# microsoft/neurips21-self-supervised-bug-detection-and-repair

Hardware: AMD Instinct MI355X
Metric: code-graphs/sec (train: fwd+bwd+optimizer) (higher is better)
Workload: dtype f32 (f16x3 / bf16x6 split products); 1 GPU; gnn-mlp hidden=128 layers=8 edge_types=16 batch=64 graphs/GPU x (2000 nodes, 10000 msgs) dropout=0.2; message_activation_placement=aggregated, message_gemm_split=f16x3, message_aggregation_function=max, global_batch=64, parallelism=dp1

## Files before the change

### include/buglab_hip.h

```cpp
#ifndef BUGLAB_HIP_H
#define BUGLAB_HIP_H

#include <stdint.h>

#ifdef __cplusplus
extern "C" {
#endif

#define BL_OK 0
#define BL_EINVAL (-1)
#define BL_ERANGE (-2)

enum { BL_ACT_NONE = 0, BL_ACT_RELU = 1, BL_ACT_SIGMOID = 2, BL_ACT_TANH = 3, BL_ACT_GELU = 4, BL_ACT_GELU_AGG = 5 };

const char* bl_last_error(void);
int bl_version(void);
void bl_set_deterministic(int32_t on);
int32_t bl_get_deterministic(void);

typedef struct {
  const float* x[3];
  const int32_t* idx[3];
  int32_t ld[3];
  int32_t width[3];
// ... 151 lines not shown
                               const uint32_t* win_bits, int32_t ld_bits, const int32_t* type_ptr, int32_t T, const float* wt,
                               int32_t E, int32_t Dm, int32_t Din, int32_t split, float* g_h_lo, int32_t ld_lo, float* g_h_hi,
                               int32_t ld_hi, float* g_src, int32_t ld_src, void* stream);

int bl_gru_cell_fwd(const float* gi, const float* gh, const float* h, int32_t ld_h, int32_t N, int32_t D,
                    bl_dropout_t drop, float* out, void* stream);
int bl_gru_cell_bwd(const float* g_out, const float* gi, const float* gh, const float* h, int32_t ld_h, int32_t N,
                    int32_t D, bl_dropout_t drop, float* g_gi, float* g_gh, float* g_h, void* stream);

int64_t bl_gru_scan_saved_elems(int32_t B, int32_t L, int32_t Hh);
int bl_gru_scan_fwd(const float* gi, int32_t ld_gi, const float* w_hh, const float* b_hh, const int32_t* lens, int32_t B, int32_t L,
                    int32_t Hh, float* out, int32_t ld_out, float* saved, void* stream);
int bl_gru_scan_bwd(const float* g_out, int32_t ld_g, const float* w_hh, const float* saved, const int32_t* lens, int32_t B, int32_t L,
                    int32_t Hh, float* g_gi, int32_t ld_ggi, float* g_gh, void* stream);

typedef struct {
  int32_t N, E, T, Din, Dm, Dout;
  const int32_t *msg_src, *msg_tgt, *type_ptr, *tgt_ptr, *tgt_msgs, *src_ptr, *src_msgs, *node_order;
  const float* W;
  const float *ln_g, *ln_b;
  const float* Wd;
  const float* bd;
  int32_t msg_act;
  float ln_eps;
  bl_dropout_t drop;
  const float* Wt;
  const uint16_t* Wd_packed;
  const uint16_t* Wd_packed_bwd;
  int32_t num_hub_slots;
  int32_t aggregation;
  int32_t num_runs;
  const int32_t* run_ptr;
  const int32_t* bwd_group_ptr;
  const int32_t* bwd_group_w;
  const int32_t* bwd_rows_tgt;
  const int32_t* bwd_rows_src;
  const int32_t* tgt_run_ptr;
  const int32_t* tgt_run_rows;
  int32_t live_num_nodes;
  int32_t live_num_recv;
  int32_t live_num_msgs;
  int32_t live_num_runs;
  const int32_t* live_nodes;
  const int32_t* live_recv;
  const int32_t* live_msgs;
  const int32_t* live_run_ptr;
  const int32_t* live_group_ptr;
  const int32_t* live_rows_tgt;
  const int32_t* live_rows_src;
  const int32_t* live_src_ptr;
  const int32_t* live_src_msgs;
  const int32_t* live_run_csr_ptr;
  const int32_t* live_run_csr_rows;
} bl_mp_layer_t;
#define BL_AGG_MAX 0
#define BL_AGG_SUM 1
#define BL_AGG_MEAN 2

int64_t bl_mp_layer_saved_bytes(int32_t N, int32_t E, int32_t Din, int32_t Dm, int32_t msg_act);
int64_t bl_mp_layer_workspace_bytes(int32_t N, int32_t E, int32_t Din, int32_t Dm, int32_t Dout, int32_t backward);
int32_t bl_mp_layer_weight_image(int32_t Din, int32_t Dm, int32_t for_backward);
int64_t bl_mp_layer_packed_weight_elems(int32_t T, int32_t Din, int32_t Dm, int32_t for_backward);

int bl_mp_layer_fwd(const bl_mp_layer_t* L, const float* h_lo, int32_t ld_lo, int32_t width_lo, const float* h_hi,
                    int32_t ld_hi, const uint16_t* w_packed, float* h_out, int32_t* winner_out, void* saved, void* ws,
                    void* stream);
int bl_mp_layer_bwd(const bl_mp_layer_t* L, const float* h_out, const float* g_out, const uint16_t* w_packed_bwd,
                    const void* saved, void* ws, float* g_h_lo, int32_t ld_lo, int32_t width_lo, float* g_h_hi,
                    int32_t ld_hi, float* g_W, float* g_ln_g, float* g_ln_b, float* g_Wd, float* g_bd, void* stream,
                    void* side_stream, int32_t join_side);

int32_t bl_node_update_bwd_ok(int32_t Dm, int32_t Dout);
int bl_node_update_bwd(const float* g_out, const float* h_out, int32_t nrows, int32_t Dout, bl_dropout_t drop,
                       const uint16_t* wd_packed_bwd, const float* agg, const float* mean, const float* rstd, const float* ln_g,
                       const float* dact, int32_t Dm, uint16_t* g_z_packed, float* g_bias, float* gq, uint16_t* gq_packed,
                       float* g_ln_g, float* g_ln_b, void* stream);
int32_t bl_set_fused_node_bwd(int32_t on);

int bl_winbits_or_runs(uint32_t* bits, int32_t ld_bits, const int32_t* run_ptr, int32_t E, int32_t R, int32_t words, void* stream);
int bl_mp_scatter_grad_runs(const float* g_a, int32_t ld_ga, const int32_t* src_ptr, const int32_t* src_msgs,
                            const int32_t* tgt_run_ptr, const int32_t* tgt_run_rows, int32_t N, int32_t Din, int32_t split,
                            float* g_h_lo, int32_t ld_lo, float* g_h_hi, int32_t ld_hi, const int32_t* node_order,
                            int32_t num_hub_slots, void* stream);
int32_t bl_set_run_rows(int32_t on);
int bl_winbits_gather(const uint32_t* bits, int32_t ld_bits, int32_t nrows_in, const int32_t* rows, int32_t n, int32_t words,
                      uint32_t* out, int32_t ld_out, void* stream);
int bl_node_update_bwd_rows(const float* g_out, const float* h_out, const int32_t* rows, int32_t nrows, int32_t Dout, bl_dropout_t drop,
                            const uint16_t* wd_packed_bwd, const float* agg, const float* mean, const float* rstd, const float* ln_g,
                            const float* dact, int32_t Dm, uint16_t* g_z_packed, float* g_bias, float* gq, uint16_t* gq_packed,
                            float* g_ln_g, float* g_ln_b, void* stream);
int bl_mp_scatter_grad_rows(const float* g_a, int32_t ld_ga, const int32_t* src_ptr, const int32_t* src_msgs,
                            const int32_t* run_csr_ptr, const int32_t* run_csr_rows, const int32_t* out_rows, int32_t n, int32_t Din,
                            int32_t split, float* g_h_lo, int32_t ld_lo, float* g_h_hi, int32_t ld_hi, void* stream);
int32_t bl_set_live_backward(int32_t on);
int32_t bl_get_live_backward(void);

int bl_prof_enable(int32_t on);
int bl_prof_reset(void);
int bl_prof_num_kinds(void);
const char* bl_prof_kind_name(int32_t kind);
int bl_prof_read(int32_t kind, double* ms, double* flop, int64_t* launches, int32_t* overlapped);
double bl_prof_read_bytes(int32_t kind);

#define BL_H3_ROW_SCALE 256.0f
#define BL_H3_W_SCALE 64.0f
int32_t bl_set_msg_gemm_mode(int32_t mode);
int32_t bl_get_msg_gemm_mode(void);
int32_t bl_set_seq_gemm_mode(int32_t mode);
int32_t bl_seq_gemm_mode(void);
int64_t bl_h3_saturation_events(int32_t reset);
int bl_pack_f16x2(const float* x, int32_t ld, int64_t R, int32_t D, int32_t D_total, int32_t col_off, float scale,
                  const float* amax_dev, uint16_t* out, void* stream);
int bl_amax(const float* x, int64_t n, float* amax_dev, void* stream);
int64_t bl_packed_weight_elems_h3(int32_t G, int32_t K, int32_t N);
int bl_pack_weights_h3(const float* w, int32_t G, int32_t K, int32_t N, int32_t w_is_kn, float scale, uint16_t* out, void* stream);
int bl_gemm_rows_h3(const bl_rows_packed_t* a, const uint32_t* win_bits, int32_t ld_bits, const uint16_t* bp, int64_t b_group_stride,
                    const int32_t* group_ptr, const int32_t* group_w, int32_t G, int32_t M, int32_t N, int32_t K, float out_scale,
                    const float* a_amax_dev, float* c, int32_t ldc, void* stream);
int bl_gemm_wgrad_h3(const bl_rows_packed_t* a, const uint16_t* g_packed, const int32_t* g_idx, const uint32_t* win_bits,
                     int32_t ld_bits, const int32_t* group_ptr, const int32_t* group_w, int32_t G, int32_t M, int32_t N, int32_t K,
                     float out_scale, const float* g_amax_dev, float* gw, int64_t gw_group_stride, int32_t ld_gw, void* stream);

int bl_calib_mfma_bf16(int32_t iters, int32_t workgroups, float* sink, double* flop, void* stream);
int bl_calib_stream_copy(const void* src, void* dst, int64_t nbytes, void* stream);

int bl_segment_log_softmax_fwd(const float* x, const int32_t* seg_ptr, const int32_t* seg_items, int32_t nseg,
                               float eps, float* y, void* stream);
int bl_segment_log_softmax_bwd(const float* g_y, const float* y, const int32_t* seg_ptr, const int32_t* seg_items,
                               int32_t nseg, float* g_x, void* stream);

int bl_rowdot_fwd(const float* x, int32_t ldx, const float* w, const float* b, int32_t R, int32_t H, float* y,
                  void* stream);
int bl_rowdot_bwd(const float* g_y, const float* x, int32_t ldx, const float* w, int32_t R, int32_t H, float* g_x,
                  int32_t ld_gx, float* g_w, float* g_b, void* stream);

int bl_scatter_add_rows(const float* src, int32_t ld_src, int32_t col_off, int32_t width, const int32_t* idx,
                        int32_t R, float* out, int32_t ld_out, void* stream);
int bl_gather_rows(const float* x, int32_t ld_x, const int32_t* idx, int32_t R, int32_t width, float* out,
                   int32_t ld_out, void* stream);

int bl_gather_concat_mlp_score_fwd(const bl_rows_t* a, const float* W1, const float* b1, const float* w2, const float* b2,
                                   int32_t R, int32_t H, float* hidden, float* score, void* stream);
int64_t bl_gather_concat_mlp_score_workspace_bytes(int32_t R, int32_t H, int32_t K);
int bl_gather_concat_mlp_score_bwd(const bl_rows_t* a, const float* W1, const float* w2, const float* hidden,
                                   const float* g_score, int32_t R, int32_t H, void* ws, float* g_W1, float* g_b1,
                                   float* g_w2, float* g_b2, float* const* g_x, const int32_t* ld_gx, void* stream);
int64_t bl_localization_scores_saved_bytes(int32_t C, int32_t B, int32_t H);
int64_t bl_localization_scores_workspace_bytes(int32_t C, int32_t B, int32_t H, int32_t backward);
// ... 337 lines not shown
```

### neurips21-self-supervised-bug-detection-and-repair_amd/buglab/models/hip_ops/_cabi.py

```python
from __future__ import annotations

import ctypes
import os
from ctypes import POINTER, Structure, c_double, c_float, c_int8, c_int32, c_int64, c_uint32, c_uint64, c_void_p
from typing import List, NamedTuple, Optional, Sequence, Tuple

import torch

__all__ = [
    "ACT_NONE", "ACT_RELU", "ACT_SIGMOID", "ACT_TANH", "ACT_GELU", "ACT_GELU_AGG", "_ACTS", "message_activation_code", "LIB_NAME",
    "HipOpsUnavailable", "bl_rows_t", "bl_rows_packed_t", "bl_dropout_t", "bl_mp_layer_t", "bl_x6_epi_t", "bl_head_view_t",
    "bl_packed_head_view_t", "bl_great_layer_t", "bl_great_layer_grads_t", "bl_pack_job_t", "bl_bug_loss_t", "bl_varmisuse_head_t",
    "VARMISUSE_STATS", "_SIGNATURES", "EXPORTED_SYMBOLS", "load_library", "_check", "_stream", "_p", "_req", "_f32", "_i32", "Dropout",
    "NO_DROPOUT", "RowSource", "_rows", "_rows_packed"]
FORWARDED_BY_PACKAGE = ("CALL_COUNT", "_lib", "LIB_PATH")

ACT_NONE, ACT_RELU, ACT_SIGMOID, ACT_TANH, ACT_GELU, ACT_GELU_AGG = 0, 1, 2, 3, 4, 5
_ACTS = {"none": ACT_NONE, "relu": ACT_RELU, "sigmoid": ACT_SIGMOID, "tanh": ACT_TANH, "gelu": ACT_GELU,
         "gelu_aggregated": ACT_GELU_AGG}


def message_activation_code(activation: str, placement: str = "aggregated") -> str:
    if activation not in ("gelu", "none"):
        raise ValueError(f"message_activation must be 'gelu' or 'none' (got {activation!r})")
    if placement not in ("aggregated", "message"):
        raise ValueError(f"message_activation_placement must be 'aggregated' or 'message' (got {placement!r})")
    return "gelu_aggregated" if (activation == "gelu" and placement == "aggregated") else activation
LIB_NAME = "libbuglab_hip.so"
LIB_PATH = os.environ.get("BL_HIP_LIB") or os.path.join(os.path.dirname(os.path.abspath(__file__)), LIB_NAME)


class HipOpsUnavailable(RuntimeError):
    pass


class bl_rows_t(Structure):
    _fields_ = [("x", c_void_p * 3), ("idx", c_void_p * 3), ("ld", c_int32 * 3), ("width", c_int32 * 3), ("nsrc", c_int32)]


class bl_rows_packed_t(Structure):
    _fields_ = [("xp", c_void_p * 3), ("idx", c_void_p * 3), ("width", c_int32 * 3), ("nsrc", c_int32)]


class bl_dropout_t(Structure):
    _fields_ = [("p", c_float), ("seed", c_uint32), ("stream", c_uint32)]


class bl_mp_layer_t(Structure):
    _fields_ = [("N", c_int32), ("E", c_int32), ("T", c_int32), ("Din", c_int32), ("Dm", c_int32), ("Dout", c_int32),
                ("msg_src", c_void_p), ("msg_tgt", c_void_p), ("type_ptr", c_void_p), ("tgt_ptr", c_void_p), ("tgt_msgs", c_void_p),
                ("src_ptr", c_void_p), ("src_msgs", c_void_p), ("node_order", c_void_p),
                ("W", c_void_p), ("ln_g", c_void_p), ("ln_b", c_void_p), ("Wd", c_void_p), ("bd", c_void_p),
                ("msg_act", c_int32), ("ln_eps", c_float), ("drop", bl_dropout_t), ("Wt", c_void_p),
                ("Wd_packed", c_void_p), ("Wd_packed_bwd", c_void_p), ("num_hub_slots", c_int32), ("aggregation", c_int32),
                ("num_runs", c_int32), ("run_ptr", c_void_p), ("bwd_group_ptr", c_void_p), ("bwd_group_w", c_void_p),
                ("bwd_rows_tgt", c_void_p), ("bwd_rows_src", c_void_p), ("tgt_run_ptr", c_void_p), ("tgt_run_rows", c_void_p),
                ("live_num_nodes", c_int32), ("live_num_recv", c_int32), ("live_num_msgs", c_int32), ("live_num_runs", c_int32),
                ("live_nodes", c_void_p), ("live_recv", c_void_p), ("live_msgs", c_void_p), ("live_run_ptr", c_void_p),
                ("live_group_ptr", c_void_p), ("live_rows_tgt", c_void_p), ("live_rows_src", c_void_p), ("live_src_ptr", c_void_p),
                ("live_src_msgs", c_void_p), ("live_run_csr_ptr", c_void_p), ("live_run_csr_rows", c_void_p)]


class bl_x6_epi_t(Structure):
    _fields_ = [("form", c_int32), ("bias", c_void_p), ("act", c_int32), ("drop", bl_dropout_t), ("res", c_void_p), ("ld_res", c_int32),
                ("y_packed", c_void_p), ("mask_scale", c_float), ("colsum", c_void_p), ("c_packed", c_void_p)]


class bl_head_view_t(Structure):
    _fields_ = [("p", c_void_p), ("sb", c_int64), ("sh", c_int32), ("sl", c_int32)]


class bl_packed_head_view_t(Structure):
    _fields_ = [("p", c_void_p), ("W", c_int32), ("col0", c_int32), ("hs", c_int32)]


class bl_great_layer_t(Structure):
    _fields_ = [("B", c_int32), ("L", c_int32), ("H", c_int32), ("dk", c_int32), ("T", c_int32), ("FF", c_int32),
                ("row_ptr", c_void_p), ("ekey", c_void_p), ("ecode", c_void_p), ("lens", c_void_p),
                ("bias_f", c_void_p), ("bias_r", c_void_p), ("norm_g", c_void_p), ("norm_b", c_void_p), ("lin1_b", c_void_p), ("lin2_b", c_void_p),
                ("qkv_w", c_void_p), ("out_w", c_void_p), ("lin1_w", c_void_p), ("lin2_w", c_void_p),
                ("qkv_w_bwd", c_void_p), ("out_w_bwd", c_void_p), ("lin1_w_bwd", c_void_p), ("lin2_w_bwd", c_void_p),
                ("ln_eps", c_float), ("drop_attn", bl_dropout_t), ("drop_att_out", bl_dropout_t), ("drop_ff_hidden", bl_dropout_t),
                ("drop_ff_out", bl_dropout_t)]


class bl_great_layer_grads_t(Structure):
    _fields_ = [("qkv_w", c_void_p), ("out_w", c_void_p), ("lin1_w", c_void_p), ("lin1_b", c_void_p), ("lin2_w", c_void_p), ("lin2_b", c_void_p),
                ("norm_g", c_void_p), ("norm_b", c_void_p), ("bias_f", c_void_p), ("bias_r", c_void_p)]


class bl_pack_job_t(Structure):
    _fields_ = [("w", c_void_p), ("out", c_void_p), ("kind", c_int32), ("G", c_int32), ("K", c_int32), ("N", c_int32),
                ("first_block", c_int32), ("pad_", c_int32)]


class bl_bug_loss_t(Structure):
    _fields_ = [("B", c_int32), ("C", c_int32), ("Rt", c_int32), ("Rv", c_int32), ("Rs", c_int32), ("G", c_int32),
                ("loc_scores", c_void_p), ("repair_logits", c_void_p), ("loc_group_ptr", c_void_p), ("loc_group_items", c_void_p),
                ("candidate_ptr", c_void_p), ("has_bug", c_void_p), ("correct_candidate_idxs", c_void_p),
                ("repair_group_ptr", c_void_p), ("repair_group_items", c_void_p), ("logit_group", c_void_p * 3),
                ("target", c_void_p * 3), ("ntarget", c_int32 * 3), ("w_buggy", c_float), ("abstain_weight", c_float)]


class bl_varmisuse_head_t(Structure):
    _fields_ = [("B", c_int32), ("L", c_int32), ("D", c_int32), ("ln_eps", c_float), ("x", c_void_p), ("ln_g", c_void_p), ("ln_b", c_void_p),
                ("W", c_void_p), ("bias", c_void_p), ("lens_att", c_void_p), ("error_location", c_void_p), ("candidate_mask", c_void_p),
                ("target_mask", c_void_p)]


VARMISUSE_STATS = 8


_SIGNATURES = {
    "bl_version": ([], ctypes.c_int),
    "bl_set_deterministic": ([c_int32], None),
    "bl_get_deterministic": ([], c_int32),
    "bl_set_wgrad_tile": ([c_int32], c_int32),
    "bl_set_wgrad_kchunk_cap": ([c_int32], c_int32),
    "bl_node_update_bwd_ok": ([c_int32, c_int32], c_int32),
    "bl_node_update_bwd": ([c_void_p, c_void_p, c_int32, c_int32, bl_dropout_t, c_void_p, c_void_p, c_void_p, c_void_p, c_void_p, c_void_p,
                            c_int32, c_void_p, c_void_p, c_void_p, c_void_p, c_void_p, c_void_p, c_void_p], ctypes.c_int),
    "bl_set_fused_node_bwd": ([c_int32], c_int32),
    "bl_set_run_rows": ([c_int32], c_int32),
    "bl_winbits_or_runs": ([c_void_p, c_int32, c_void_p, c_int32, c_int32, c_int32, c_void_p], ctypes.c_int),
    "bl_mp_scatter_grad_runs": ([c_void_p, c_int32, c_void_p, c_void_p, c_void_p, c_void_p, c_int32, c_int32, c_int32, c_void_p, c_int32, c_void_p,
                                 c_int32, c_void_p, c_int32, c_void_p], ctypes.c_int),
    "bl_set_live_backward": ([c_int32], c_int32),
    "bl_get_live_backward": ([], c_int32),
    "bl_winbits_gather": ([c_void_p, c_int32, c_int32, c_void_p, c_int32, c_int32, c_void_p, c_int32, c_void_p], ctypes.c_int),
    "bl_node_update_bwd_rows": ([c_void_p, c_void_p, c_void_p, c_int32, c_int32, bl_dropout_t, c_void_p, c_void_p, c_void_p, c_void_p, c_void_p,
                                 c_void_p, c_int32, c_void_p, c_void_p, c_void_p, c_void_p, c_void_p, c_void_p, c_void_p], ctypes.c_int),
    "bl_mp_scatter_grad_rows": ([c_void_p, c_int32, c_void_p, c_void_p, c_void_p, c_void_p, c_void_p, c_int32, c_int32, c_int32, c_void_p,
                                 c_int32, c_void_p, c_int32, c_void_p], ctypes.c_int),
    "bl_last_error": ([], ctypes.c_char_p),
    "bl_embed_subtoken_pool_fwd": ([c_void_p, c_int32, c_int32, c_void_p, c_void_p, c_int32, c_int32, c_int32, bl_dropout_t, c_int32, c_void_p, c_int32, c_void_p, c_void_p], ctypes.c_int),
    "bl_embed_subtoken_pool_bwd": ([c_void_p, c_int32, c_void_p, c_void_p, c_void_p, c_int32, c_int32, c_int32, c_int32, c_int32, bl_dropout_t, c_int32, c_void_p, c_void_p], ctypes.c_int),
    "bl_embed_subtoken_pool_bwd_sorted": ([c_void_p, c_int32, c_void_p, c_void_p, c_void_p, c_int32, c_void_p, c_void_p, c_int32, c_int32, c_int32, bl_dropout_t, c_int32, c_void_p, c_void_p], ctypes.c_int),
    "bl_embed_subtoken_max_fwd": ([c_void_p, c_int32, c_int32, c_void_p, c_void_p, c_int32, c_int32, bl_dropout_t, c_int32, c_void_p, c_int32, c_void_p, c_void_p], ctypes.c_int),
    "bl_embed_subtoken_max_bwd": ([c_void_p, c_int32, c_void_p, c_void_p, c_int32, c_int32, c_int32, c_int32, bl_dropout_t, c_int32, c_void_p, c_void_p], ctypes.c_int),
    "bl_embed_subtoken_max_bwd_sorted": ([c_void_p, c_int32, c_void_p, c_void_p, c_void_p, c_int32, c_void_p, c_int32, c_int32, bl_dropout_t, c_int32, c_void_p, c_void_p], ctypes.c_int),
    "bl_gemm_rows": ([POINTER(bl_rows_t), c_void_p, c_int64, c_int32, c_int32, c_void_p, c_void_p, c_void_p, c_int32, c_int32, c_int32, c_int32, c_int32, bl_dropout_t, c_void_p, c_int32, c_void_p], ctypes.c_int),
    "bl_gemm_rows_routed": ([POINTER(bl_rows_t), c_void_p, c_int32, c_void_p, c_int64, c_int32, c_void_p, c_void_p, c_int32, c_int32, c_int32, c_int32, c_void_p, c_int32, c_void_p], ctypes.c_int),
    "bl_pack_bf16x3": ([c_void_p, c_int32, c_int64, c_int32, c_void_p, c_void_p], ctypes.c_int),
    "bl_pack_weights_x6": ([c_void_p, c_int32, c_int32, c_int32, c_int32, c_void_p, c_void_p], ctypes.c_int),
    "bl_pack_job_blocks": ([c_int32, c_int32, c_int32, c_int32], c_int64),
    "bl_pack_weights_multi": ([c_void_p, c_int32, c_int32, c_void_p], ctypes.c_int),
    "bl_gemm_rows_x6": ([POINTER(bl_rows_packed_t), c_void_p, c_int32, c_void_p, c_int64, c_void_p, c_void_p, c_int32, c_int32, c_int32, c_int32, c_void_p, c_int32, c_void_p], ctypes.c_int),
    "bl_gemm_rows_x6w_ok": ([c_int32, c_int32], c_int32),
    "bl_set_rows_tile": ([c_int32], c_int32),
    "bl_packed_weight_elems_x6w": ([c_int32, c_int32, c_int32], c_int64),
    "bl_pack_weights_x6w": ([c_void_p, c_int32, c_int32, c_int32, c_int32, c_void_p, c_void_p], ctypes.c_int),
    "bl_gemm_rows_x6w": ([POINTER(bl_rows_packed_t), c_void_p, c_int32, c_void_p, c_int64, c_void_p, c_void_p, c_int32, c_int32, c_int32, c_int32, c_void_p, c_int32, c_void_p], ctypes.c_int),
    "bl_gemm_rows_x6_epi": ([POINTER(bl_rows_packed_t), c_void_p, c_int64, c_void_p, c_void_p, c_int32, c_int32, c_int32, c_int32, c_void_p, c_int32,
                             bl_dropout_t, c_void_p, c_int32, c_void_p], ctypes.c_int),
    "bl_gemm_rows_x6_epi2": ([POINTER(bl_rows_packed_t), c_void_p, c_int32, c_int32, c_int32, POINTER(bl_x6_epi_t), c_void_p, c_int32, c_void_p], ctypes.c_int),
    "bl_gemm_wgrad_x6": ([POINTER(bl_rows_packed_t), c_void_p, c_void_p, c_void_p, c_void_p, c_int32, c_int32, c_int32, c_int32, c_void_p, c_int64,
                          c_int32, c_void_p], ctypes.c_int),
    "bl_routed_dgrad_vec_ok": ([c_int32, c_int32], c_int32),
    "bl_routed_dgrad_vec": ([c_void_p, c_int32, c_void_p, c_void_p, c_int32, c_void_p, c_int32, c_void_p, c_int32, c_int32, c_int32, c_void_p, c_int32, c_void_p], ctypes.c_int),
    "bl_routed_dgrad_nodes": ([c_void_p, c_int32, c_void_p, c_void_p, c_void_p, c_int32, c_void_p, c_int32, c_void_p, c_int32, c_int32, c_int32, c_int32,
                               c_void_p, c_int32, c_void_p, c_int32, c_void_p], ctypes.c_int),
    "bl_routed_dgrad_nodes_rows": ([c_void_p, c_int32, c_void_p, c_void_p, c_void_p, c_int32, c_void_p, c_int32, c_void_p, c_int32, c_int32, c_int32,
                                    c_int32, c_void_p, c_int32, c_void_p, c_int32, c_void_p, c_int32, c_void_p], ctypes.c_int),
    "bl_gemm_wgrad_routed_x6": ([POINTER(bl_rows_packed_t), c_void_p, c_void_p, c_void_p, c_int32, c_void_p, c_void_p, c_int32, c_int32, c_int32, c_int32, c_void_p, c_int64, c_int32, c_void_p], ctypes.c_int),
    "bl_gemm_wgrad": ([POINTER(bl_rows_t), c_void_p, c_int32, c_void_p, c_void_p, c_int32, c_int32, c_int32, c_int32, c_void_p, c_int64, c_int32, c_void_p], ctypes.c_int),
    "bl_gemm_wgrad_routed": ([POINTER(bl_rows_t), c_void_p, c_int32, c_void_p, c_void_p, c_int32, c_void_p, c_void_p, c_int32, c_int32, c_int32, c_int32, c_void_p, c_int64, c_int32, c_void_p], ctypes.c_int),
    "bl_pack_bf16x3_cols": ([c_void_p, c_int32, c_int64, c_int32, c_int32, c_int32, c_void_p, c_void_p], ctypes.c_int),
    "bl_mp_scatter_grad_split": ([c_void_p, c_int32, c_void_p, c_void_p, c_void_p, c_void_p, c_int32, c_int32, c_int32, c_void_p, c_int32, c_void_p, c_int32, c_void_p, c_void_p], ctypes.c_int),
    "bl_mp_layer_saved_bytes": ([c_int32, c_int32, c_int32, c_int32, c_int32], c_int64),
    "bl_mp_layer_workspace_bytes": ([c_int32, c_int32, c_int32, c_int32, c_int32, c_int32], c_int64),
    "bl_mp_layer_packed_weight_elems": ([c_int32, c_int32, c_int32, c_int32], c_int64),
    "bl_mp_layer_weight_image": ([c_int32, c_int32, c_int32], c_int32),
    "bl_mp_layer_fwd": ([POINTER(bl_mp_layer_t), c_void_p, c_int32, c_int32, c_void_p, c_int32, c_void_p, c_void_p, c_void_p, c_void_p, c_void_p, c_void_p], ctypes.c_int),
    "bl_mp_layer_bwd": ([POINTER(bl_mp_layer_t), c_void_p, c_void_p, c_void_p, c_void_p, c_void_p, c_void_p, c_int32, c_int32, c_void_p, c_int32,
                         c_void_p, c_void_p, c_void_p, c_void_p, c_void_p, c_void_p, c_void_p, c_int32], ctypes.c_int),
    "bl_gather_concat_mlp_score_fwd": ([POINTER(bl_rows_t), c_void_p, c_void_p, c_void_p, c_void_p, c_int32, c_int32, c_void_p, c_void_p, c_void_p], ctypes.c_int),
    "bl_gather_concat_mlp_score_workspace_bytes": ([c_int32, c_int32, c_int32], c_int64),
    "bl_gather_concat_mlp_score_bwd": ([POINTER(bl_rows_t), c_void_p, c_void_p, c_void_p, c_void_p, c_int32, c_int32, c_void_p, c_void_p, c_void_p,
                                        c_void_p, c_void_p, POINTER(c_void_p), POINTER(c_int32), c_void_p], ctypes.c_int),
    "bl_localization_scores_saved_bytes": ([c_int32, c_int32, c_int32], c_int64),
    "bl_localization_scores_workspace_bytes": ([c_int32, c_int32, c_int32, c_int32], c_int64),
# ... 290 lines not shown
```

### neurips21-self-supervised-bug-detection-and-repair_amd/buglab/models/hip_ops/graph.py

```python
from __future__ import annotations

import ctypes
from typing import NamedTuple, Optional

import torch

from . import _switches, _streams
from ._cabi import (ACT_GELU_AGG, ACT_NONE, ACT_TANH, _ACTS, bl_mp_layer_t, _check, Dropout, _f32, _i32, load_library,
                    NO_DROPOUT, _p, _stream)
from ._streams import _direct_grad_target, _direct_small, _on_side_stream, _timed
from ._autograd import _take_saved
from .gemm import (act_bwd, gemm_rows, gemm_rows_routed, gemm_rows_x6, gemm_wgrad, gemm_wgrad_routed, gemm_wgrad_routed_x6,
                   layernorm_bwd, pack_bf16x3, pack_weights_x6, scatter_add_rows, segment_max, x6_ok)
from .weights import _as_groups, _packed_layer_weights, _packed_message_weights, _transposed_layer_weights

__all__ = ["GraphIndex", "MessageRuns", "LiveRows", "live_rows_of", "POOLINGS", "AGGREGATIONS", "_EmbedSubtokenMax", "embed_subtoken_max", "_MpLayer", "node_update_bwd",
           "_use_vector_dgrad", "_layer_desc", "_MpLayerFused", "_pending_uses", "set_grad_ready_callback", "_note_use",
           "_notify_backward_launched", "fused_layer_ok", "_GatedMpLayer", "gated_mp_layer", "_MpLayerFeat",
           "mp_layer_with_edge_features", "mp_layer"]


class MessageRuns(NamedTuple):

    run_ptr: torch.Tensor
    bwd_group_ptr: torch.Tensor
    bwd_group_w: torch.Tensor
    bwd_rows_tgt: torch.Tensor
    bwd_rows_src: torch.Tensor
    tgt_run_ptr: torch.Tensor
    tgt_run_rows: torch.Tensor

    @classmethod
    def of(cls, *arrays) -> Optional["MessageRuns"]:
        return cls(*arrays) if all(a is not None for a in arrays) else None

    @property
    def num_runs(self) -> int:
        return int(self.run_ptr.shape[0]) - 1


class LiveRows(NamedTuple):

    nodes: torch.Tensor
    recv: torch.Tensor
    msgs: torch.Tensor
    run_ptr: torch.Tensor
    group_ptr: torch.Tensor
    rows_tgt: torch.Tensor
    rows_src: torch.Tensor
    src_ptr: torch.Tensor
    src_msgs: torch.Tensor
    run_csr_ptr: torch.Tensor
    run_csr_rows: torch.Tensor


def live_rows_of(live_arrays: torch.Tensor, live_layout, T: int):
    out = []
    for row in (live_layout.tolist() if hasattr(live_layout, "tolist") else live_layout):
        nn, nr, ex, rx = row[:4]
        sizes = (nn, nr, ex, rx + 1, 2 * T + 1, ex + rx, ex + rx, nr + 1, ex, nr + 1, rx)
        out.append(LiveRows(*[live_arrays[o : o + n] for o, n in zip(row[4:], sizes)]))
    return out


class GraphIndex(NamedTuple):

    msg_src: torch.Tensor
    msg_tgt: torch.Tensor
    type_ptr: torch.Tensor
    tgt_ptr: torch.Tensor
    tgt_msgs: torch.Tensor
    src_ptr: torch.Tensor
    src_msgs: torch.Tensor
    num_nodes: int
    num_messages: int
    num_types: int
    node_order: Optional[torch.Tensor] = None
    num_hubs: int = -1
    runs: Optional[MessageRuns] = None
    live: Optional[LiveRows] = None


POOLINGS = ("max", "sum", "mean")


AGGREGATIONS = ("max", "sum", "mean")


class _EmbedSubtokenMax(torch.autograd.Function):
    @staticmethod
    def forward(ctx, table, ids, lens, drop: Dropout, tok_csr, before_pool: bool, comb: int):
        _f32(table, "embedding table")
        N, S = ids.shape
        V, H = table.shape
        out = torch.empty((N, H), dtype=torch.float32, device=table.device)
        argsub = torch.empty((N, H), dtype=torch.int8, device=table.device) if comb == 0 else None
        _check(
            load_library().bl_embed_subtoken_pool_fwd(table.data_ptr(), V, H, _i32(ids).data_ptr(), _i32(lens).data_ptr(), N, S, comb,
                                                      drop.c(), int(bool(before_pool)), out.data_ptr(), out.stride(0), _p(argsub), _stream()),
            "bl_embed_subtoken_pool_fwd")
        ctx.saved = (table, ids, lens, argsub, drop, V, H, tok_csr, int(bool(before_pool)), comb)
        return out

    @staticmethod
    def backward(ctx, g_out):
        table, ids, lens, argsub, drop, V, H, tok_csr, before_pool, comb = _take_saved(ctx)
        g_out = g_out.contiguous()
        N, S = ids.shape
        direct = _direct_small(table)
        g_table = direct if direct is not None else torch.zeros((V, H), dtype=torch.float32, device=g_out.device)
        if tok_csr is not None:
            occ, chunk_ptr, chunk_tok = tok_csr
            _check(
                load_library().bl_embed_subtoken_pool_bwd_sorted(g_out.data_ptr(), g_out.stride(0), _i32(occ).data_ptr(),
                                                                 _i32(chunk_ptr).data_ptr(), _i32(chunk_tok).data_ptr(),
                                                                 int(chunk_tok.shape[0]), _i32(lens).data_ptr(), _p(argsub), S, H, comb, drop.c(),
                                                                 before_pool, g_table.data_ptr(), _stream()),
                "bl_embed_subtoken_pool_bwd_sorted")
        else:
            _check(
                load_library().bl_embed_subtoken_pool_bwd(g_out.data_ptr(), g_out.stride(0), ids.data_ptr(), _i32(lens).data_ptr(), _p(argsub),
                                                          N, S, H, V, comb, drop.c(), before_pool, g_table.data_ptr(), _stream()),
                "bl_embed_subtoken_pool_bwd")
        return (None if direct is not None else g_table), None, None, None, None, None, None


def embed_subtoken_max(table, ids, lens, drop: Dropout = NO_DROPOUT, tok_csr=None, dropout_before_pooling: bool = False,
                       combination: str = "max"):
    return _EmbedSubtokenMax.apply(table, ids, lens, drop, tok_csr, bool(dropout_before_pooling), POOLINGS.index(combination))


class _MpLayer(torch.autograd.Function):

    @staticmethod
    def forward(ctx, h, W, ln_g, ln_b, Wd, bd, g: GraphIndex, msg_act: int, drop: Dropout):
# ... 72 lines not shown
        with side2:
            if hp is not None:
                gemm_wgrad_routed_x6([(hp, g.msg_src, Din), (hp, g.msg_tgt, Din)], gqp, g.msg_tgt, bits, E, Dm, g_W,
                                     gw_group_stride=K2 * Dm, group_ptr=g.type_ptr, G=T)
            else:
                gemm_wgrad_routed([(h, g.msg_src), (h, g.msg_tgt)], gq, g.msg_tgt, arg, E, Dm, g_W, gw_group_stride=K2 * Dm,
                                  group_ptr=g.type_ptr, G=T)
        if gqp is not None:
            g_a = gemm_rows_x6([(gqp, g.msg_tgt, Dm)], pack_weights_x6(W, False), E, K2, group_ptr=g.type_ptr, G=T,
                               win_bits=bits, kind="gemm_rows_nk_routed_x6")
        else:
            g_a = gemm_rows_routed(gq, g.msg_tgt, arg, W, E, K2, b_group_stride=K2 * Dm, ldb=Dm, group_ptr=g.type_ptr, G=T)
        g_h = torch.empty((N, Din), dtype=torch.float32, device=dev)
        _check(
            load_library().bl_mp_scatter_grad(g_a.data_ptr(), g_a.stride(0), g.src_ptr.data_ptr(), g.src_msgs.data_ptr(),
                                              g.tgt_ptr.data_ptr(), g.tgt_msgs.data_ptr(), N, Din, 0, g_h.data_ptr(),
                                              g_h.stride(0), _p(g.node_order), _stream()),
            "bl_mp_scatter_grad")
        if W_direct is not None and Wd_direct is not None:
            _streams.mark_free_running()
            side2.detach(h, gq, arg, bits, hp, gqp)
            side1.detach(ln_out, g_z)
            pair.__exit__(None, None, None)
            return g_h, None, g_lng, g_lnb, None, g_bd, None, None, None
        side2.join()
        side1.join()
        pair.__exit__(None, None, None)
        if W_direct is not None:
            g_W = None
        if Wd_direct is not None:
            g_Wd = None
        return g_h, g_W, g_lng, g_lnb, g_Wd, g_bd, None, None, None


def node_update_bwd(g_out, h_out, drop: "Dropout", wd_packed_bwd, agg, mean, rstd, ln_g, dact, g_bias, g_ln_g, g_ln_b, want_f32=True):
    N, Dout = g_out.shape
    Dm = agg.shape[1]
    dev = g_out.device
    gz = torch.empty((N, 3 * Dout), dtype=torch.int16, device=dev)
    gq = torch.empty((N, Dm), dtype=torch.float32, device=dev) if want_f32 else None
    gqp = torch.empty((N, 3 * Dm), dtype=torch.int16, device=dev)
    _check(load_library().bl_node_update_bwd(_f32(g_out).data_ptr(), _f32(h_out).data_ptr(), N, Dout, drop.c(), wd_packed_bwd.data_ptr(),
                                             _f32(agg).data_ptr(), mean.data_ptr(), rstd.data_ptr(), ln_g.data_ptr(), _p(dact), Dm,
                                             gz.data_ptr(), _p(g_bias), _p(gq), gqp.data_ptr(), g_ln_g.data_ptr(), g_ln_b.data_ptr(),
                                             _stream()), "bl_node_update_bwd")
    return gz, gq, gqp


def _use_vector_dgrad(lib, E: int, Dm: int, K2: int) -> bool:
    want = _switches.DGRAD_VEC if _switches.DGRAD_VEC is not None else not lib.bl_get_msg_gemm_mode()
    return bool(want) and E > 0 and bool(lib.bl_routed_dgrad_vec_ok(Dm, K2))


def _layer_desc(g: "GraphIndex", W, ln_g, ln_b, Wd, bd, Din, msg_act, drop: Dropout, agg: int = 0, backward: bool = False) -> bl_mp_layer_t:
    L = bl_mp_layer_t()
    L.aggregation = int(agg)
    L.N, L.E, L.T, L.Din, L.Dm, L.Dout = g.num_nodes, g.num_messages, W.shape[0], Din, W.shape[2], Wd.shape[1]
    L.msg_src, L.msg_tgt, L.type_ptr = g.msg_src.data_ptr(), g.msg_tgt.data_ptr(), g.type_ptr.data_ptr()
    L.tgt_ptr, L.tgt_msgs, L.src_ptr, L.src_msgs = g.tgt_ptr.data_ptr(), g.tgt_msgs.data_ptr(), g.src_ptr.data_ptr(), g.src_msgs.data_ptr()
    L.node_order = _p(g.node_order)
    L.num_hub_slots = int(g.num_hubs)
    L.W, L.ln_g, L.ln_b, L.Wd, L.bd = W.data_ptr(), ln_g.data_ptr(), ln_b.data_ptr(), Wd.data_ptr(), bd.data_ptr()
    L.msg_act, L.ln_eps, L.drop = int(msg_act), 1e-5, drop.c()
    if g.runs is not None and g.runs.num_runs > 0:
        L.num_runs = g.runs.num_runs
        for name in MessageRuns._fields:
            setattr(L, name, getattr(g.runs, name).data_ptr())
    if backward and g.live is not None and g.live.nodes.shape[0] > 0:
        lv = g.live
        L.live_num_nodes, L.live_num_recv = int(lv.nodes.shape[0]), int(lv.recv.shape[0])
        L.live_num_msgs, L.live_num_runs = int(lv.msgs.shape[0]), int(lv.run_ptr.shape[0]) - 1
        for name in LiveRows._fields:
            setattr(L, "live_" + name, getattr(lv, name).data_ptr())
    return L


class _MpLayerFused(torch.autograd.Function):

    @staticmethod
    def forward(ctx, h_lo, h_hi, W, ln_g, ln_b, Wd, bd, g: GraphIndex, msg_act: int, drop: Dropout, agg: int = 0):
        _f32(h_lo, "node states")
        lib = load_library()
        N = h_lo.shape[0]
        Din = h_lo.shape[1] + (h_hi.shape[1] if h_hi is not None else 0)
        T, K2, Dm = W.shape
        Dout = Wd.shape[1]
        E = g.num_messages
        assert K2 == 2 * Din and T == g.num_types and N == g.num_nodes
        for t, nm in ((W, "W"), (ln_g, "ln_g"), (ln_b, "ln_b"), (Wd, "Wd"), (bd, "bd")):
            _f32(t, nm)
        need_bwd = any(ctx.needs_input_grad[:7])
        use_vec = agg == 0 and _use_vector_dgrad(lib, E, Dm, K2)
        wkn, wnk = _packed_message_weights(W, Din, need_bwd and not use_vec)
        wt = _transposed_layer_weights(W) if (need_bwd and use_vec) else None
        dev = h_lo.device
        L = _layer_desc(g, W, ln_g, ln_b, Wd, bd, Din, msg_act, drop, agg)
        dense_x6 = _switches.DENSE_X6 and Dm % 32 == 0 and Dout % 32 == 0
        wd_kn = wd_nk = None
        if dense_x6:
            wd_kn, wd_nk = _packed_layer_weights(Wd, need_bwd)
            L.Wd_packed = wd_kn.data_ptr()
        infer = not need_bwd and _switches.INFERENCE_MODE
        saved_act = ACT_GELU_AGG if (agg == 2 and msg_act == ACT_NONE) else msg_act
        saved = None if infer else torch.empty((lib.bl_mp_layer_saved_bytes(N, E + L.num_runs, Din, Dm, saved_act),), dtype=torch.uint8, device=dev)
        ws = torch.empty((lib.bl_mp_layer_workspace_bytes(N, E, Din, Dm, Dout, 3 if infer else 0),), dtype=torch.uint8, device=dev)
        out = torch.empty((N, Dout), dtype=torch.float32, device=dev)
        winner = torch.empty((N, Dm), dtype=torch.int32, device=dev) if (_switches.WINNER_SINK is not None and agg == 0) else None
        _check(lib.bl_mp_layer_fwd(ctypes.byref(L), h_lo.data_ptr(), h_lo.stride(0), h_lo.shape[1], _p(h_hi),
                                   h_hi.stride(0) if h_hi is not None else 0, wkn.data_ptr(), out.data_ptr(), _p(winner),
                                   _p(saved), ws.data_ptr() if (E > 0 or infer) else None, _stream()), "bl_mp_layer_fwd")
        if winner is not None:
            _switches.WINNER_SINK.append(winner)
        if need_bwd:
            _note_use((W, ln_g, ln_b, Wd, bd))
        ctx.save_for_backward(out)
        ctx.saved = (h_lo.shape[1], h_hi.shape[1] if h_hi is not None else 0, W, ln_g, ln_b, Wd, bd, g, msg_act, drop, saved, wnk,
                     dense_x6, wd_kn, wd_nk, wt, agg)
        return out

    @staticmethod
    def backward(ctx, g_out):
        w_lo, w_hi, W, ln_g, ln_b, Wd, bd, g, msg_act, drop, saved, wnk, dense_x6, wd_kn, wd_nk, wt, agg = _take_saved(ctx)
        (out,) = ctx.saved_tensors
        lib = load_library()
        N, E = g.num_nodes, g.num_messages
        T, K2, Dm = W.shape
        Din, Dout = w_lo + w_hi, Wd.shape[1]
        dev = out.device
        g_out = g_out.contiguous()
        use_vec = agg == 0 and _use_vector_dgrad(lib, E, Dm, 2 * Din)
        if use_vec and wt is None:
            wt = _transposed_layer_weights(W)
        if wnk is None and not use_vec:
            wnk = _packed_message_weights(W, Din, True)[1]
        direct = [_direct_small(bd), _direct_small(ln_g), _direct_small(ln_b), _direct_grad_target(Wd), _direct_grad_target(W)]
        tgt = [d if d is not None else torch.zeros_like(p) for d, p in zip(direct, (bd, ln_g, ln_b, Wd, W))]
        g_bd, g_lng, g_lnb, g_Wd, g_W = tgt
        L = _layer_desc(g, W, ln_g, ln_b, Wd, bd, Din, msg_act, drop, agg, backward=True)
        if dense_x6:
            if wd_nk is None:
                wd_nk = pack_weights_x6(_as_groups(Wd.detach()), False)
            L.Wd_packed, L.Wd_packed_bwd = wd_kn.data_ptr(), wd_nk.data_ptr()
        ws_mode = 1
        if use_vec:
            L.Wt = wt.data_ptr()
            if not lib.bl_get_deterministic():
                ws_mode = 2
        ws = torch.empty((lib.bl_mp_layer_workspace_bytes(N, E, Din, Dm, Dout, ws_mode),), dtype=torch.uint8, device=dev)
        g_lo = torch.empty((N, w_lo), dtype=torch.float32, device=dev)
        g_hi = torch.empty((N, w_hi), dtype=torch.float32, device=dev) if w_hi else None
        side = _streams.side_stream_for_current_device()
        free_running = side is not None and direct[3] is not None and direct[4] is not None
        _check(lib.bl_mp_layer_bwd(ctypes.byref(L), out.data_ptr(), g_out.data_ptr(), _p(wnk), saved.data_ptr(), ws.data_ptr(),
                                   g_lo.data_ptr(), g_lo.stride(0), w_lo, _p(g_hi), g_hi.stride(0) if g_hi is not None else 0,
                                   g_W.data_ptr(), g_lng.data_ptr(), g_lnb.data_ptr(), g_Wd.data_ptr(), g_bd.data_ptr(), _stream(),
                                   side.cuda_stream if side is not None else None, 0 if free_running else 1), "bl_mp_layer_bwd")
        if free_running:
            _streams.mark_free_running(saved, ws)
        ret = [None if d is not None else t for d, t in zip(direct, tgt)]
        if all(d is not None for d in direct):
            _notify_backward_launched((W, ln_g, ln_b, Wd, bd))
        return g_lo, g_hi, ret[4], ret[1], ret[2], ret[3], ret[0], None, None, None, None


_pending_uses = {}


def set_grad_ready_callback(fn) -> None:
    _switches.GRAD_READY_CALLBACK = fn
    _pending_uses.clear()


def _note_use(params) -> None:
    if _switches.GRAD_READY_CALLBACK is not None:
        for p in params:
            _pending_uses[id(p)] = _pending_uses.get(id(p), 0) + 1


def _notify_backward_launched(params) -> None:
    if _switches.GRAD_READY_CALLBACK is None:
        return
    done = []
    for p in params:
        n = _pending_uses.get(id(p), 1) - 1
        if n <= 0:
            _pending_uses.pop(id(p), None)
            done.append(p)
        else:
            _pending_uses[id(p)] = n
    if done:
        _switches.GRAD_READY_CALLBACK(done)
# ... 94 lines not shown
            dact = None
        out = gemm_rows([(ln_out, None)], _f32(Wd, "Wd"), N, Dout, bias=_f32(bd), act=ACT_TANH, drop=drop)
        ctx.save_for_backward(out)
        ctx.saved = (h, hp, tp, bits, W, ln_g, Wd, table, msg_feat, dact, arg, agg, mean, rstd, ln_out, g, drop)
        return out

    @staticmethod
    def backward(ctx, g_out):
        h, hp, tp, bits, W, ln_g, Wd, table, msg_feat, dact, arg, agg, mean, rstd, ln_out, g, drop = _take_saved(ctx)
        (out,) = ctx.saved_tensors
        N, Din = h.shape
        T, K3, Dm = W.shape
        F, Dout, E, dev = table.shape[1], Wd.shape[1], g.num_messages, h.device
        z = lambda *shape: torch.zeros(shape, dtype=torch.float32, device=dev)
        g_bd, g_Wd, g_W, g_lng, g_lnb, g_table = z(Dout), torch.zeros_like(Wd), torch.zeros_like(W), z(Dm), z(Dm), torch.zeros_like(table)
        g_z = act_bwd(g_out.contiguous(), out, ACT_TANH, drop, g_bd)
        gemm_wgrad([(ln_out, None)], g_z, N, Dout, g_Wd)
        g_ln = gemm_rows([(g_z, None)], Wd, N, Dm, b_is_nk=True, ldb=Dout)
        if hp is not None:
            gqp = layernorm_bwd(g_ln, agg, mean, rstd, ln_g, g_lng, g_lnb, post_scale=dact, want="packed")
            gemm_wgrad_routed_x6([(hp, g.msg_src, Din), (hp, g.msg_tgt, Din), (tp, msg_feat, F)], gqp, g.msg_tgt, bits, E, Dm, g_W,
                                 gw_group_stride=K3 * Dm, group_ptr=g.type_ptr, G=T)
            g_a = gemm_rows_x6([(gqp, g.msg_tgt, Dm)], _packed_layer_weights(W, True)[1], E, K3, group_ptr=g.type_ptr, G=T, win_bits=bits,
                               kind="gemm_rows_nk_routed_x6")
        else:
            gq = layernorm_bwd(g_ln, agg, mean, rstd, ln_g, g_lng, g_lnb, post_scale=dact)
            src3 = [(h, g.msg_src), (h, g.msg_tgt), (table, msg_feat)]
            gemm_wgrad_routed(src3, gq, g.msg_tgt, arg, E, Dm, g_W, gw_group_stride=K3 * Dm, group_ptr=g.type_ptr, G=T)
            g_a = gemm_rows_routed(gq, g.msg_tgt, arg, W, E, K3, b_group_stride=K3 * Dm, ldb=Dm, group_ptr=g.type_ptr, G=T)
        g_h = torch.empty((N, Din), dtype=torch.float32, device=dev)
        _check(load_library().bl_mp_scatter_grad(g_a.data_ptr(), g_a.stride(0), g.src_ptr.data_ptr(), g.src_msgs.data_ptr(), g.tgt_ptr.data_ptr(),
                                                 g.tgt_msgs.data_ptr(), N, Din, 0, g_h.data_ptr(), g_h.stride(0), _p(g.node_order), _stream()),
               "bl_mp_scatter_grad")
        if E > 0:
            scatter_add_rows(g_a, 2 * Din, F, msg_feat, g_table)
        return g_h, g_W, g_lng, g_lnb, g_Wd, g_bd, g_table, None, None, None, None


def mp_layer_with_edge_features(h, W, ln_g, ln_b, Wd, bd, table, msg_feat, graph: GraphIndex, msg_act: str = "gelu_aggregated",
                                drop: Dropout = NO_DROPOUT):
    if isinstance(h, (tuple, list)):
        h = torch.cat(list(h), dim=-1)
    return _MpLayerFeat.apply(h.contiguous(), W, ln_g, ln_b, Wd, bd, table, msg_feat, graph, _ACTS[msg_act], drop)


def mp_layer(h, W, ln_g, ln_b, Wd, bd, graph: GraphIndex, msg_act: str = "gelu_aggregated", drop: Dropout = NO_DROPOUT,
             aggregation: str = "max"):
    pair = isinstance(h, (tuple, list))
    Din = sum(t.shape[1] for t in h) if pair else h.shape[1]
    agg = AGGREGATIONS.index(aggregation)
    if fused_layer_ok(Din, W.shape[2]) and (not pair or h[0].shape[1] % 32 == 0):
        lo, hi = (h[0].contiguous(), h[1].contiguous()) if pair else (h.contiguous(), None)
        return _MpLayerFused.apply(lo, hi, W, ln_g, ln_b, Wd, bd, graph, _ACTS[msg_act], drop, agg)
    if agg != 0:
        raise NotImplementedError("sum / mean message aggregation runs in the one-call layer form only (state and message widths multiples of "
                                  "32, message width <= 512, FUSED_LAYER on)")
    if pair:
        h = torch.cat(list(h), dim=-1)
    return _MpLayer.apply(h.contiguous(), W, ln_g, ln_b, Wd, bd, graph, _ACTS[msg_act], drop)
```

### neurips21-self-supervised-bug-detection-and-repair_amd/buglab/models/hip_ops/runtime.py

```python
from __future__ import annotations

import os

from . import _switches
from ._cabi import load_library

__all__ = ["set_deterministic", "_MSG_GEMM_MODES", "set_msg_gemm_mode", "msg_gemm_mode", "set_seq_gemm_mode", "seq_gemm_mode", "set_wgrad_tile",
           "set_wgrad_kchunk_cap", "set_fused_node_bwd", "set_run_rows", "set_live_backward", "live_backward", "deterministic"]


def set_deterministic(on: bool = True) -> None:
    load_library().bl_set_deterministic(1 if on else 0)
    os.environ["BL_DETERMINISTIC"] = "1" if on else "0"


_MSG_GEMM_MODES = ("bf16x6", "f16x3", "f16x1")


def set_msg_gemm_mode(mode: str) -> str:
    if mode not in _MSG_GEMM_MODES:
        raise ValueError(f"mode must be one of {_MSG_GEMM_MODES}")
    prev = load_library().bl_set_msg_gemm_mode(_MSG_GEMM_MODES.index(mode))
    return _MSG_GEMM_MODES[prev]


def msg_gemm_mode() -> str:
    return _MSG_GEMM_MODES[load_library().bl_get_msg_gemm_mode()]


def set_seq_gemm_mode(mode: str) -> str:
    if mode not in _switches._SEQ_GEMM_MODES:
        raise ValueError(f"mode must be one of {_switches._SEQ_GEMM_MODES}")
    prev = load_library().bl_set_seq_gemm_mode(_switches._SEQ_GEMM_MODES.index(mode))
    return _switches._SEQ_GEMM_MODES[prev]


def seq_gemm_mode() -> str:
    return _switches._SEQ_GEMM_MODES[load_library().bl_seq_gemm_mode()]


def set_wgrad_tile(rows: int) -> int:
    return int(load_library().bl_set_wgrad_tile(int(rows)))


def set_wgrad_kchunk_cap(rows: int) -> int:
    return int(load_library().bl_set_wgrad_kchunk_cap(int(rows)))


def set_fused_node_bwd(on: bool) -> bool:
    return bool(load_library().bl_set_fused_node_bwd(1 if on else 0))


def set_run_rows(on: bool) -> bool:
    return bool(load_library().bl_set_run_rows(1 if on else 0))


def set_live_backward(on: bool) -> bool:
    return bool(load_library().bl_set_live_backward(1 if on else 0))


def live_backward() -> bool:
    return bool(load_library().bl_get_live_backward())


def deterministic() -> bool:
    return bool(load_library().bl_get_deterministic())
```

### neurips21-self-supervised-bug-detection-and-repair_amd/buglab/models/layers/messagepassing.py

```python
from __future__ import annotations

import math
from typing import Any, Dict, List, NamedTuple, Optional

import torch
from torch import nn

from buglab.models import hip_ops
from buglab.models.hip_ops import Dropout, GraphIndex, MessageRuns, live_rows_of


class GnnOutput(NamedTuple):

    input_node_representations: torch.Tensor
    output_node_representations: torch.Tensor
    node_to_graph_idx: torch.Tensor
    node_idx_references: Dict[str, torch.Tensor]
    node_graph_idx_reference: Dict[str, torch.Tensor]
    num_graphs: int
    head_node_representations: Optional[torch.Tensor] = None
    head_idx_references: Optional[Dict[str, torch.Tensor]] = None


MAX_MESSAGE_DIMENSION = 512
# ... 86 lines not shown

    def __init__(self, state_dimension: int, message_dimension: int, num_edge_types: int,
                 message_aggregation_function: str = "max", dropout_rate: float = 0.0):
        super().__init__()
        if message_aggregation_function != "max":
            raise NotImplementedError("the HIP path implements the reference's `max` aggregation (gnnlayerdefs.py:47,63)")
        D, Dm, T = state_dimension, message_dimension, num_edge_types
        _check_message_width(Dm, "GatedMessagePassingLayer")
        self.state_dimension, self.message_dimension, self.output_state_dimension = D, Dm, D
        self.num_edge_types, self.dropout_rate = T, dropout_rate
        k = 1.0 / math.sqrt(D)
        self.W = nn.Parameter(_uniform_(torch.empty(T, D, Dm), 1.0 / math.sqrt(D)))
        self.Wi = nn.Parameter(_uniform_(torch.empty(Dm, 3 * D), k))
        self.bi = nn.Parameter(_uniform_(torch.empty(3 * D), k))
        self.Wh = nn.Parameter(_uniform_(torch.empty(D, 3 * D), k))
        self.bh = nn.Parameter(_uniform_(torch.empty(3 * D), k))

    def forward(self, node_states, graph: GraphIndex, drop: Dropout):
        return hip_ops.gated_mp_layer(node_states, self.W, self.Wi, self.bi, self.Wh, self.bh, graph, drop)


class ConcatResidualLayer:

    def __init__(self, hidden_state_size: int):
        self.hidden_state_size = hidden_state_size
        self.output_state_dimension = 2 * hidden_state_size
        self.dummy = _PassThrough(self)

    def pass_through_dummy_layer(self):
        return self.dummy


class _PassThrough:
    def __init__(self, owner: ConcatResidualLayer):
        self.owner = owner
        self.output_state_dimension = owner.hidden_state_size


class GraphNeuralNetwork(nn.Module):

    def __init__(self, node_embedder: SubtokenEmbedder, layer_recipe: List[Any], edge_embedder: Optional[TokenEmbedder] = None):
        super().__init__()
        self.embed = node_embedder
        self.edge_embed = edge_embedder
        self._recipe = layer_recipe
        mp, seen = [], set()
        for l in layer_recipe:
            if isinstance(l, (MlpMessagePassingLayer, GatedMessagePassingLayer)) and id(l) not in seen:
                seen.add(id(l))
                mp.append(l)
        self.mp = nn.ModuleList(mp)
        self.input_node_state_dim = node_embedder.embedding_size
        self.output_node_state_dim = [l for l in layer_recipe if isinstance(l, nn.Module)][-1].output_state_dimension

    @property
    def message_passing_layers(self):
        return list(self.mp)

    def forward(self, *, token_ids, token_lens, msg_src, msg_tgt, type_ptr, tgt_ptr, tgt_msgs, src_ptr, src_msgs,
                node_to_graph, reference_node_ids, reference_node_graph_idx, num_graphs, num_nodes, num_messages,
                return_all_states: bool = False, dropout_seed: Optional[int] = None, tok_occ=None, tok_chunk_ptr=None,
                tok_chunk_id=None, node_order=None, num_hub_nodes: int = -1, msg_feat=None, input_transform=None, run_ptr=None,
                bwd_group_ptr=None, bwd_group_w=None, bwd_rows_tgt=None, bwd_rows_src=None, tgt_run_ptr=None, tgt_run_rows=None,
                live_arrays=None, live_layout=None, live_backward: bool = False, **_unused) -> GnnOutput:
        graph = GraphIndex(msg_src, msg_tgt, type_ptr, tgt_ptr, tgt_msgs, src_ptr, src_msgs, int(num_nodes),
                           int(num_messages), int(type_ptr.shape[0]) - 1, node_order, int(num_hub_nodes),
                           MessageRuns.of(run_ptr, bwd_group_ptr, bwd_group_w, bwd_rows_tgt, bwd_rows_src, tgt_run_ptr, tgt_run_rows))
        training = self.training and dropout_seed is not None
        seed = int(dropout_seed or 0)
        mk = lambda rate, stream: Dropout(rate if training else 0.0, seed, stream)
        tok_csr = (tok_occ, tok_chunk_ptr, tok_chunk_id) if tok_occ is not None else None
        h0 = self.embed(token_ids, token_lens, mk(self.embed.dropout_rate, 0), tok_csr)
        if input_transform is not None:
            h0 = input_transform(h0)
        edge_features = None
        if self.edge_embed is not None:
            if msg_feat is None:
                raise ValueError("the model has an edge-feature embedding but the minibatch carries no `msg_feat`")
            edge_features = (self.edge_embed.table, msg_feat)
        live = []
        if live_backward and live_arrays is not None and live_layout is not None and not return_all_states and input_transform is None:
            live = live_rows_of(live_arrays, live_layout, graph.num_types)
        num_mp = sum(1 for l in self._recipe if isinstance(l, nn.Module))
        h = h0
        all_states = [h0]
        stash: Dict[int, torch.Tensor] = {}
        li = 0
        for layer in self._recipe:
            if isinstance(layer, _PassThrough):
                stash[id(layer.owner)] = h
            elif isinstance(layer, ConcatResidualLayer):
                h = (stash.pop(id(layer)), h)
            else:
                if isinstance(h, tuple) and not isinstance(layer, MlpMessagePassingLayer):
                    h = torch.cat(h, dim=-1)
                depth = num_mp - 1 - li
                layer_graph = graph._replace(live=live[depth]) if depth < len(live) else graph
                if isinstance(layer, MlpMessagePassingLayer) and layer.features_dimension > 0:
                    h = layer(h, graph, mk(layer.dropout_rate, 1 + li), edge_features)
                else:
                    h = layer(h, layer_graph, mk(layer.dropout_rate, 1 + li))
                li += 1
                all_states.append(h)
        if isinstance(h, tuple):
            h = torch.cat(h, dim=-1)
        out = torch.cat(all_states, dim=-1) if return_all_states else h
        return GnnOutput(h0, out, node_to_graph, reference_node_ids, reference_node_graph_idx, int(num_graphs))
```

### neurips21-self-supervised-bug-detection-and-repair_amd/csrc/bl_common.h

```cpp
#pragma once
#include <hip/hip_runtime.h>
#include <stdint.h>
#include <stdio.h>

#include "../../include/buglab_hip.h"

#define BL_WAVE 64

void bl_set_error(const char* fmt, ...);
extern "C" int32_t bl_get_deterministic(void);
int bl_num_cus();
int bl_max_lds_per_block();
unsigned* bl_order_counters(int n, void* stream);
unsigned* bl_h3_sat_counter();

int bl_segment_max_fwd_impl(const float* x, int32_t ldx, const int32_t* seg_ptr, const int32_t* seg_items, int32_t nseg, int32_t D,
                            int32_t act, float* out, int32_t* arg, const float* ln_g, const float* ln_b, float eps, float* ln_out,
                            float* mean, float* rstd, float* dact, uint32_t* winbits, const int32_t* seg_order,
                            uint16_t* ln_out_packed, int32_t num_hub_slots, void* stream);
int bl_segment_sum_fwd_impl(const float* x, int32_t ldx, const int32_t* seg_ptr, const int32_t* seg_items, int32_t nseg, int32_t D,
                            int32_t act, int32_t mean_agg, float* out, const float* ln_g, const float* ln_b, float eps, float* ln_out,
                            float* mean, float* rstd, float* dact, const int32_t* seg_order, uint16_t* ln_out_packed, void* stream);
int bl_act_bwd_impl(const float* g_y, const float* y, int32_t nrows, int32_t N, int32_t ld, int32_t act, bl_dropout_t drop,
                    float* g_z, float* g_bias, uint16_t* g_z_packed, void* stream);
int bl_mp_scatter_src_accum_impl(const float* g_src, int32_t ld_src, const int32_t* src_ptr, const int32_t* src_msgs, int32_t N,
                                 int32_t Din, int32_t split, float* g_h_lo, int32_t ld_lo, float* g_h_hi, int32_t ld_hi,
                                 const int32_t* node_order, int32_t hub_slots, void* stream);
int bl_mp_scatter_grad_hubs_impl(const float* g_a, int32_t ld_ga, const int32_t* src_ptr, const int32_t* src_msgs, const int32_t* tgt_ptr,
                                 const int32_t* tgt_msgs, int32_t N, int32_t Din, int32_t split, float* g_h_lo, int32_t ld_lo, float* g_h_hi,
                                 int32_t ld_hi, const int32_t* node_order, int32_t hub_slots, int32_t col_tgt, void* stream,
                                 const int32_t* out_rows = nullptr);
int bl_gemm_wgrad_h3_impl(const bl_rows_packed_t* a, const uint16_t* g_packed, const int32_t* g_idx, const uint32_t* win_bits,
                          int32_t ld_bits, const int32_t* group_ptr, const int32_t* group_w, int32_t G, int32_t M, int32_t N, int32_t K,
                          float out_scale, const float* g_amax_dev, float* gw, int64_t gw_group_stride, int32_t ld_gw,
                          bool group_w_one_to_one, void* stream);

int bl_node_update_bwd_impl(const float* g_out, const float* h_out, int32_t nrows, int32_t Dout, bl_dropout_t drop,
                            const uint16_t* wd_packed_bwd, const float* agg, const float* mean, const float* rstd, const float* ln_g,
                            const float* dact, int32_t Dm, uint16_t* g_z_packed, float* g_bias, float* gq, uint16_t* gq_packed,
                            float* g_ln_g, float* g_ln_b, float* gq_amax, const int32_t* rows, void* stream);

struct BlProfScope {
  void* st;
  bool on;
  BlProfScope(int kind, double flop, void* stream, double bytes = 0.0, bool overlapped = false);
  ~BlProfScope();
};
enum {
  BL_PROF_PACK_ROWS = 0,
  BL_PROF_LINEAR_FWD = 17,
  BL_PROF_LINEAR_DGRAD,
  BL_PROF_LINEAR_WGRAD,
  BL_PROF_ATTN_PROBS_FWD,
  BL_PROF_ATTN_PROBS_BWD,
  BL_PROF_ATTN_ROWS_TIMES,
  BL_PROF_ATTN_TRANSPOSED_TIMES,
  BL_PROF_ADD_LAYERNORM,
  BL_PROF_LAYERNORM_BWD_BRANCH
};

#define BL_CHECK_ARG(cond, ...)   \
  do {                            \
    if (!(cond)) {                \
      bl_set_error(__VA_ARGS__);  \
      return BL_EINVAL;           \
    }                             \
  } while (0)
#define BL_CHECK_RANGE(cond, ...) \
  do {                            \
    if (!(cond)) {                \
      bl_set_error(__VA_ARGS__);  \
      return BL_ERANGE;           \
// ... 138 lines not shown
```

### neurips21-self-supervised-bug-detection-and-repair_amd/csrc/bl_gemm_h3.hip

```cpp
#include <stdio.h>
#include <stdlib.h>

#include "bl_common.h"
#include "bl_gemm_host.h"
#include "bl_gemm_split.h"
#include "bl_x6_locate.h"
#include "bl_h3_image.h"

__global__ __launch_bounds__(256) void pack_rows_h_kernel(const float* __restrict__ x, int ld, long long R, int D, uint4* __restrict__ out,
                                                          int kg_total, int kg_off, float scale, const float* __restrict__ amax_dev,
                                                          unsigned* __restrict__ sat_counter) {
  const int kgs = D >> 3;
  const long long t = (long long)blockIdx.x * blockDim.x + threadIdx.x;
  if (t >= R * kgs) return;
  if (amax_dev) scale *= h3_scale_from_amax(*amax_dev);
  const long long r = t / kgs;
  const int kgn = kg_total;
  const int kg = (int)(t % kgs) + kg_off;
  x -= 8 * kg_off;
  const float4 a = *reinterpret_cast<const float4*>(x + r * ld + 8 * kg);
  const float4 b = *reinterpret_cast<const float4*>(x + r * ld + 8 * kg + 4);
  const float v[8] = {a.x, a.y, a.z, a.w, b.x, b.y, b.z, b.w};
  uint16_t h[8], l[8];
  bool sat = false;
#pragma unroll
  for (int j = 0; j < 8; ++j) split2h(v[j] * scale, h[j], l[j], sat);
  if (sat && sat_counter) atomicAdd(sat_counter, 1u);
  uint4* o = out + r * 2 * kgn + kg;
  o[0] = make_uint4(PK(h[0], h[1]), PK(h[2], h[3]), PK(h[4], h[5]), PK(h[6], h[7]));
  o[kgn] = make_uint4(PK(l[0], l[1]), PK(l[2], l[3]), PK(l[4], l[5]), PK(l[6], l[7]));
}

__global__ __launch_bounds__(256) void pack_weights_h_kernel(const float* __restrict__ w, int G, int K, int N, int w_is_kn,
                                                             uint4* __restrict__ out, float scale, unsigned* __restrict__ sat_counter) {
  pack_weights_h_thread(w, G, K, N, w_is_kn, out, (long long)blockIdx.x * blockDim.x + threadIdx.x, scale, sat_counter);
}

template <bool MASKED, bool ONE>
__global__ __launch_bounds__(256, MASKED ? 2 : 3) void gemm_rows_h3_kernel(
    const uint4* __restrict__ xp0, const uint4* __restrict__ xp1, const uint4* __restrict__ xp2,
    const int* __restrict__ idx0, const int* __restrict__ idx1, const int* __restrict__ idx2, int w0, int w1, int w2,
    int koff1, int koff2, int nsrc, const uint32_t* __restrict__ win_bits, int ld_bits, const uint4* __restrict__ bp,
    long long strideB, const int* __restrict__ group_ptr, const int* __restrict__ group_w, int G, int M, int N, int K,
    float* __restrict__ c, int ldc, int xcd_remap, float out_scale, const float* __restrict__ a_amax_dev) {
  gemm_rows_body<SplitF16x2, MASKED, -1, ONE>(xp0, xp1, xp2, idx0, idx1, idx2, w0, w1, w2, koff1, koff2, nsrc, win_bits, ld_bits, bp,
                                              strideB, group_ptr, group_w, G, M, N, K, c, ldc, xcd_remap, X6Epi{}, out_scale, a_amax_dev);
}

template <bool ROUTED, bool ONE>
__global__ __launch_bounds__(256, 2) void gemm_wgrad_h3_kernel(
    const uint4* __restrict__ xp0, const uint4* __restrict__ xp1, const uint4* __restrict__ xp2,
    const int* __restrict__ idx0, const int* __restrict__ idx1, const int* __restrict__ idx2, int w0, int w1, int w2,
    int koff1, int koff2, int nsrc, const uint4* __restrict__ gp, const int* __restrict__ g_idx,
    const uint32_t* __restrict__ win_bits, int ld_bits, const int* __restrict__ group_ptr, const int* __restrict__ group_w, int G,
    int M, int N, int K, int kchunk, float* __restrict__ gw_base, long long strideW, int ldw, int ntiles_n, int xcd_remap,
    unsigned* __restrict__ order_ctr, float out_scale, const float* __restrict__ g_amax_dev) {
  gemm_wgrad_body<SplitF16x2, ROUTED, ONE>(xp0, xp1, xp2, idx0, idx1, idx2, w0, w1, w2, koff1, koff2, nsrc, gp, g_idx, win_bits, ld_bits,
                                           group_ptr, group_w, G, M, N, K, kchunk, gw_base, strideW, ldw, ntiles_n, xcd_remap, order_ctr,
                                           out_scale, g_amax_dev);
}

__global__ __launch_bounds__(256) void amax_kernel(const float* __restrict__ x, long long n4, float* __restrict__ amax) {
  __shared__ float part[4];
  float m = 0.f;
  const long long stride = (long long)gridDim.x * blockDim.x;
  for (long long i = (long long)blockIdx.x * blockDim.x + threadIdx.x; i < n4; i += stride) {
    const float4 v = reinterpret_cast<const float4*>(x)[i];
    m = fmaxf(m, fmaxf(fmaxf(fabsf(v.x), fabsf(v.y)), fmaxf(fabsf(v.z), fabsf(v.w))));
  }
  m = bl_wave_max(m);
  if ((threadIdx.x & 63) == 0) part[threadIdx.x >> 6] = m;
  __syncthreads();
  if (threadIdx.x == 0) {
    m = fmaxf(fmaxf(part[0], part[1]), fmaxf(part[2], part[3]));
    if (m > 0.f) atomicMax(reinterpret_cast<unsigned int*>(amax), __float_as_uint(m));
  }
}

unsigned* bl_h3_sat_counter() {
  static unsigned* ctr[BL_MAX_DEVICES] = {nullptr};
  int dev = 0;
  if (hipGetDevice(&dev) != hipSuccess || dev < 0 || dev >= BL_MAX_DEVICES) return nullptr;
  if (ctr[dev] == nullptr) {
    if (hipMalloc((void**)&ctr[dev], sizeof(unsigned)) != hipSuccess) return nullptr;
    if (hipMemset(ctr[dev], 0, sizeof(unsigned)) != hipSuccess) return nullptr;
  }
  return ctr[dev];
}

extern "C" int64_t bl_h3_saturation_events(int32_t reset) {
  unsigned* c = bl_h3_sat_counter();
  unsigned v = 0;
  if (c == nullptr || hipMemcpy(&v, c, sizeof(v), hipMemcpyDeviceToHost) != hipSuccess) return -1;
  if (reset && hipMemset(c, 0, sizeof(unsigned)) != hipSuccess) return -1;
  return (int64_t)v;
}

extern "C" int bl_pack_f16x2(const float* x, int32_t ld, int64_t R, int32_t D, int32_t D_total, int32_t col_off, float scale,
                             const float* amax_dev, uint16_t* out, void* stream) {
  if (R == 0) return BL_OK;
  BL_CHECK_ARG(x && out && bl_aligned16(x) && bl_aligned16(out), "bl_pack_f16x2: null or misaligned pointer");
  BL_CHECK_ARG(D > 0 && D % 8 == 0 && ld % 4 == 0 && D_total % 8 == 0 && col_off % 8 == 0 && col_off >= 0 && col_off + D <= D_total,
               "bl_pack_f16x2: widths / offset must be multiples of 8 with col_off + D <= D_total");
  BL_CHECK_ARG(scale > 0.f, "bl_pack_f16x2: scale must be positive (a power of two)");
  const long long total = (long long)R * (D / 8);
  hipLaunchKernelGGL(pack_rows_h_kernel, dim3((unsigned)((total + 255) / 256)), dim3(256), 0, (hipStream_t)stream, x, ld, (long long)R, D,
                     reinterpret_cast<uint4*>(out), D_total / 8, col_off / 8, scale, amax_dev, bl_h3_sat_counter());
  BL_LAUNCH_CHECK("bl_pack_f16x2");
  return BL_OK;
}

extern "C" int bl_amax(const float* x, int64_t n, float* amax_dev, void* stream) {
  if (n == 0) return BL_OK;
  BL_CHECK_ARG(x && amax_dev && bl_aligned16(x) && n % 4 == 0, "bl_amax: aligned pointer and a multiple of 4 elements required");
  const long long n4 = n / 4;
  const int grid = (int)((n4 + 255) / 256 < (long long)bl_num_cus() * 2 ? (n4 + 255) / 256 : (long long)bl_num_cus() * 2);
  hipLaunchKernelGGL(amax_kernel, dim3(grid), dim3(256), 0, (hipStream_t)stream, x, n4, amax_dev);
  BL_LAUNCH_CHECK("bl_amax");
  return BL_OK;
}

extern "C" int64_t bl_packed_weight_elems_h3(int32_t G, int32_t K, int32_t N) { return (int64_t)G * ((N + 127) / 128) * (K / 32) * 8192; }

extern "C" int bl_pack_weights_h3(const float* w, int32_t G, int32_t K, int32_t N, int32_t w_is_kn, float scale, uint16_t* out,
                                  void* stream) {
  if (G == 0) return BL_OK;
  BL_CHECK_ARG(w && out && bl_aligned16(out), "bl_pack_weights_h3: null or misaligned pointer");
  BL_CHECK_ARG(K > 0 && K % 32 == 0 && N > 0 && scale > 0.f, "bl_pack_weights_h3: K must be a multiple of 32 (got %d), scale positive", K);
  const long long total = (long long)G * ((N + 127) / 128) * (K / 32) * 512;
  hipLaunchKernelGGL(pack_weights_h_kernel, dim3((unsigned)((total + 255) / 256)), dim3(256), 0, (hipStream_t)stream, w, G, K, N, w_is_kn,
                     reinterpret_cast<uint4*>(out), scale, bl_h3_sat_counter());
  BL_LAUNCH_CHECK("bl_pack_weights_h3");
  return BL_OK;
}

bool g_h3_one_term = false;

extern "C" int bl_gemm_rows_h3(const bl_rows_packed_t* a, const uint32_t* win_bits, int32_t ld_bits, const uint16_t* bp,
                               int64_t b_group_stride, const int32_t* group_ptr, const int32_t* group_w, int32_t G, int32_t M, int32_t N,
                               int32_t K, float out_scale, const float* a_amax_dev, float* c, int32_t ldc, void* stream) {
  const char* who = "bl_gemm_rows_h3";
  if (M == 0) return BL_OK;
  BlPackedRows r;
  dim3 grid;
  if (int rc = bl_rows_gemm_plan(who, a, win_bits, ld_bits, bp, group_ptr, G, M, N, K, c, ldc, XBM, r, grid)) return rc;
  BL_CHECK_ARG(b_group_stride % 8 == 0 && (G <= 1 || b_group_stride >= bl_packed_weight_elems_h3(1, K, N)),
               "%s: packed group stride must cover one group's tiled weights (bl_pack_weights_h3)", who);
  BL_CHECK_ARG(out_scale > 0.f, "%s: out_scale must be positive", who);
#define H3_ARGS                                                                                                               \
  BL_PACKED_ROWS_ARGS(r), win_bits, ld_bits, reinterpret_cast<const uint4*>(bp), (long long)(b_group_stride / 8), group_ptr, \
      group_w, G, M, N, K, c, ldc, 1, out_scale, a_amax_dev
  if (g_h3_one_term) {
    if (win_bits)
      hipLaunchKernelGGL((gemm_rows_h3_kernel<true, true>), grid, dim3(256), 0, (hipStream_t)stream, H3_ARGS);
    else
      hipLaunchKernelGGL((gemm_rows_h3_kernel<false, true>), grid, dim3(256), 0, (hipStream_t)stream, H3_ARGS);
  } else if (win_bits)
    hipLaunchKernelGGL((gemm_rows_h3_kernel<true, false>), grid, dim3(256), 0, (hipStream_t)stream, H3_ARGS);
  else
    hipLaunchKernelGGL((gemm_rows_h3_kernel<false, false>), grid, dim3(256), 0, (hipStream_t)stream, H3_ARGS);
  BL_LAUNCH_CHECK(who);
// ... 47 lines not shown
```

### neurips21-self-supervised-bug-detection-and-repair_amd/csrc/bl_gemm_split.h

```cpp
#pragma once
#include <float.h>

#include "bl_common.h"
#include "bl_x6_locate.h"

typedef float f32x16 __attribute__((ext_vector_type(16)));
typedef __bf16 bf16x8 __attribute__((ext_vector_type(8)));
typedef _Float16 f16x8 __attribute__((ext_vector_type(8)));
typedef short s16x4 __attribute__((ext_vector_type(4)));

#define XBM 128
#define XBN 128
#define PK(a_, b_) ((uint32_t)(a_) | ((uint32_t)(b_) << 16))

__device__ __forceinline__ float h3_scale_from_amax(float amax) {
  if (!(amax > 0.f) || amax > FLT_MAX) return 1.f;
  int e;
  (void)frexpf(amax, &e);
  int k = 14 - e;
  k = k > 100 ? 100 : (k < -100 ? -100 : k);
  return ldexpf(1.f, k);
}

struct SplitBf16x3 {
  static constexpr int NP = 3;
  typedef bf16x8 frag;
  static constexpr bool SCALED = false;
  static constexpr bool STREAM_OUT = false;
  static constexpr bool swizzled(bool masked) { return masked; }
  static constexpr int row(bool masked, bool one) { return one ? (masked ? 4 : 5) : (masked ? 12 : 13); }
  static constexpr int NT = 6;
  static __device__ __forceinline__ f32x16 term(int t, const frag* x, const frag* y, f32x16 a) {
    constexpr int X[NT] = {1, 2, 0, 1, 0, 0}, Y[NT] = {1, 0, 2, 0, 1, 0};
    return __builtin_amdgcn_mfma_f32_32x32x16_bf16(x[X[t]], y[Y[t]], a, 0, 0, 0);
  }
};

struct SplitF16x2 {
  static constexpr int NP = 2;
  typedef f16x8 frag;
  static constexpr bool SCALED = true;
  static constexpr bool STREAM_OUT = true;
  static constexpr bool swizzled(bool) { return false; }
  static constexpr int row(bool, bool) { return 9; }
  static constexpr int NT = 3;
  static __device__ __forceinline__ f32x16 term(int t, const frag* x, const frag* y, f32x16 a) {
    constexpr int X[NT] = {1, 0, 0}, Y[NT] = {0, 1, 0};
    return __builtin_amdgcn_mfma_f32_32x32x16_f16(x[X[t]], y[Y[t]], a, 0, 0, 0);
  }
};

struct X6Epi {
  const float* bias;
  int act;
  uint32_t drop_key, drop_thresh;
  float drop_scale;
  int form;
  const float* res;
  int ld_res;
  const uint2* himask;
  float mask_scale;
  float* colsum;
  uint2* c_packed;
};

template <class S, bool MASKED, int EPI, bool ONE>
__device__ __forceinline__ void gemm_rows_body(
    const uint4* __restrict__ xp0, const uint4* __restrict__ xp1, const uint4* __restrict__ xp2,
    const int* __restrict__ idx0, const int* __restrict__ idx1, const int* __restrict__ idx2, int w0, int w1, int w2,
    int koff1, int koff2, int nsrc, const uint32_t* __restrict__ win_bits, int ld_bits, const uint4* __restrict__ bp,
    long long strideB, const int* __restrict__ group_ptr, const int* __restrict__ group_w, int G, int M, int N, int K,
    float* __restrict__ c, int ldc, int xcd_remap, X6Epi epi, float out_scale, const float* __restrict__ a_amax_dev) {
  static_assert(EPI == -1 || !S::SCALED, "the epilogues are built for the unscaled split only");
  constexpr bool E_ACT = EPI >= 0 && EPI < 32, E_PACK = EPI >= 16 && (EPI < 32 || EPI == 64), E_RES = EPI == 32, E_MASK = EPI == 64;
  constexpr int ACT = EPI >= 0 ? (EPI & 15) : 0;
  constexpr bool SWZ = S::swizzled(MASKED);
  constexpr int NP = ONE ? 1 : S::NP;
  constexpr int T0 = ONE ? S::NT - 1 : 0;
  constexpr int XROW = S::row(MASKED, ONE);
  constexpr int XEPI = 4 * 32 * 68 / 4;
  constexpr int XLDS = (XBM + XBN) * XROW > XEPI ? (XBM + XBN) * XROW : XEPI;
#define XSLOT(row_, kg_) (SWZ ? ((kg_) ^ (((row_) >> 2) & 3)) : (kg_))
  __shared__ uint4 ABs[XLDS];
  uint4* As = ABs;
  uint4* Bs = ABs + XBM * XROW;

  const int tid = threadIdx.x, lane = tid & 63, wave = tid >> 6;
  int g, row0, nrows, tile_y;
  if (!x6_locate(group_ptr, G, M, XBM, xcd_remap, tile_y, g, row0, nrows)) return;
  const int n0 = tile_y * XBN;
  const int wsel = group_w ? group_w[g] : g;
  const uint4* __restrict__ Bt = bp + (long long)wsel * strideB + (size_t)tile_y * (K >> 5) * (S::NP * 512) + tid;

  const int p_kg = tid & 3, p_row0 = tid >> 2;
  int gr0[2], gr1[2], gr2[2];
#pragma unroll
  for (int i = 0; i < 2; ++i) {
    const int r = row0 + min(p_row0 + 64 * i, nrows - 1);
    gr0[i] = idx0 ? idx0[r] : r;
    gr1[i] = nsrc > 1 ? (idx1 ? idx1[r] : r) : 0;
    gr2[i] = nsrc > 2 ? (idx2 ? idx2[r] : r) : 0;
  }
  uint4 ra[2][NP], rb[2][NP];
  uint32_t ma[2];
  const int nk = (K + 31) / 32;

#define ROWS_LOAD_STAGE(k0_)                                                                                  \
  {                                                                                                           \
    const int k_ = (k0_) + 8 * p_kg;                                                                          \
    const int kc_ = k_ < K ? k_ : 0;                                                                          \
    int j_ = 0;                                                                                               \
    if (nsrc > 1 && kc_ >= koff1) j_ = 1;                                                                     \
    if (nsrc > 2 && kc_ >= koff2) j_ = 2;                                                                     \
    const int kl_ = kc_ - (j_ == 0 ? 0 : (j_ == 1 ? koff1 : koff2));                                          \
    const uint4* base_ = j_ == 0 ? xp0 : (j_ == 1 ? xp1 : xp2);                                               \
    const int wj_ = j_ == 0 ? w0 : (j_ == 1 ? w1 : w2);                                                       \
    _Pragma("unroll") for (int i = 0; i < 2; ++i) {                                                           \
      const int row_ = p_row0 + 64 * i;                                                                       \
      const int gr_ = j_ == 0 ? gr0[i] : (j_ == 1 ? gr1[i] : gr2[i]);                                         \
      const uint4* src_ = base_ + (size_t)gr_ * S::NP * (wj_ >> 3) + (kl_ >> 3);                              \
      ra[i][0] = src_[0];                                                                                     \
      if constexpr (NP > 1) ra[i][1] = src_[wj_ >> 3];                                                        \
      if constexpr (NP > 2) ra[i][2] = src_[2 * (wj_ >> 3)];                                                  \
      if (MASKED) ma[i] = win_bits[(size_t)(row0 + min(row_, nrows - 1)) * ld_bits + (kc_ >> 5)];              \
      const uint4* bsrc_ = Bt + (size_t)((k0_) >> 5) * (S::NP * 512) + i * (S::NP * 256);                     \
      rb[i][0] = bsrc_[0];                                                                                    \
      if constexpr (NP > 1) rb[i][1] = bsrc_[256];                                                            \
// ... 24 lines not shown
#pragma unroll
    for (int tj = 0; tj < 2; ++tj)
#pragma unroll
      for (int r = 0; r < 16; ++r) acc[ti][tj][r] = 0.f;

  const int wm = wave >> 1, wn = wave & 1, li = lane & 31, half = lane >> 5;

  ROWS_LOAD_STAGE(0)
  ROWS_STORE_STAGE(0)
  __syncthreads();
  for (int kt = 0; kt < nk; ++kt) {
    if (kt + 1 < nk) ROWS_LOAD_STAGE((kt + 1) * 32)
#pragma unroll
    for (int s = 0; s < 2; ++s) {
      const int kg = 2 * s + half;
      typename S::frag af[2][NP], bf[2][NP];
#pragma unroll
      for (int t = 0; t < 2; ++t) {
        const uint4* pa = &As[(wm * 64 + t * 32 + li) * XROW + XSLOT(li, kg)];
        const uint4* pb = &Bs[(wn * 64 + t * 32 + li) * XROW + XSLOT(li, kg)];
#pragma unroll
        for (int p = 0; p < NP; ++p) {
          af[t][p] = __builtin_bit_cast(typename S::frag, pa[4 * p]);
          bf[t][p] = __builtin_bit_cast(typename S::frag, pb[4 * p]);
        }
      }
#pragma unroll
      for (int ti = 0; ti < 2; ++ti)
#pragma unroll
        for (int tj = 0; tj < 2; ++tj) {
          f32x16 a = acc[ti][tj];
#pragma unroll
          for (int t = T0; t < S::NT; ++t) a = S::term(t, bf[tj], af[ti], a);
          acc[ti][tj] = a;
        }
    }
    __syncthreads();
    if (kt + 1 < nk) {
      ROWS_STORE_STAGE((kt + 1) * 32)
      __syncthreads();
    }
  }
#undef ROWS_LOAD_STAGE
#undef ROWS_STORE_STAGE
#undef XSLOT

  if constexpr (S::SCALED)
    if (a_amax_dev) out_scale /= h3_scale_from_amax(*a_amax_dev);
  float* stage = reinterpret_cast<float*>(ABs) + wave * (32 * 68);
  float4 csum = make_float4(0.f, 0.f, 0.f, 0.f);
#pragma unroll
  for (int ti = 0; ti < 2; ++ti) {
    const int m = wm * 64 + ti * 32 + li;
#pragma unroll
    for (int tj = 0; tj < 2; ++tj)
#pragma unroll
      for (int gq = 0; gq < 4; ++gq) {
        const int n = n0 + wn * 64 + tj * 32 + 8 * gq + 4 * half;
        float v[4] = {acc[ti][tj][4 * gq + 0], acc[ti][tj][4 * gq + 1], acc[ti][tj][4 * gq + 2], acc[ti][tj][4 * gq + 3]};
        if constexpr (S::SCALED) {
#pragma unroll
          for (int u = 0; u < 4; ++u) v[u] *= out_scale;
        }
        if (E_ACT) {
          float4 bv = make_float4(0.f, 0.f, 0.f, 0.f);
          if (epi.bias && n < N) bv = *reinterpret_cast<const float4*>(epi.bias + n);
          v[0] += bv.x; v[1] += bv.y; v[2] += bv.z; v[3] += bv.w;
#pragma unroll
          for (int u = 0; u < 4; ++u) {
            v[u] = bl_act(ACT, v[u]);
            if (epi.drop_thresh) {
              const uint32_t idx = (uint32_t)(row0 + m) * (uint32_t)N + (uint32_t)(n + u);
              v[u] = ((bl_lowbias32(idx + epi.drop_key) >> 8) >= epi.drop_thresh) ? v[u] * epi.drop_scale : 0.f;
            }
          }
        }
        *reinterpret_cast<float4*>(stage + li * 68 + tj * 32 + 8 * gq + 4 * half) = make_float4(v[0], v[1], v[2], v[3]);
      }
    const int c4 = lane & 15, n = n0 + wn * 64 + 4 * c4;
#pragma unroll
    for (int j = 0; j < 8; ++j) {
      const int r = (lane >> 4) + 4 * j;
      const int mm = wm * 64 + ti * 32 + r;
      float4 v = *reinterpret_cast<const float4*>(stage + r * 68 + 4 * c4);
      if (mm < nrows && n < N) {
        const size_t grow = (size_t)(row0 + mm);
        if (E_RES) {
          const float4 rv = *reinterpret_cast<const float4*>(epi.res + grow * epi.ld_res + n);
          v.x += rv.x; v.y += rv.y; v.z += rv.z; v.w += rv.w;
        }
        if (E_MASK) {
          const uint2 hm = epi.himask[(grow * 3 * N + n) >> 2];
          v.x = (hm.x & 0x7fffu) ? v.x * epi.mask_scale : 0.f;
          v.y = (hm.x & 0x7fff0000u) ? v.y * epi.mask_scale : 0.f;
          v.z = (hm.y & 0x7fffu) ? v.z * epi.mask_scale : 0.f;
          v.w = (hm.y & 0x7fff0000u) ? v.w * epi.mask_scale : 0.f;
          csum.x += v.x; csum.y += v.y; csum.z += v.z; csum.w += v.w;
        }
        if (E_PACK) {
          uint16_t h[4], m[4], l[4];
          split3(v.x, h[0], m[0], l[0]);
          split3(v.y, h[1], m[1], l[1]);
          split3(v.z, h[2], m[2], l[2]);
          split3(v.w, h[3], m[3], l[3]);
          uint2* o = epi.c_packed + ((grow * 3 * N + n) >> 2);
          o[0] = make_uint2(PK(h[0], h[1]), PK(h[2], h[3]));
          o[N >> 2] = make_uint2(PK(m[0], m[1]), PK(m[2], m[3]));
          o[N >> 1] = make_uint2(PK(l[0], l[1]), PK(l[2], l[3]));
        } else if constexpr (S::STREAM_OUT) {
          bl_store_streaming(c + grow * ldc + n, v);
        } else {
          *reinterpret_cast<float4*>(c + grow * ldc + n) = v;
        }
      }
    }
  }
  if (E_MASK) {
    csum.x += __shfl_xor(csum.x, 16, 64); csum.y += __shfl_xor(csum.y, 16, 64); csum.z += __shfl_xor(csum.z, 16, 64); csum.w += __shfl_xor(csum.w, 16, 64);
    csum.x += __shfl_xor(csum.x, 32, 64); csum.y += __shfl_xor(csum.y, 32, 64); csum.z += __shfl_xor(csum.z, 32, 64); csum.w += __shfl_xor(csum.w, 32, 64);
    const int n = n0 + wn * 64 + 4 * (lane & 15);
    if (lane < 16 && n < N && epi.colsum) {
      unsafeAtomicAdd(epi.colsum + n, csum.x);
      unsafeAtomicAdd(epi.colsum + n + 1, csum.y);
      unsafeAtomicAdd(epi.colsum + n + 2, csum.z);
      unsafeAtomicAdd(epi.colsum + n + 3, csum.w);
    }
  }
}

#define WRS 160
#define WPLANE (32 * WRS)

template <class F>
__device__ __forceinline__ F tr_frag(const short* p) {
  typedef s16x4 __attribute__((address_space(3))) * lds_s16x4_ptr;
  const s16x4 lo = __builtin_amdgcn_ds_read_tr16_b64_v4i16((lds_s16x4_ptr)(p));
  const s16x4 hi = __builtin_amdgcn_ds_read_tr16_b64_v4i16((lds_s16x4_ptr)(p + 4 * WRS));
  return __builtin_bit_cast(F, __builtin_shufflevector(lo, hi, 0, 1, 2, 3, 4, 5, 6, 7));
}
// ... 154 lines not shown
```

### neurips21-self-supervised-bug-detection-and-repair_amd/csrc/bl_gemm_x6.hip

```cpp
#include <stdio.h>
#include <stdlib.h>
#include <string.h>

#include "bl_common.h"
#include "bl_gemm_host.h"
#include "bl_gemm_split.h"
#include "bl_x6_locate.h"
#include "bl_x6w_image.h"
#include "bl_h3_image.h"

__global__ __launch_bounds__(256) void pack_rows_kernel(const float* __restrict__ x, int ld, long long R, int D,
                                                        uint4* __restrict__ out, int kg_total, int kg_off) {
  const int kgs = D >> 3;
  const long long t = (long long)blockIdx.x * blockDim.x + threadIdx.x;
  if (t >= R * kgs) return;
  const long long r = t / kgs;
  const int kgn = kg_total;
  const int kg = (int)(t % kgs) + kg_off;
  x -= 8 * kg_off;
  const float4 a = *reinterpret_cast<const float4*>(x + r * ld + 8 * kg);
  const float4 b = *reinterpret_cast<const float4*>(x + r * ld + 8 * kg + 4);
  const float v[8] = {a.x, a.y, a.z, a.w, b.x, b.y, b.z, b.w};
  uint16_t h[8], m[8], l[8];
#pragma unroll
// ... 349 lines not shown
                     bl_h3_sat_counter());
  BL_LAUNCH_CHECK("bl_pack_weights_multi");
  return BL_OK;
}

static int g_seq_gemm_mode = -1;
extern "C" int32_t bl_seq_gemm_mode(void) {
  if (g_seq_gemm_mode < 0) {
    const char* e = getenv("BL_SEQ_GEMM");
    g_seq_gemm_mode = (e && (strcmp(e, "x1") == 0 || strcmp(e, "bf16x1") == 0 || strcmp(e, "amp") == 0)) ? 1 : 0;
  }
  return g_seq_gemm_mode;
}
extern "C" int32_t bl_set_seq_gemm_mode(int32_t mode) {
  const int32_t prev = bl_seq_gemm_mode();
  BL_CHECK_ARG(mode == 0 || mode == 1, "bl_set_seq_gemm_mode: mode must be 0 (bf16x6) or 1 (bf16x1), got %d", mode);
  g_seq_gemm_mode = mode;
  return prev;
}

namespace {
int gemm_rows_x6_impl(const char* who, const bl_rows_packed_t* a, const uint32_t* win_bits, int32_t ld_bits, const uint16_t* bp,
                      int64_t b_group_stride, const int32_t* group_ptr, const int32_t* group_w, int32_t G, int32_t M, int32_t N,
                      int32_t K, const X6Epi* epi, float* c, int32_t ldc, void* stream) {
  const bool one = bl_seq_gemm_mode() == 1;
  if (M == 0) return BL_OK;
  BlPackedRows r;
  dim3 grid;
  if (int rc = bl_rows_gemm_plan(who, a, win_bits, ld_bits, bp, group_ptr, G, M, N, K, c, ldc, XBM, r, grid)) return rc;
  BL_CHECK_ARG(b_group_stride % 8 == 0 && (G <= 1 || b_group_stride >= (int64_t)((N + 127) / 128) * (K / 32) * 12288),
               "%s: packed group stride must cover one group's tiled weights (bl_pack_weights_x6)", who);
  BL_CHECK_ARG(!(win_bits && epi), "%s: the routed form has no epilogue", who);
  const int xcd = 1;
  X6Epi e = {nullptr, BL_ACT_NONE, 0u, 0u, 1.f, 0, nullptr, 0, nullptr, 1.f, nullptr, nullptr};
  if (epi) e = *epi;
#define X6_ARGS                                                                                                               \
  BL_PACKED_ROWS_ARGS(r), win_bits, ld_bits, reinterpret_cast<const uint4*>(bp), (long long)(b_group_stride / 8), group_ptr, \
      group_w, G, M, N, K, c, ldc, xcd, e
#define X6_LAUNCH(masked_, epi_)                                                                                        \
  {                                                                                                                    \
    if (one)                                                                                                           \
      hipLaunchKernelGGL((gemm_rows_x6_kernel<masked_, epi_, true>), grid, dim3(256), 0, (hipStream_t)stream, X6_ARGS);  \
    else                                                                                                               \
      hipLaunchKernelGGL((gemm_rows_x6_kernel<masked_, epi_, false>), grid, dim3(256), 0, (hipStream_t)stream, X6_ARGS); \
  }
  if (win_bits)
    X6_LAUNCH(true, -1)
  else if (epi && e.form == BL_X6_EPI_ACT_PACK && e.act == BL_ACT_RELU)
    X6_LAUNCH(false, 16 + BL_ACT_RELU)
  else if (epi && e.form == BL_X6_EPI_RES)
    X6_LAUNCH(false, 32)
  else if (epi && e.form == BL_X6_EPI_MASK_PACK)
    X6_LAUNCH(false, 64)
  else if (epi && e.form != BL_X6_EPI_ACT) {
    bl_set_error("%s: epilogue form %d with activation %d is not built (packed result: relu only)", who, e.form, e.act);
    return BL_EINVAL;
  } else if (epi == nullptr)
    X6_LAUNCH(false, -1)
  else if (e.act == BL_ACT_TANH)
    X6_LAUNCH(false, BL_ACT_TANH)
  else if (e.act == BL_ACT_RELU)
    X6_LAUNCH(false, BL_ACT_RELU)
  else if (e.act == BL_ACT_SIGMOID)
    X6_LAUNCH(false, BL_ACT_SIGMOID)
  else if (e.act == BL_ACT_NONE)
    X6_LAUNCH(false, BL_ACT_NONE)
  else {
    bl_set_error("%s: activation %d has no bf16x6 epilogue (none / relu / sigmoid / tanh)", who, e.act);
    return BL_EINVAL;
  }
  BL_LAUNCH_CHECK(who);
  return BL_OK;
}

bool g_wgrad_wide = true;

template <bool ROUTED, bool ONE>
int wgrad_x6_resident() {
  return bl_resident_workgroups<gemm_wgrad_x6_kernel<ROUTED, ONE>>(256, 2);
}

int gemm_wgrad_x6_impl(const char* who, const bl_rows_packed_t* a, const uint16_t* g_packed, const int32_t* g_idx,
                       const uint32_t* win_bits, int32_t ld_bits, const int32_t* group_ptr, const int32_t* group_w, int32_t G,
                       int32_t M, int32_t N, int32_t K, float* gw, int64_t gw_group_stride, int32_t ld_gw, bool one, void* stream) {
  if (M == 0) return BL_OK;
  BlPackedRows r;
  if (int rc = bl_packed_rows(who, a, K, r)) return rc;
  BL_CHECK_ARG(M > 0 && N > 0 && N % 32 == 0 && g_packed && gw && bl_aligned16(g_packed),
               "%s: N a multiple of 32 and aligned pointers required", who);
  const bool routed = win_bits != nullptr;
  BL_CHECK_ARG(!routed || (g_idx && ld_bits * 32 >= N), "%s: the routed form needs g_idx and ld_bits >= N / 32", who);
  bool wide = g_wgrad_wide && K % 256 == 0;
  int nidx = g_idx ? 1 : 0;
  for (int j = 0; j < a->nsrc; ++j) {
    wide = wide && a->width[j] % 128 == 0;
    nidx += a->idx[j] ? 1 : 0;
  }
  const bool gather = nidx == a->nsrc + 1;
  wide = wide && (gather || nidx == 0) && (gather || !routed);
  if (!gather && M < 65536) wide = false;
  if (one) wide = false;
  const int resident = wide ? bl_num_cus() : (one ? (routed ? wgrad_x6_resident<true, true>() : wgrad_x6_resident<false, true>())
                                                        : (routed ? wgrad_x6_resident<true, false>() : wgrad_x6_resident<false, false>()));
  const BlWgradPlan p = bl_wgrad_plan(group_ptr, group_w, G, M, N, K, wide ? 256 : XBM, XBN, resident, stream);
  const dim3 grid = p.grid;
#define WX6_ARGS                                                                                                              \
  BL_PACKED_ROWS_ARGS(r), reinterpret_cast<const uint4*>(g_packed), g_idx, win_bits, ld_bits, group_ptr, group_w, G, M, N, K, \
      p.kchunk, gw, (long long)gw_group_stride, ld_gw, p.ntiles_n, p.xcd, p.order_ctr
  if (wide && routed)
    hipLaunchKernelGGL((gemm_wgrad_x6_wide_kernel<true, true>), grid, dim3(512), 0, (hipStream_t)stream, WX6_ARGS);
  else if (wide && gather)
    hipLaunchKernelGGL((gemm_wgrad_x6_wide_kernel<false, true>), grid, dim3(512), 0, (hipStream_t)stream, WX6_ARGS);
  else if (wide)
    hipLaunchKernelGGL((gemm_wgrad_x6_wide_kernel<false, false>), grid, dim3(512), 0, (hipStream_t)stream, WX6_ARGS);
  else if (routed && one)
    hipLaunchKernelGGL((gemm_wgrad_x6_kernel<true, true>), grid, dim3(256), 0, (hipStream_t)stream, WX6_ARGS);
  else if (one)
    hipLaunchKernelGGL((gemm_wgrad_x6_kernel<false, true>), grid, dim3(256), 0, (hipStream_t)stream, WX6_ARGS);
  else if (routed)
    hipLaunchKernelGGL((gemm_wgrad_x6_kernel<true, false>), grid, dim3(256), 0, (hipStream_t)stream, WX6_ARGS);
  else
    hipLaunchKernelGGL((gemm_wgrad_x6_kernel<false, false>), grid, dim3(256), 0, (hipStream_t)stream, WX6_ARGS);
  BL_LAUNCH_CHECK(who);
  return BL_OK;
}
}

extern "C" int32_t bl_set_wgrad_tile(int32_t rows) {
  const int32_t prev = g_wgrad_wide ? 256 : 128;
  g_wgrad_wide = rows != 128;
  return prev;
}

extern "C" int32_t bl_set_wgrad_kchunk_cap(int32_t rows) {
  const int32_t prev = g_wgrad_kchunk_cap;
  if (rows >= 256) g_wgrad_kchunk_cap = rows;
  return prev;
}

extern "C" int bl_gemm_rows_x6(const bl_rows_packed_t* a, const uint32_t* win_bits, int32_t ld_bits, const uint16_t* bp,
                               int64_t b_group_stride, const int32_t* group_ptr, const int32_t* group_w, int32_t G,
                               int32_t M, int32_t N, int32_t K, float* c, int32_t ldc, void* stream) {
  return gemm_rows_x6_impl("bl_gemm_rows_x6", a, win_bits, ld_bits, bp, b_group_stride, group_ptr, group_w, G, M, N, K, nullptr, c, ldc,
                           stream);
}

extern "C" int bl_gemm_rows_x6_epi(const bl_rows_packed_t* a, const uint16_t* bp, int64_t b_group_stride, const int32_t* group_ptr,
                                   const int32_t* group_w, int32_t G, int32_t M, int32_t N, int32_t K, const float* bias,
                                   int32_t act, bl_dropout_t drop, float* c, int32_t ldc, void* stream) {
  BL_CHECK_ARG((uint64_t)M * (uint64_t)N < (1ull << 32) || drop.p <= 0.f, "bl_gemm_rows_x6_epi: dropout index space is 32 bit");
  BL_CHECK_ARG(bias == nullptr || bl_aligned16(bias), "bl_gemm_rows_x6_epi: misaligned bias");
  const bl_drop_dev d = bl_make_drop(drop);
  X6Epi e = {bias, act, d.key, d.thresh, d.scale, 0, nullptr, 0, nullptr, 1.f, nullptr, nullptr};
  return gemm_rows_x6_impl("bl_gemm_rows_x6_epi", a, nullptr, 0, bp, b_group_stride, group_ptr, group_w, G, M, N, K, &e, c, ldc, stream);
}

extern "C" int bl_gemm_rows_x6_epi2(const bl_rows_packed_t* a, const uint16_t* bp, int32_t M, int32_t N, int32_t K, const bl_x6_epi_t* epi,
                                    float* c, int32_t ldc, void* stream) {
  BL_CHECK_ARG(epi, "bl_gemm_rows_x6_epi2: null epilogue");
  BL_CHECK_ARG((uint64_t)M * (uint64_t)N < (1ull << 32) || epi->drop.p <= 0.f, "bl_gemm_rows_x6_epi2: dropout index space is 32 bit");
  BL_CHECK_ARG(epi->bias == nullptr || bl_aligned16(epi->bias), "bl_gemm_rows_x6_epi2: misaligned bias");
  const bool packs = epi->form == BL_X6_EPI_ACT_PACK || epi->form == BL_X6_EPI_MASK_PACK;
  BL_CHECK_ARG(!packs || (epi->c_packed && bl_aligned16(epi->c_packed) && N % 8 == 0),
               "bl_gemm_rows_x6_epi2: the packed result needs a 16-byte aligned buffer and N %% 8 == 0");
  BL_CHECK_ARG(epi->form != BL_X6_EPI_RES || (epi->res && bl_aligned16(epi->res) && epi->ld_res % 4 == 0 && epi->ld_res >= N),
               "bl_gemm_rows_x6_epi2: the residual needs an aligned [M, ld_res >= N] matrix");
  BL_CHECK_ARG(epi->form != BL_X6_EPI_MASK_PACK || (epi->y_packed && bl_aligned16(epi->y_packed)),
               "bl_gemm_rows_x6_epi2: the masked form needs the packed forward output");
  BL_CHECK_ARG(epi->form != BL_X6_EPI_MASK_PACK || epi->colsum == nullptr || !bl_get_deterministic(),
               "bl_gemm_rows_x6_epi2: the column sums are flushed by unordered atomics (deterministic mode is on)");
  const bl_drop_dev d = bl_make_drop(epi->drop);
  X6Epi e = {epi->bias, epi->act, d.key, d.thresh, d.scale, epi->form, epi->res, epi->ld_res,
             reinterpret_cast<const uint2*>(epi->y_packed), epi->mask_scale, epi->colsum, reinterpret_cast<uint2*>(epi->c_packed)};
  float* cc = packs ? reinterpret_cast<float*>(epi->c_packed) : c;
  return gemm_rows_x6_impl("bl_gemm_rows_x6_epi2", a, nullptr, 0, bp, 0, nullptr, nullptr, 1, M, N, K, &e, cc, packs ? N : ldc, stream);
}

extern "C" int bl_gemm_wgrad_routed_x6(const bl_rows_packed_t* a, const uint16_t* g_node_packed, const int32_t* g_idx,
                                       const uint32_t* win_bits, int32_t ld_bits, const int32_t* group_ptr,
                                       const int32_t* group_w, int32_t G, int32_t M, int32_t N, int32_t K, float* gw,
                                       int64_t gw_group_stride, int32_t ld_gw, void* stream) {
  BL_CHECK_ARG(M == 0 || (g_idx && win_bits), "bl_gemm_wgrad_routed_x6: needs g_idx and the winner bitmask");
  return gemm_wgrad_x6_impl("bl_gemm_wgrad_routed_x6", a, g_node_packed, g_idx, win_bits, ld_bits, group_ptr, group_w, G, M, N, K, gw,
                            gw_group_stride, ld_gw, false, stream);
}

extern "C" int bl_gemm_wgrad_x6(const bl_rows_packed_t* a, const uint16_t* g_packed, const int32_t* g_idx, const int32_t* group_ptr,
                                const int32_t* group_w, int32_t G, int32_t M, int32_t N, int32_t K, float* gw,
                                int64_t gw_group_stride, int32_t ld_gw, void* stream) {
  return gemm_wgrad_x6_impl("bl_gemm_wgrad_x6", a, g_packed, g_idx, nullptr, 0, group_ptr, group_w, G, M, N, K, gw, gw_group_stride, ld_gw,
                            bl_seq_gemm_mode() == 1, stream);
}
```

### neurips21-self-supervised-bug-detection-and-repair_amd/csrc/bl_graph_ops.hip

```cpp
#include "bl_common.h"

#define NEG_INF (-__builtin_huge_valf())
#define BL_MAX_WINS(t, best) ((t) > (best) || ((t) != (t) && (best) == (best)))

__global__ __launch_bounds__(256) void embed_fwd_kernel(const float* __restrict__ table, int H,
                                                        const int* __restrict__ ids, const int* __restrict__ lens,
                                                        int N, int S, bl_drop_dev drop, float* __restrict__ out,
                                                        int ld_out, int8_t* __restrict__ argsub, int drop_before_pool, int comb) {
  const int h4n = H >> 2;
  const long long t = (long long)blockIdx.x * blockDim.x + threadIdx.x;
  if (t >= (long long)N * h4n) return;
  const int n = (int)(t / h4n), h = (int)(t % h4n) * 4;
  int len = lens[n];
  len = len < 1 ? 1 : (len > S ? S : len);
  const bool pre = drop_before_pool && drop.thresh;
  float4 best = *reinterpret_cast<const float4*>(table + (size_t)ids[(size_t)n * S] * H + h);
  if (pre) {
    const uint32_t i = (uint32_t)n * (uint32_t)S * (uint32_t)H + (uint32_t)h;
    best.x = bl_keep(drop, i) ? best.x * drop.scale : 0.f;
    best.y = bl_keep(drop, i + 1) ? best.y * drop.scale : 0.f;
    best.z = bl_keep(drop, i + 2) ? best.z * drop.scale : 0.f;
    best.w = bl_keep(drop, i + 3) ? best.w * drop.scale : 0.f;
  }
  int a0 = 0, a1 = 0, a2 = 0, a3 = 0;
// ... 97 lines not shown
                                                               int comb, const int* __restrict__ lens) {
  const int lane = threadIdx.x & 63;
  const int c = blockIdx.x * (blockDim.x >> 6) + (threadIdx.x >> 6);
  if (c >= nchunks) return;
  const int beg = chunk_ptr[c], end = chunk_ptr[c + 1];
  float acc[NV];
#pragma unroll
  for (int j = 0; j < NV; ++j) acc[j] = 0.f;
  for (int base = beg; base < end; base += 64) {
    const int cnt = min(64, end - base);
    const int mine = lane < cnt ? occ[base + lane] : 0;
    for (int i0 = 0; i0 < cnt; i0 += 4) {
      float g[4][NV], inv[4];
      int a[4][NV], n[4], sl[4];
#pragma unroll
      for (int u = 0; u < 4; ++u) {
        const int pos = __shfl(mine, min(i0 + u, cnt - 1), 64);
        n[u] = pos / S;
        sl[u] = i0 + u < cnt ? pos - n[u] * S : -2;
        inv[u] = 1.f;
        if (comb == 2) {
          int len = lens[n[u]];
          len = len < 1 ? 1 : (len > S ? S : len);
          inv[u] = 1.0f / (float)len;
        }
#pragma unroll
        for (int j = 0; j < NV; ++j) {
          const int h = lane + 64 * j;
          g[u][j] = h < H ? g_out[(size_t)n[u] * ld_g + h] : 0.f;
          a[u][j] = comb != 0 ? (h < H ? sl[u] : -1) : (h < H ? (int)argsub[(size_t)n[u] * H + h] : -1);
        }
      }
#pragma unroll
      for (int u = 0; u < 4; ++u)
#pragma unroll
        for (int j = 0; j < NV; ++j) {
          float v = g[u][j];
          if (drop.thresh) v = bl_keep(drop, embed_mask_index(n[u], sl[u] < 0 ? 0 : sl[u], lane + 64 * j, S, H, drop_before_pool)) ? v * drop.scale : 0.f;
          if (a[u][j] == sl[u] && sl[u] >= 0) acc[j] += v * inv[u];
        }
    }
  }
  const size_t row = (size_t)chunk_tok[c] * H;
#pragma unroll
  for (int j = 0; j < NV; ++j) {
    const int h = lane + 64 * j;
    if (h < H && acc[j] != 0.f) unsafeAtomicAdd(&g_table[row + h], acc[j]);
  }
}

#define SEGMAX_HUB 40
#define SEGMAX_HUB_SLOTS 4096

template <int NV, bool GELU2>
__device__ __forceinline__ void segmax_scan(const float* __restrict__ x, int ldx, const int* __restrict__ seg_items, int beg, int end, int D,
                                            int act, float (&best)[NV], int (&barg)[NV], float (&low)[NV], int (&larg)[NV]) {
  constexpr int U = NV <= 4 ? 8 : 4;
  const int lane = threadIdx.x & 63;
  for (int base = beg; base < end; base += 64) {
    const int cnt = min(64, end - base);
    const int mine = lane < cnt ? (seg_items ? seg_items[base + lane] : base + lane) : 0;
    for (int i = 0; i < cnt; i += U) {
      int e[U];
      float v[U][NV];
#pragma unroll
      for (int u = 0; u < U; ++u) {
        e[u] = __shfl(mine, min(i + u, cnt - 1), 64);
        const float* __restrict__ row = x + (size_t)e[u] * ldx;
#pragma unroll
        for (int j = 0; j < NV; ++j) {
          const int d = lane + 64 * j;
          v[u][j] = d < D ? row[d] : NEG_INF;
        }
      }
#pragma unroll
      for (int u = 0; u < U; ++u) {
        if (i + u >= cnt) break;
#pragma unroll
        for (int j = 0; j < NV; ++j) {
          if (lane + 64 * j >= D) continue;
          float t = v[u][j];
          if (GELU2) {
            if (t < low[j]) { low[j] = t; larg[j] = e[u]; }
          } else if (act == BL_ACT_GELU) {
            t = bl_gelu(t);
          }
          if (BL_MAX_WINS(t, best[j])) { best[j] = t; barg[j] = e[u]; }
        }
      }
    }
  }
}

template <int NV, bool GELU2>
__device__ __forceinline__ void segmax_pick(float (&best)[NV], int (&barg)[NV], const float (&low)[NV], const int (&larg)[NV], float (&raw)[NV],
                                            float (&werf)[NV]) {
  if (GELU2) {
#pragma unroll
    for (int j = 0; j < NV; ++j) {
      raw[j] = best[j];
      werf[j] = 0.f;
      if (barg[j] < 0) continue;
      const float eh = erff(best[j] * 0.70710678118654752440f), el = erff(low[j] * 0.70710678118654752440f);
      const float gh = 0.5f * best[j] * (1.0f + eh), gl = 0.5f * low[j] * (1.0f + el);
      best[j] = gh;
      werf[j] = eh;
      if (gl > gh || gl != gl) { best[j] = gl; barg[j] = larg[j]; raw[j] = low[j]; werf[j] = el; }
    }
  }
}

template <int NV>
__device__ __forceinline__ void segmax_winbits(const int* __restrict__ seg_items, int beg, int end, int D, const int (&barg)[NV],
                                               uint32_t* __restrict__ winbits) {
  const int lane = threadIdx.x & 63;
  const int wpr = (D + 31) >> 5;
  for (int base = beg; base < end; base += 64) {
    const int cnt = min(64, end - base);
    const int mine = lane < cnt ? (seg_items ? seg_items[base + lane] : base + lane) : 0;
    for (int i = 0; i < cnt; ++i) {
      const int e = __shfl(mine, i, 64);
// ... 112 lines not shown
  if (HUBS && split) {
    if (wave > 0) {
#pragma unroll
      for (int j = 0; j < NV; ++j) { hub_f[wave - 1][lane + 64 * j] = best[j]; hub_i[wave - 1][lane + 64 * j] = barg[j]; }
    }
    __syncthreads();
    if (wave == 0) {
      for (int w = 0; w < 3; ++w) {
#pragma unroll
        for (int j = 0; j < NV; ++j) {
          const float tb = hub_f[w][lane + 64 * j];
          const int ab = hub_i[w][lane + 64 * j];
          if (ab >= 0 && BL_MAX_WINS(tb, best[j])) { best[j] = tb; barg[j] = ab; }
        }
      }
    }
    if (GELU2) {
      __syncthreads();
      if (wave > 0) {
#pragma unroll
        for (int j = 0; j < NV; ++j) { hub_f[wave - 1][lane + 64 * j] = low[j]; hub_i[wave - 1][lane + 64 * j] = larg[j]; }
      }
      __syncthreads();
      if (wave == 0) {
        for (int w = 0; w < 3; ++w) {
#pragma unroll
          for (int j = 0; j < NV; ++j) {
            const float tl = hub_f[w][lane + 64 * j];
            const int al = hub_i[w][lane + 64 * j];
            if (al >= 0 && tl < low[j]) { low[j] = tl; larg[j] = al; }
          }
        }
      }
    }
    if (wave == 0) {
      segmax_pick<NV, GELU2>(best, barg, low, larg, raw, werf);
#pragma unroll
      for (int j = 0; j < NV; ++j) hub_i[0][lane + 64 * j] = barg[j];
    }
    __syncthreads();
    if (winbits) {
      int fin[NV];
#pragma unroll
      for (int j = 0; j < NV; ++j) fin[j] = hub_i[0][lane + 64 * j];
      segmax_winbits<NV>(seg_items, wb, we, D, fin, winbits);
    }
    if (wave > 0) return;
  } else {
    segmax_pick<NV, GELU2>(best, barg, low, larg, raw, werf);
    if (winbits) segmax_winbits<NV>(seg_items, beg, end, D, barg, winbits);
  }
  segmax_finish<NV, HAS_LN, GELU2>(x, ldx, seg, D, act, best, barg, raw, werf, out, arg, ln_g, ln_b, eps, ln_out, mean_out, rstd_out, dact,
                                   ln_out_packed);
}

template <int NV, bool HAS_LN>
__global__ __launch_bounds__(256) void segment_sum_kernel(const float* __restrict__ x, int ldx, const int* __restrict__ seg_ptr,
                                                          const int* __restrict__ seg_items, int nseg, int D, int act, int mean_agg,
                                                          float* __restrict__ out, const float* __restrict__ ln_g,
                                                          const float* __restrict__ ln_b, float eps, float* __restrict__ ln_out,
                                                          float* __restrict__ mean_out, float* __restrict__ rstd_out,
                                                          float* __restrict__ dact, const int* __restrict__ seg_order,
                                                          uint32_t* __restrict__ ln_out_packed) {
  constexpr int U = NV <= 4 ? 8 : 4;
  const int lane = threadIdx.x & 63;
  const int slot = (int)blockIdx.x * 4 + (threadIdx.x >> 6);
  if (slot >= nseg) return;
  const int seg = seg_order ? seg_order[slot] : slot;
  const int beg = seg_ptr[seg], end = seg_ptr[seg + 1];
  float best[NV], raw[NV], werf[NV];
  int barg[NV];
#pragma unroll
  for (int j = 0; j < NV; ++j) { best[j] = 0.f; raw[j] = 0.f; werf[j] = 0.f; barg[j] = (end > beg && lane + 64 * j < D) ? 0 : -1; }
  for (int base = beg; base < end; base += 64) {
    const int cnt = min(64, end - base);
    const int mine = lane < cnt ? (seg_items ? seg_items[base + lane] : base + lane) : 0;
    for (int i = 0; i < cnt; i += U) {
      float v[U][NV];
#pragma unroll
      for (int u = 0; u < U; ++u) {
        const int e = __shfl(mine, min(i + u, cnt - 1), 64);
        const float* __restrict__ row = x + (size_t)e * ldx;
#pragma unroll
        for (int j = 0; j < NV; ++j) {
          const int d = lane + 64 * j;
          v[u][j] = d < D ? row[d] : 0.f;
        }
      }
#pragma unroll
      for (int u = 0; u < U; ++u) {
        if (i + u >= cnt) break;
#pragma unroll
        for (int j = 0; j < NV; ++j) best[j] += v[u][j];
      }
    }
  }
  float dscale = 1.f;
  if (mean_agg && end > beg) {
    dscale = 1.0f / (float)(end - beg);
#pragma unroll
    for (int j = 0; j < NV; ++j) best[j] *= dscale;
  }
  segmax_finish<NV, HAS_LN, false>(x, ldx, seg, D, act, best, barg, raw, werf, out, nullptr, ln_g, ln_b, eps, ln_out, mean_out, rstd_out, dact,
                                   ln_out_packed, dscale);
}

// ... 381 lines not shown
  BL_LAUNCH_CHECK(who);
  return BL_OK;
}

extern "C" int bl_embed_subtoken_pool_bwd_sorted(const float* g_out, int32_t ld_g, const int32_t* occ, const int32_t* chunk_ptr,
                                                 const int32_t* chunk_tok, int32_t nchunks, const int32_t* lens, const int8_t* argsub,
                                                 int32_t S, int32_t H, int32_t combination, bl_dropout_t drop, int32_t drop_before_pool,
                                                 float* g_table, void* stream) {
  const char* who = "bl_embed_subtoken_pool_bwd_sorted";
  if (nchunks == 0) return BL_OK;
  BL_CHECK_ARG(combination >= 0 && combination <= 2, "%s: combination must be 0 (max), 1 (sum) or 2 (mean)", who);
  BL_CHECK_ARG(g_out && occ && chunk_ptr && chunk_tok && g_table && (combination == 0 ? argsub != nullptr : true) &&
                   (combination == 2 ? lens != nullptr : true), "%s: null pointer", who);
  BL_CHECK_ARG(H > 0 && H <= 512 && S >= 1 && S <= 127, "%s: H in 1..512, 1 <= S <= 127", who);
  hipStream_t st = (hipStream_t)stream;
  DISPATCH_NV(H, hipLaunchKernelGGL((embed_bwd_sorted_kernel<NV>), dim3((nchunks + 3) / 4), dim3(256), 0, st, g_out, ld_g, occ,
                                     chunk_ptr, chunk_tok, nchunks, argsub, S, H, bl_make_drop(drop), g_table, drop_before_pool,
                                     combination, lens))
  BL_LAUNCH_CHECK(who);
  return BL_OK;
}

extern "C" int bl_embed_subtoken_max_fwd(const float* table, int32_t V, int32_t H, const int32_t* ids,
                                         const int32_t* lens, int32_t N, int32_t S, bl_dropout_t drop, int32_t drop_before_pool,
                                         float* out, int32_t ld_out, int8_t* argsub, void* stream) {
  return bl_embed_subtoken_pool_fwd(table, V, H, ids, lens, N, S, 0, drop, drop_before_pool, out, ld_out, argsub, stream);
}

extern "C" int bl_embed_subtoken_max_bwd(const float* g_out, int32_t ld_g, const int32_t* ids, const int8_t* argsub,
                                         int32_t N, int32_t S, int32_t H, int32_t V, bl_dropout_t drop, int32_t drop_before_pool,
                                         float* g_table, void* stream) {
  return bl_embed_subtoken_pool_bwd(g_out, ld_g, ids, nullptr, argsub, N, S, H, V, 0, drop, drop_before_pool, g_table, stream);
}

extern "C" int bl_embed_subtoken_max_bwd_sorted(const float* g_out, int32_t ld_g, const int32_t* occ,
                                               const int32_t* chunk_ptr, const int32_t* chunk_tok, int32_t nchunks,
                                               const int8_t* argsub, int32_t S, int32_t H, bl_dropout_t drop,
                                               int32_t drop_before_pool, float* g_table, void* stream) {
  return bl_embed_subtoken_pool_bwd_sorted(g_out, ld_g, occ, chunk_ptr, chunk_tok, nchunks, nullptr, argsub, S, H, 0, drop, drop_before_pool,
                                           g_table, stream);
}

extern "C" int bl_segment_max_fwd(const float* x, int32_t ldx, const int32_t* seg_ptr, const int32_t* seg_items,
                                  int32_t nseg, int32_t D, int32_t act, float* out, int32_t* arg, const float* ln_g,
                                  const float* ln_b, float eps, float* ln_out, float* mean, float* rstd, float* dact,
                                  uint32_t* winbits, const int32_t* seg_order, void* stream) {
  return bl_segment_max_fwd_impl(x, ldx, seg_ptr, seg_items, nseg, D, act, out, arg, ln_g, ln_b, eps, ln_out, mean, rstd, dact, winbits,
                                 seg_order, nullptr, -1, stream);
}

int bl_segment_max_fwd_impl(const float* x, int32_t ldx, const int32_t* seg_ptr, const int32_t* seg_items, int32_t nseg, int32_t D,
                            int32_t act, float* out, int32_t* arg, const float* ln_g, const float* ln_b, float eps, float* ln_out,
                            float* mean, float* rstd, float* dact, uint32_t* winbits, const int32_t* seg_order,
                            uint16_t* ln_out_packed, int32_t num_hub_slots, void* stream) {
  if (nseg == 0) return BL_OK;
  BL_CHECK_ARG(seg_ptr && (out || ln_g), "bl_segment_max_fwd: null pointer");
  BL_CHECK_ARG(D > 0 && D <= 512, "bl_segment_max_fwd: D must be in 1..512 (got %d)", D);
  BL_CHECK_ARG(ldx >= D, "bl_segment_max_fwd: ldx (%d) must be >= D (%d)", ldx, D);
  BL_CHECK_ARG(act == BL_ACT_NONE || act == BL_ACT_GELU || act == BL_ACT_GELU_AGG, "bl_segment_max_fwd: act must be NONE, GELU or GELU_AGG");
  const bool has_ln = ln_g != nullptr;
  BL_CHECK_ARG(!has_ln || (ln_b && (ln_out || ln_out_packed) && (mean == nullptr) == (rstd == nullptr)), "bl_segment_max_fwd: LayerNorm outputs missing");
  BL_CHECK_ARG(ln_out_packed == nullptr || (has_ln && D % 8 == 0), "bl_segment_max_fwd: the packed LayerNorm output needs D %% 8 == 0");
  hipStream_t st = (hipStream_t)stream;
  uint32_t* lnp = reinterpret_cast<uint32_t*>(ln_out_packed);
  const int hub_slots = seg_order ? (num_hub_slots < 0 ? min(nseg, SEGMAX_HUB_SLOTS) : min(nseg, num_hub_slots)) : 0;
  dim3 grid(hub_slots + (nseg - hub_slots + 3) / 4), block(256);
#define SEGMAX_GO(LN_, G2_)                                                                                                          \
  DISPATCH_NV(D, {                                                                                                                   \
    if (hub_slots > 0)                                                                                                               \
      hipLaunchKernelGGL((segment_max_kernel<NV, LN_, G2_, true>), grid, block, 0, st, x, ldx, seg_ptr, seg_items, nseg, D, act, out, \
                         arg, ln_g, ln_b, eps, ln_out, mean, rstd, dact, winbits, seg_order, lnp, hub_slots);                        \
    else                                                                                                                             \
      hipLaunchKernelGGL((segment_max_kernel<NV, LN_, G2_, false>), grid, block, 0, st, x, ldx, seg_ptr, seg_items, nseg, D, act,     \
                         out, arg, ln_g, ln_b, eps, ln_out, mean, rstd, dact, winbits, seg_order, lnp, 0);                           \
  })
  if (has_ln) {
    if (act == BL_ACT_GELU) SEGMAX_GO(true, true) else SEGMAX_GO(true, false)
  } else {
    if (act == BL_ACT_GELU) SEGMAX_GO(false, true) else SEGMAX_GO(false, false)
  }
  BL_LAUNCH_CHECK("bl_segment_max_fwd");
  return BL_OK;
}

int bl_segment_sum_fwd_impl(const float* x, int32_t ldx, const int32_t* seg_ptr, const int32_t* seg_items, int32_t nseg, int32_t D,
                            int32_t act, int32_t mean_agg, float* out, const float* ln_g, const float* ln_b, float eps, float* ln_out,
                            float* mean, float* rstd, float* dact, const int32_t* seg_order, uint16_t* ln_out_packed, void* stream) {
  if (nseg == 0) return BL_OK;
  BL_CHECK_ARG(seg_ptr && (out || ln_g), "bl_segment_sum_fwd: null pointer");
  BL_CHECK_ARG(D > 0 && D <= 512, "bl_segment_sum_fwd: D must be in 1..512 (got %d)", D);
  BL_CHECK_ARG(act == BL_ACT_NONE || act == BL_ACT_GELU_AGG, "bl_segment_sum_fwd: the activation sits on the aggregate (GELU_AGG) or is absent");
  const bool has_ln = ln_g != nullptr;
  BL_CHECK_ARG(!has_ln || (ln_b && (ln_out || ln_out_packed) && (mean == nullptr) == (rstd == nullptr)), "bl_segment_sum_fwd: LayerNorm outputs missing");
  BL_CHECK_ARG(ln_out_packed == nullptr || (has_ln && D % 8 == 0), "bl_segment_sum_fwd: the packed LayerNorm output needs D %% 8 == 0");
  hipStream_t st = (hipStream_t)stream;
  uint32_t* lnp = reinterpret_cast<uint32_t*>(ln_out_packed);
  dim3 grid((nseg + 3) / 4), block(256);
  DISPATCH_NV(D, {
    if (has_ln)
      hipLaunchKernelGGL((segment_sum_kernel<NV, true>), grid, block, 0, st, x, ldx, seg_ptr, seg_items, nseg, D, act, mean_agg, out, ln_g, ln_b,
                         eps, ln_out, mean, rstd, dact, seg_order, lnp);
    else
      hipLaunchKernelGGL((segment_sum_kernel<NV, false>), grid, block, 0, st, x, ldx, seg_ptr, seg_items, nseg, D, act, mean_agg, out, ln_g, ln_b,
                         eps, ln_out, mean, rstd, dact, seg_order, lnp);
  })
  BL_LAUNCH_CHECK("bl_segment_sum_fwd");
  return BL_OK;
}

extern "C" int bl_segment_max_bwd(const float* g_out, const int32_t* arg, const float* x, int32_t ldx,
                                  const int32_t* seg_of, int32_t nitems, int32_t D, int32_t act, float* g_x,
                                  void* stream) {
  if (nitems == 0) return BL_OK;
  BL_CHECK_ARG(g_out && arg && seg_of && g_x, "bl_segment_max_bwd: null pointer");
  BL_CHECK_ARG(D > 0 && D % 4 == 0 && ldx % 4 == 0, "bl_segment_max_bwd: D and ldx must be multiples of 4");
  BL_CHECK_ARG(act == BL_ACT_NONE || ((act == BL_ACT_GELU || act == BL_ACT_GELU_AGG) && x), "bl_segment_max_bwd: act must be NONE or GELU / GELU_AGG (+x)");
  const long long total = (long long)nitems * (D / 4);
// ... 245 lines not shown
```

### neurips21-self-supervised-bug-detection-and-repair_amd/csrc/bl_mp_layer.hip

```cpp
#include <vector>

#include <string.h>

#include "bl_common.h"

namespace {
struct ProfRec {
  int kind;
  double flop;
  hipEvent_t e0, e1;
  bool overlapped;
  double bytes;
};
bool g_prof_on = false;
std::vector<ProfRec> g_prof;
std::vector<hipEvent_t> g_prof_pool;
const char* kProfNames[] = {"pack_rows",      "msg_gemm_x6",  "segment_max_ln", "dense_fwd",    "act_bwd",       "dense_wgrad",
                            "dense_dgrad",    "layernorm_bwd", "msg_wgrad_x6",   "msg_dgrad_x6", "node_grad_sums", "msg_dgrad_nodes",
                            "node_update_bwd", "msg_gemm_h3", "msg_wgrad_h3", "msg_dgrad_h3", "pack_gq_h3",
                            "linear_x6_epi", "linear_dgrad_x6", "gemm_wgrad_x6", "attn_probs_fwd", "attn_probs_bwd", "attn_rows_times",
                            "attn_transposed_times", "add_layernorm", "layernorm_bwd_branch",
                            "winbits_or_runs",
                            "winbits_gather_live"};
constexpr int kProfWinbitsOrRuns = 26;
constexpr int kProfWinbitsGatherLive = 27;
constexpr int kProfKinds = sizeof(kProfNames) / sizeof(kProfNames[0]);
static_assert(kProfWinbitsGatherLive == kProfKinds - 1 && kProfWinbitsOrRuns == kProfKinds - 2, "the kProf constants must index their names");

hipEvent_t prof_event() {
  if (!g_prof_pool.empty()) {
    hipEvent_t e = g_prof_pool.back();
    g_prof_pool.pop_back();
    return e;
  }
  hipEvent_t e = nullptr;
  (void)hipEventCreate(&e);
  return e;
}

struct ProfScope {
  hipStream_t st;
  bool on;
  ProfScope(int kind, double flop, hipStream_t s, bool overlapped) : st(s), on(g_prof_on) {
    if (!on) return;
    ProfRec r{kind, flop, prof_event(), prof_event(), overlapped, 0.0};
    (void)hipEventRecord(r.e0, st);
    g_prof.push_back(r);
  }
  ~ProfScope() {
    if (on) (void)hipEventRecord(g_prof.back().e1, st);
  }
};
}

BlProfScope::BlProfScope(int kind, double flop, void* stream, double bytes, bool overlapped) : st(stream), on(g_prof_on) {
  if (!on) return;
  ProfRec r{kind, flop, prof_event(), prof_event(), overlapped, bytes};
  (void)hipEventRecord(r.e0, (hipStream_t)st);
  g_prof.push_back(r);
}
BlProfScope::~BlProfScope() {
  if (on) (void)hipEventRecord(g_prof.back().e1, (hipStream_t)st);
}

extern "C" int bl_prof_enable(int32_t on) {
  g_prof_on = on != 0;
  return BL_OK;
}
extern "C" int bl_prof_reset(void) {
  for (auto& r : g_prof) {
    g_prof_pool.push_back(r.e0);
    g_prof_pool.push_back(r.e1);
  }
  g_prof.clear();
  return BL_OK;
}
extern "C" int bl_prof_num_kinds(void) { return kProfKinds; }
extern "C" const char* bl_prof_kind_name(int32_t kind) { return kind >= 0 && kind < kProfKinds ? kProfNames[kind] : ""; }
extern "C" int bl_prof_read(int32_t kind, double* ms, double* flop, int64_t* launches, int32_t* overlapped) {
  double t = 0, f = 0;
// ... 84 lines not shown
  WsBwd w;
  char* p = (char*)base;
  size_t o = 0;
  auto take = [&](size_t b) { char* q = p ? p + o : nullptr; o += al(b); return q; };
  w.g_z = (float*)take((size_t)N * Dout * 6);
  w.g_ln = (float*)take((size_t)N * Dm * 4);
  w.gqp = (uint16_t*)take((size_t)N * 3 * Dm * 2);
  w.g_a = (float*)take((size_t)E * (full_ga ? 2 : 1) * Din * 4);
  w.amax = (float*)take(256);
  w.bytes = o;
  return w;
}

int g_msg_h3 = -1;
bool msg_h3() {
  if (g_msg_h3 < 0) {
    const char* e = getenv("BL_MSG_GEMM");
    g_msg_h3 = (e && (e[0] == 'x' || e[0] == 'b')) ? 0 : ((e && (strcmp(e, "amp") == 0 || strcmp(e, "f16x1") == 0)) ? 2 : 1);
    g_h3_one_term = g_msg_h3 == 2;
  }
  return g_msg_h3 >= 1;
}

bool g_fused_node_bwd = true;

int g_run_rows = -1;
bool run_rows_on() {
  if (g_run_rows < 0) {
    const char* e = getenv("BL_RUN_ROWS");
    g_run_rows = (e && e[0] == '0') ? 0 : 1;
  }
  return g_run_rows != 0;
}
int g_live_bwd = -1;
bool live_bwd_on() {
  if (g_live_bwd < 0) {
    const char* e = getenv("BL_LIVE_BWD");
    g_live_bwd = (e && e[0] == '0') ? 0 : 1;
  }
  return g_live_bwd != 0;
}
inline bool layer_has_live(const bl_mp_layer_t* L) {
  if (!(L->live_nodes && L->live_num_nodes > 0 && L->live_num_nodes <= L->N && L->live_recv && L->live_num_recv > 0 && L->live_num_recv <= L->N &&
        L->live_num_msgs >= 0 && L->live_num_msgs <= L->E && L->live_num_runs >= 0 && L->live_num_runs <= L->live_num_msgs && L->live_group_ptr))
    return false;
  return L->live_num_msgs == 0 || (L->live_msgs && L->live_run_ptr && L->live_rows_tgt && L->live_rows_src && L->live_src_ptr &&
                                   L->live_src_msgs && L->live_run_csr_ptr && L->live_run_csr_rows);
}
inline int layer_runs(const bl_mp_layer_t* L) {
  return (L->num_runs > 0 && L->run_ptr && L->bwd_group_ptr && L->bwd_group_w && L->bwd_rows_tgt && L->bwd_rows_src && L->tgt_run_ptr &&
          L->tgt_run_rows) ? L->num_runs : 0;
}

constexpr int kMaxDevices = 16;
struct SideEvents { hipEvent_t fork1 = nullptr, fork2 = nullptr, join = nullptr; };
SideEvents g_side_events[kMaxDevices];
SideEvents* ensure_events() {
  int dev = 0;
  if (hipGetDevice(&dev) != hipSuccess || dev < 0 || dev >= kMaxDevices) return nullptr;
  SideEvents& e = g_side_events[dev];
  if (e.join) return &e;
  if (hipEventCreateWithFlags(&e.fork1, hipEventDisableTiming) != hipSuccess || hipEventCreateWithFlags(&e.fork2, hipEventDisableTiming) != hipSuccess ||
      hipEventCreateWithFlags(&e.join, hipEventDisableTiming) != hipSuccess)
    return nullptr;
  return &e;
}

inline int saved_act_code(const bl_mp_layer_t* L) {
  return (L->aggregation == BL_AGG_MEAN && L->msg_act == BL_ACT_NONE) ? BL_ACT_GELU_AGG : L->msg_act;
}

int check_layer(const bl_mp_layer_t* L, const char* who) {
  BL_CHECK_ARG(L && L->N > 0 && L->E >= 0 && L->T > 0, "%s: bad sizes", who);
  BL_CHECK_ARG(L->Din % 32 == 0 && L->Dm % 32 == 0 && L->Dout % 4 == 0 && L->Din > 0 && L->Dm > 0 && L->Dm <= 512 && L->Dout > 0,
               "%s: the fused layer needs Din, Dm multiples of 32 (bf16x6 GEMMs), Dm <= 512", who);
  BL_CHECK_ARG(L->type_ptr && L->tgt_ptr && L->src_ptr && (L->E == 0 || (L->msg_src && L->msg_tgt && L->tgt_msgs && L->src_msgs)),
               "%s: null graph index array", who);
  BL_CHECK_ARG(L->W && L->ln_g && L->ln_b && L->Wd && L->bd, "%s: null parameter", who);
  BL_CHECK_ARG(L->msg_act == BL_ACT_NONE || L->msg_act == BL_ACT_GELU || L->msg_act == BL_ACT_GELU_AGG,
               "%s: message activation must be none, gelu (per message) or gelu_agg (on the aggregate)", who);
  BL_CHECK_ARG(L->aggregation >= BL_AGG_MAX && L->aggregation <= BL_AGG_MEAN, "%s: aggregation must be BL_AGG_MAX, BL_AGG_SUM or BL_AGG_MEAN", who);
  BL_CHECK_ARG(L->num_runs >= 0 && L->num_runs <= L->E && (long long)L->E + L->num_runs <= 0x7fffffffLL, "%s: num_runs outside 0..E", who);
  BL_CHECK_ARG(L->aggregation == BL_AGG_MAX || L->msg_act != BL_ACT_GELU,
               "%s: sum / mean aggregation takes the activation on the aggregate (BL_ACT_GELU_AGG) or none: a per-message activation would need "
               "the [E, Dm] messages again in backward", who);
  return BL_OK;
}
}

extern "C" int32_t bl_set_fused_node_bwd(int32_t on) {
  const int32_t prev = g_fused_node_bwd ? 1 : 0;
  g_fused_node_bwd = on != 0;
  return prev;
}

extern "C" int32_t bl_set_run_rows(int32_t on) {
  const int32_t prev = run_rows_on() ? 1 : 0;
  g_run_rows = on != 0 ? 1 : 0;
  return prev;
}

extern "C" int32_t bl_set_live_backward(int32_t on) {
  const int32_t prev = live_bwd_on() ? 1 : 0;
  g_live_bwd = on != 0 ? 1 : 0;
  return prev;
}

extern "C" int32_t bl_get_live_backward(void) { return live_bwd_on() ? 1 : 0; }

extern "C" int64_t bl_mp_layer_saved_bytes(int32_t N, int32_t E, int32_t Din, int32_t Dm, int32_t msg_act) {
  return (int64_t)carve_saved(nullptr, N, E, Din, Dm, msg_act).bytes;
}
extern "C" int64_t bl_mp_layer_workspace_bytes(int32_t N, int32_t E, int32_t Din, int32_t Dm, int32_t Dout, int32_t backward) {
  if (backward == 3) return (int64_t)carve_infer(nullptr, N, E, Din, Dm).bytes;
  if (backward) return (int64_t)carve_bwd(nullptr, N, E, Din, Dm, Dout, backward != 2).bytes;
  return (int64_t)al((size_t)E * Dm * 4);
}
extern "C" int32_t bl_mp_layer_weight_image(int32_t Din, int32_t Dm, int32_t for_backward) {
  if (msg_h3()) return 2;
  return for_backward ? bl_gemm_rows_x6w_ok(2 * Din, Dm) : bl_gemm_rows_x6w_ok(Dm, 2 * Din);
}
extern "C" int32_t bl_set_msg_gemm_mode(int32_t mode) {
  (void)msg_h3();
  const int32_t prev = g_msg_h3;
  g_msg_h3 = mode == 2 ? 2 : (mode ? 1 : 0);
  g_h3_one_term = g_msg_h3 == 2;
  return prev;
}
extern "C" int32_t bl_get_msg_gemm_mode(void) {
  (void)msg_h3();
  return g_msg_h3;
}

extern "C" int64_t bl_mp_layer_packed_weight_elems(int32_t T, int32_t Din, int32_t Dm, int32_t for_backward) {
  if (msg_h3()) return for_backward ? bl_packed_weight_elems_h3(T, Dm, 2 * Din) : bl_packed_weight_elems_h3(T, 2 * Din, Dm);
  if (bl_mp_layer_weight_image(Din, Dm, for_backward))
    return for_backward ? bl_packed_weight_elems_x6w(T, Dm, 2 * Din) : bl_packed_weight_elems_x6w(T, 2 * Din, Dm);
  return (int64_t)(for_backward ? packed_w_elems(T, Dm, 2 * Din) : packed_w_elems(T, 2 * Din, Dm));
}

#define BL_TRY(call_)        \
  do {                       \
    int rc_ = (call_);       \
    if (rc_ != BL_OK) return rc_; \
  } while (0)

extern "C" int bl_mp_layer_fwd(const bl_mp_layer_t* L, const float* h_lo, int32_t ld_lo, int32_t width_lo, const float* h_hi,
                               int32_t ld_hi, const uint16_t* w_packed, float* h_out, int32_t* winner_out, void* saved,
                               void* ws, void* stream) {
  BL_TRY(check_layer(L, "bl_mp_layer_fwd"));
  const int N = L->N, E = L->E, T = L->T, Din = L->Din, Dm = L->Dm, Dout = L->Dout;
  const bool infer = saved == nullptr;
  BL_CHECK_ARG(h_lo && w_packed && h_out && (ws || (E == 0 && !infer)), "bl_mp_layer_fwd: null buffer");
  BL_CHECK_ARG((h_hi == nullptr && width_lo == Din) || (h_hi != nullptr && width_lo > 0 && width_lo < Din && width_lo % 32 == 0),
               "bl_mp_layer_fwd: width_lo must be Din (one source) or a multiple of 32 below Din (two sources)");
  hipStream_t st = (hipStream_t)stream;
  const int32_t* node_order = L->num_hub_slots == 0 ? nullptr : L->node_order;
  Saved S = carve_saved(saved, N, E + layer_runs(L), Din, Dm, saved_act_code(L));
  float* pre = (float*)ws;
  if (infer) {
    const WsInfer I = carve_infer(ws, N, E, Din, Dm);
    pre = I.pre;
    S.hp = I.hp;
    S.ln_out = I.ln_out;
    S.dact = nullptr; S.bits = nullptr; S.agg = nullptr; S.mean = nullptr; S.rstd = nullptr;
  }
  const bool h3 = msg_h3();
  if (h3) {
    ProfScope ps(0, 0.0, st, false);
    BL_TRY(bl_pack_f16x2(h_lo, ld_lo, N, h_hi ? width_lo : Din, Din, 0, BL_H3_ROW_SCALE, nullptr, S.hp, st));
    if (h_hi) BL_TRY(bl_pack_f16x2(h_hi, ld_hi, N, Din - width_lo, Din, width_lo, BL_H3_ROW_SCALE, nullptr, S.hp, st));
  } else {
    ProfScope ps(0, 0.0, st, false);
    if (h_hi == nullptr) {
      BL_TRY(bl_pack_bf16x3(h_lo, ld_lo, N, Din, S.hp, st));
    } else {
      BL_TRY(bl_pack_bf16x3_cols(h_lo, ld_lo, N, width_lo, Din, 0, S.hp, st));
      BL_TRY(bl_pack_bf16x3_cols(h_hi, ld_hi, N, Din - width_lo, Din, width_lo, S.hp, st));
    }
  }
  bl_rows_packed_t a;
  a.xp[0] = S.hp; a.xp[1] = S.hp; a.xp[2] = nullptr;
  a.idx[0] = L->msg_src; a.idx[1] = L->msg_tgt; a.idx[2] = nullptr;
  a.width[0] = Din; a.width[1] = Din; a.width[2] = 0;
  a.nsrc = 2;
  if (h3) {
    ProfScope ps(13, 2.0 * E * (2.0 * Din) * Dm, st, false);
    BL_TRY(bl_gemm_rows_h3(&a, nullptr, 0, w_packed, bl_packed_weight_elems_h3(1, 2 * Din, Dm), L->type_ptr, nullptr, T, E, Dm, 2 * Din,
                           1.0f / (BL_H3_ROW_SCALE * BL_H3_W_SCALE), nullptr, pre, Dm, st));
  } else {
    ProfScope ps(1, 2.0 * E * (2.0 * Din) * Dm, st, false);
    if (bl_mp_layer_weight_image(Din, Dm, 0))
      BL_TRY(bl_gemm_rows_x6w(&a, nullptr, 0, w_packed, bl_packed_weight_elems_x6w(1, 2 * Din, Dm), L->type_ptr, nullptr, T, E, Dm,
                              2 * Din, pre, Dm, st));
    else
      BL_TRY(bl_gemm_rows_x6(&a, nullptr, 0, w_packed, (int64_t)packed_w_elems(1, 2 * Din, Dm), L->type_ptr, nullptr, T, E, Dm,
                             2 * Din, pre, Dm, st));
  }
  const bool dense_x6 = L->Wd_packed != nullptr && Dm % 32 == 0 && Dout % 32 == 0;
  {
    ProfScope ps(2, 0.0, st, false);
    if (L->aggregation != BL_AGG_MAX)
      BL_TRY(bl_segment_sum_fwd_impl(pre, Dm, L->tgt_ptr, L->tgt_msgs, N, Dm, L->msg_act, L->aggregation == BL_AGG_MEAN, S.agg, L->ln_g, L->ln_b,
                                     L->ln_eps, dense_x6 ? nullptr : S.ln_out, S.mean, S.rstd, S.dact, node_order,
                                     dense_x6 ? (uint16_t*)S.ln_out : nullptr, st));
    else
    BL_TRY(bl_segment_max_fwd_impl(pre, Dm, L->tgt_ptr, L->tgt_msgs, N, Dm, L->msg_act, S.agg, winner_out, L->ln_g, L->ln_b,
                                   L->ln_eps, dense_x6 ? nullptr : S.ln_out, S.mean, S.rstd, S.dact, S.bits, node_order,
                                   dense_x6 ? (uint16_t*)S.ln_out : nullptr, L->num_hub_slots, st));
  }
  {
    ProfScope ps(3, 2.0 * N * (double)Dm * Dout, st, false);
    if (dense_x6) {
      bl_rows_packed_t d;
      d.xp[0] = (const uint16_t*)S.ln_out; d.xp[1] = d.xp[2] = nullptr; d.idx[0] = d.idx[1] = d.idx[2] = nullptr;
      d.width[0] = Dm; d.width[1] = d.width[2] = 0; d.nsrc = 1;
      BL_TRY(bl_gemm_rows_x6_epi(&d, L->Wd_packed, 0, nullptr, nullptr, 1, N, Dout, Dm, L->bd, BL_ACT_TANH, L->drop, h_out, Dout, st));
    } else {
      bl_rows_t d;
      d.x[0] = S.ln_out; d.idx[0] = nullptr; d.ld[0] = Dm; d.width[0] = Dm; d.nsrc = 1;
      d.x[1] = d.x[2] = nullptr; d.idx[1] = d.idx[2] = nullptr; d.ld[1] = d.ld[2] = 0; d.width[1] = d.width[2] = 0;
      BL_TRY(bl_gemm_rows(&d, L->Wd, 0, Dout, 0, L->bd, nullptr, nullptr, 1, N, Dout, Dm, BL_ACT_TANH, L->drop, h_out, Dout, st));
    }
  }
  return BL_OK;
}

extern "C" int bl_mp_layer_bwd(const bl_mp_layer_t* L, const float* h_out, const float* g_out, const uint16_t* w_packed_bwd,
                               const void* saved, void* ws, float* g_h_lo, int32_t ld_lo, int32_t width_lo, float* g_h_hi,
                               int32_t ld_hi, float* g_W, float* g_ln_g, float* g_ln_b, float* g_Wd, float* g_bd,
                               void* stream, void* side_stream, int32_t join_side) {
  BL_TRY(check_layer(L, "bl_mp_layer_bwd"));
  const int N = L->N, E = L->E, T = L->T, Din = L->Din, Dm = L->Dm, Dout = L->Dout;
  BL_CHECK_ARG(h_out && g_out && saved && ws && g_h_lo && g_W && g_ln_g && g_ln_b && g_Wd && g_bd, "bl_mp_layer_bwd: null buffer");
  BL_CHECK_ARG(w_packed_bwd || (L->Wt && L->E > 0 && bl_routed_dgrad_vec_ok(L->Dm, 2 * L->Din)) || L->E == 0,
               "bl_mp_layer_bwd: w_packed_bwd may only be NULL when the input gradient takes the Wt path");
  BL_CHECK_ARG((g_h_hi == nullptr && width_lo == Din) || (g_h_hi != nullptr && width_lo > 0 && width_lo < Din),
               "bl_mp_layer_bwd: width_lo must be Din (one output) or below Din (two outputs)");
  hipStream_t st = (hipStream_t)stream, side = side_stream ? (hipStream_t)side_stream : st;
  const int32_t* node_order = L->num_hub_slots == 0 ? nullptr : L->node_order;
  const bool two = side != st;
  SideEvents* ev = two ? ensure_events() : nullptr;
  if (two) BL_CHECK_ARG(ev != nullptr, "bl_mp_layer_bwd: cannot create HIP events");
  const int R = layer_runs(L);
  Saved S = carve_saved(const_cast<void*>(saved), N, E + R, Din, Dm, saved_act_code(L));
  const uint32_t* bits = L->aggregation == BL_AGG_MAX ? S.bits : nullptr;
  const bool vec_dgrad = L->Wt != nullptr && E > 0 && bl_routed_dgrad_vec_ok(Dm, 2 * Din) && L->aggregation == BL_AGG_MAX;
  const bool fused_sums = vec_dgrad && !bl_get_deterministic();
  const bool run_rows = R > 0 && E > 0 && run_rows_on() && msg_h3() && g_msg_h3 == 1 && !vec_dgrad && L->aggregation == BL_AGG_MAX &&
                        Din % 128 == 0 && w_packed_bwd != nullptr;
  WsBwd B = carve_bwd(ws, N, E, Din, Dm, Dout, !fused_sums);

  const bool dense_x6 = L->Wd_packed != nullptr && L->Wd_packed_bwd != nullptr && Dm % 32 == 0 && Dout % 32 == 0;
  BL_CHECK_ARG(dense_x6 || L->Wd_packed == nullptr, "bl_mp_layer_bwd: Wd_packed given without Wd_packed_bwd");
  const bool fused_node = dense_x6 && g_fused_node_bwd && bl_node_update_bwd_ok(Dm, Dout);
  const int Ex = L->live_num_msgs, Rx = L->live_num_runs;
  const size_t live_ga_bytes = al(((size_t)Ex + Rx) * Din * 4);
  const bool live = run_rows && fused_node && live_bwd_on() && layer_has_live(L) &&
                    ((uint64_t)N * (uint64_t)Dout < (1ull << 32) || L->drop.p <= 0.f) &&
                    live_ga_bytes + ((size_t)Ex + Rx) * (Dm / 32) * 4 <= (size_t)E * 2 * Din * 4;
  const int Nn = live ? L->live_num_nodes : N;
  uint32_t* live_bits = live ? (uint32_t*)((char*)B.g_a + live_ga_bytes) : nullptr;
  const bool h3 = msg_h3();
  if (h3 && E > 0 && hipMemsetAsync(B.amax, 0, 4, st) != hipSuccess) { bl_set_error("bl_mp_layer_bwd: memset failed"); return BL_EINVAL; }
  if (fused_node) {
    ProfScope ps(12, 2.0 * Nn * (double)Dm * Dout, st, false);
    BL_TRY(bl_node_update_bwd_impl(g_out, h_out, Nn, Dout, L->drop, L->Wd_packed_bwd, S.agg, S.mean, S.rstd, L->ln_g, S.dact, Dm,
                                   (uint16_t*)B.g_z, g_bd, (vec_dgrad || h3) ? B.g_ln : nullptr, h3 ? nullptr : B.gqp, g_ln_g, g_ln_b,
                                   (h3 && E > 0) ? B.amax : nullptr, live ? L->live_nodes : nullptr, st));
  } else {
    ProfScope ps(4, 0.0, st, false);
    BL_TRY(bl_act_bwd_impl(g_out, h_out, N, Dout, Dout, BL_ACT_TANH, L->drop, dense_x6 ? nullptr : B.g_z, g_bd,
                           dense_x6 ? (uint16_t*)B.g_z : nullptr, st));
  }
  bl_rows_t r1;
  r1.x[1] = r1.x[2] = nullptr; r1.idx[0] = r1.idx[1] = r1.idx[2] = nullptr; r1.ld[1] = r1.ld[2] = 0; r1.width[1] = r1.width[2] = 0; r1.nsrc = 1;
  bl_rows_packed_t p1;
  p1.xp[1] = p1.xp[2] = nullptr; p1.idx[0] = p1.idx[1] = p1.idx[2] = nullptr; p1.width[1] = p1.width[2] = 0; p1.nsrc = 1;
  if (two) {
    (void)hipEventRecord(ev->fork1, st);
    (void)hipStreamWaitEvent(side, ev->fork1, 0);
  }
  {
    ProfScope ps(5, 2.0 * Nn * (double)Dm * Dout, side, two);
    if (dense_x6) {
      p1.xp[0] = (const uint16_t*)S.ln_out; p1.width[0] = Dm; p1.idx[0] = live ? L->live_nodes : nullptr;
      BL_TRY(bl_gemm_wgrad_x6(&p1, (const uint16_t*)B.g_z, nullptr, nullptr, nullptr, 1, Nn, Dout, Dm, g_Wd, 0, Dout, side));
      p1.idx[0] = nullptr;
    } else {
      r1.x[0] = S.ln_out; r1.ld[0] = Dm; r1.width[0] = Dm;
      BL_TRY(bl_gemm_wgrad(&r1, B.g_z, Dout, nullptr, nullptr, 1, N, Dout, Dm, g_Wd, 0, Dout, side));
    }
  }
  if (!fused_node) {
    ProfScope ps(6, 2.0 * N * (double)Dm * Dout, st, two);
    if (dense_x6) {
      p1.xp[0] = (const uint16_t*)B.g_z; p1.width[0] = Dout;
      bl_dropout_t nodrop = {0.f, 0u, 0u};
      BL_TRY(bl_gemm_rows_x6_epi(&p1, L->Wd_packed_bwd, 0, nullptr, nullptr, 1, N, Dm, Dout, nullptr, BL_ACT_NONE, nodrop, B.g_ln, Dm, st));
    } else {
      r1.x[0] = B.g_z; r1.ld[0] = Dout; r1.width[0] = Dout;
      bl_dropout_t nodrop = {0.f, 0u, 0u};
      BL_TRY(bl_gemm_rows(&r1, L->Wd, 0, Dout, 1, nullptr, nullptr, nullptr, 1, N, Dm, Dout, BL_ACT_NONE, nodrop, B.g_ln, Dm, st));
    }
  }
  if (!fused_node) {
    ProfScope ps(7, 0.0, st, two);
    BL_TRY(bl_layernorm_bwd(B.g_ln, S.agg, S.mean, S.rstd, L->ln_g, N, Dm, (vec_dgrad || h3) ? B.g_ln : nullptr, g_ln_g, g_ln_b, S.dact,
                            h3 ? nullptr : B.gqp, st));
  }
  if (h3 && E > 0) {
    ProfScope ps(16, 0.0, st, two);
    if (!fused_node) BL_TRY(bl_amax(B.g_ln, (int64_t)N * Dm, B.amax, st));
// ... 123 lines not shown
```

Measured before the change: 6023 graphs/s.

## Run trailing message-passing layers' forward over live rows only

Adds a 'live forward' mode. For the last layers whose outputs feed only the live (loss-relevant) nodes, the forward packs only the live receiver rows, runs the message GEMM over the live messages, aggregates only the live nodes, and writes the node update only to live rows, zeroing the rest for the last layer. A Python plan decides which trailing layers qualify, and the C side validates that the backward will take the matching live path. This is meant to cut forward GEMM and aggregation work that the backward already skips, at the cost of extra index kernels, a full memset of the output, and stricter coupling between forward and backward switches.

```diff
diff --git a/include/buglab_hip.h b/include/buglab_hip.h
--- a/include/buglab_hip.h
+++ b/include/buglab_hip.h
@@ -227,7 +227,10 @@
   const int32_t* live_src_msgs;
   const int32_t* live_run_csr_ptr;
   const int32_t* live_run_csr_rows;
+  int32_t live_fwd;
 } bl_mp_layer_t;
+#define BL_LIVE_FWD_INNER 1
+#define BL_LIVE_FWD_LAST 2
 #define BL_AGG_MAX 0
 #define BL_AGG_SUM 1
 #define BL_AGG_MEAN 2
@@ -269,6 +272,14 @@
                             int32_t split, float* g_h_lo, int32_t ld_lo, float* g_h_hi, int32_t ld_hi, void* stream);
 int32_t bl_set_live_backward(int32_t on);
 int32_t bl_get_live_backward(void);
+int32_t bl_mp_layer_live_ok(const bl_mp_layer_t* L, int32_t have_w_packed_bwd, int32_t forward, int32_t want_winners);
+int32_t bl_set_live_forward(int32_t on);
+int32_t bl_get_live_forward(void);
+int bl_pack_f16x2_rows(const float* x, int32_t ld, const int32_t* rows, int32_t R, int32_t D, int32_t D_total, int32_t col_off,
+                       float scale, uint16_t* out, void* stream);
+int bl_gemm_rows_x6_epi_rows(const bl_rows_packed_t* a, const uint16_t* bp, int32_t M, int32_t N, int32_t K, const float* bias,
+                             int32_t act, bl_dropout_t drop, const int32_t* out_rows, int32_t nrows_out, float* c, int32_t ldc,
+                             void* stream);
 
 int bl_prof_enable(int32_t on);
 int bl_prof_reset(void);
diff --git a/neurips21-self-supervised-bug-detection-and-repair_amd/buglab/models/hip_ops/_cabi.py b/neurips21-self-supervised-bug-detection-and-repair_amd/buglab/models/hip_ops/_cabi.py
--- a/neurips21-self-supervised-bug-detection-and-repair_amd/buglab/models/hip_ops/_cabi.py
+++ b/neurips21-self-supervised-bug-detection-and-repair_amd/buglab/models/hip_ops/_cabi.py
@@ -58,7 +58,7 @@
                 ("live_num_nodes", c_int32), ("live_num_recv", c_int32), ("live_num_msgs", c_int32), ("live_num_runs", c_int32),
                 ("live_nodes", c_void_p), ("live_recv", c_void_p), ("live_msgs", c_void_p), ("live_run_ptr", c_void_p),
                 ("live_group_ptr", c_void_p), ("live_rows_tgt", c_void_p), ("live_rows_src", c_void_p), ("live_src_ptr", c_void_p),
-                ("live_src_msgs", c_void_p), ("live_run_csr_ptr", c_void_p), ("live_run_csr_rows", c_void_p)]
+                ("live_src_msgs", c_void_p), ("live_run_csr_ptr", c_void_p), ("live_run_csr_rows", c_void_p), ("live_fwd", c_int32)]
 
 
 class bl_x6_epi_t(Structure):
@@ -127,6 +127,12 @@
                                  c_int32, c_void_p, c_int32, c_void_p], ctypes.c_int),
     "bl_set_live_backward": ([c_int32], c_int32),
     "bl_get_live_backward": ([], c_int32),
+    "bl_set_live_forward": ([c_int32], c_int32),
+    "bl_get_live_forward": ([], c_int32),
+    "bl_mp_layer_live_ok": ([c_void_p, c_int32, c_int32, c_int32], c_int32),
+    "bl_pack_f16x2_rows": ([c_void_p, c_int32, c_void_p, c_int32, c_int32, c_int32, c_int32, ctypes.c_float, c_void_p, c_void_p], ctypes.c_int),
+    "bl_gemm_rows_x6_epi_rows": ([c_void_p, c_void_p, c_int32, c_int32, c_int32, c_void_p, c_int32, bl_dropout_t, c_void_p, c_int32, c_void_p,
+                                  c_int32, c_void_p], ctypes.c_int),
     "bl_winbits_gather": ([c_void_p, c_int32, c_int32, c_void_p, c_int32, c_int32, c_void_p, c_int32, c_void_p], ctypes.c_int),
     "bl_node_update_bwd_rows": ([c_void_p, c_void_p, c_void_p, c_int32, c_int32, bl_dropout_t, c_void_p, c_void_p, c_void_p, c_void_p, c_void_p,
                                  c_void_p, c_int32, c_void_p, c_void_p, c_void_p, c_void_p, c_void_p, c_void_p, c_void_p], ctypes.c_int),
diff --git a/neurips21-self-supervised-bug-detection-and-repair_amd/buglab/models/hip_ops/graph.py b/neurips21-self-supervised-bug-detection-and-repair_amd/buglab/models/hip_ops/graph.py
--- a/neurips21-self-supervised-bug-detection-and-repair_amd/buglab/models/hip_ops/graph.py
+++ b/neurips21-self-supervised-bug-detection-and-repair_amd/buglab/models/hip_ops/graph.py
@@ -14,7 +14,7 @@
                    layernorm_bwd, pack_bf16x3, pack_weights_x6, scatter_add_rows, segment_max, x6_ok)
 from .weights import _as_groups, _packed_layer_weights, _packed_message_weights, _transposed_layer_weights
 
-__all__ = ["GraphIndex", "MessageRuns", "LiveRows", "live_rows_of", "POOLINGS", "AGGREGATIONS", "_EmbedSubtokenMax", "embed_subtoken_max", "_MpLayer", "node_update_bwd",
+__all__ = ["GraphIndex", "MessageRuns", "LiveRows", "live_rows_of", "live_forward_ok", "LIVE_FWD_INNER", "LIVE_FWD_LAST", "POOLINGS", "AGGREGATIONS", "_EmbedSubtokenMax", "embed_subtoken_max", "_MpLayer", "node_update_bwd",
            "_use_vector_dgrad", "_layer_desc", "_MpLayerFused", "_pending_uses", "set_grad_ready_callback", "_note_use",
            "_notify_backward_launched", "fused_layer_ok", "_GatedMpLayer", "gated_mp_layer", "_MpLayerFeat",
            "mp_layer_with_edge_features", "mp_layer"]
@@ -79,8 +79,10 @@
     num_hubs: int = -1
     runs: Optional[MessageRuns] = None
     live: Optional[LiveRows] = None
-
-
+    live_fwd: int = 0
+
+
+LIVE_FWD_INNER, LIVE_FWD_LAST = 1, 2
 POOLINGS = ("max", "sum", "mean")
 
 
@@ -259,7 +261,7 @@
     return bool(want) and E > 0 and bool(lib.bl_routed_dgrad_vec_ok(Dm, K2))
 
 
-def _layer_desc(g: "GraphIndex", W, ln_g, ln_b, Wd, bd, Din, msg_act, drop: Dropout, agg: int = 0, backward: bool = False) -> bl_mp_layer_t:
+def _layer_desc(g: "GraphIndex", W, ln_g, ln_b, Wd, bd, Din, msg_act, drop: Dropout, agg: int = 0, live_fwd: int = 0) -> bl_mp_layer_t:
     L = bl_mp_layer_t()
     L.aggregation = int(agg)
     L.N, L.E, L.T, L.Din, L.Dm, L.Dout = g.num_nodes, g.num_messages, W.shape[0], Din, W.shape[2], Wd.shape[1]
@@ -273,13 +275,33 @@
         L.num_runs = g.runs.num_runs
         for name in MessageRuns._fields:
             setattr(L, name, getattr(g.runs, name).data_ptr())
-    if backward and g.live is not None and g.live.nodes.shape[0] > 0:
+    if g.live is not None and g.live.nodes.shape[0] > 0:
         lv = g.live
         L.live_num_nodes, L.live_num_recv = int(lv.nodes.shape[0]), int(lv.recv.shape[0])
         L.live_num_msgs, L.live_num_runs = int(lv.msgs.shape[0]), int(lv.run_ptr.shape[0]) - 1
         for name in LiveRows._fields:
             setattr(L, "live_" + name, getattr(lv, name).data_ptr())
+    L.live_fwd = int(live_fwd)
     return L
+
+
+def live_forward_ok(din: int, lo_width: Optional[int], W, ln_g, ln_b, Wd, bd, g: "GraphIndex", msg_act: str, drop: Dropout,
+                    aggregation: str = "max") -> bool:
+    if g.live is None or g.live.nodes.shape[0] == 0 or not torch.is_grad_enabled():
+        return False
+    if not (fused_layer_ok(din, W.shape[2]) and (lo_width is None or lo_width % 32 == 0)):
+        return False
+    if not all(p.requires_grad for p in (W, ln_g, ln_b, Wd, bd)):
+        return False
+    lib = load_library()
+    agg = AGGREGATIONS.index(aggregation)
+    Dm, Dout = W.shape[2], Wd.shape[1]
+    if not (_switches.DENSE_X6 and Dm % 32 == 0 and Dout % 32 == 0):
+        return False
+    use_vec = agg == 0 and _use_vector_dgrad(lib, g.num_messages, Dm, 2 * din)
+    L = _layer_desc(g, W, ln_g, ln_b, Wd, bd, din, _ACTS[msg_act], drop, agg)
+    L.Wd_packed = _packed_layer_weights(Wd, True)[0].data_ptr()
+    return bool(lib.bl_mp_layer_live_ok(ctypes.byref(L), 0 if use_vec else 1, 1, 1 if _switches.WINNER_SINK is not None else 0))
 
 
 class _MpLayerFused(torch.autograd.Function):
@@ -301,7 +323,7 @@
         wkn, wnk = _packed_message_weights(W, Din, need_bwd and not use_vec)
         wt = _transposed_layer_weights(W) if (need_bwd and use_vec) else None
         dev = h_lo.device
-        L = _layer_desc(g, W, ln_g, ln_b, Wd, bd, Din, msg_act, drop, agg)
+        L = _layer_desc(g, W, ln_g, ln_b, Wd, bd, Din, msg_act, drop, agg, live_fwd=g.live_fwd)
         dense_x6 = _switches.DENSE_X6 and Dm % 32 == 0 and Dout % 32 == 0
         wd_kn = wd_nk = None
         if dense_x6:
@@ -343,7 +365,7 @@
         direct = [_direct_small(bd), _direct_small(ln_g), _direct_small(ln_b), _direct_grad_target(Wd), _direct_grad_target(W)]
         tgt = [d if d is not None else torch.zeros_like(p) for d, p in zip(direct, (bd, ln_g, ln_b, Wd, W))]
         g_bd, g_lng, g_lnb, g_Wd, g_W = tgt
-        L = _layer_desc(g, W, ln_g, ln_b, Wd, bd, Din, msg_act, drop, agg, backward=True)
+        L = _layer_desc(g, W, ln_g, ln_b, Wd, bd, Din, msg_act, drop, agg, live_fwd=g.live_fwd)
         if dense_x6:
             if wd_nk is None:
                 wd_nk = pack_weights_x6(_as_groups(Wd.detach()), False)
@@ -544,6 +566,8 @@
     if fused_layer_ok(Din, W.shape[2]) and (not pair or h[0].shape[1] % 32 == 0):
         lo, hi = (h[0].contiguous(), h[1].contiguous()) if pair else (h.contiguous(), None)
         return _MpLayerFused.apply(lo, hi, W, ln_g, ln_b, Wd, bd, graph, _ACTS[msg_act], drop, agg)
+    if graph.live_fwd:
+        raise RuntimeError("mp_layer: the graph index asks for the live forward, which only the one-call layer form has")
     if agg != 0:
         raise NotImplementedError("sum / mean message aggregation runs in the one-call layer form only (state and message widths multiples of "
                                   "32, message width <= 512, FUSED_LAYER on)")
diff --git a/neurips21-self-supervised-bug-detection-and-repair_amd/buglab/models/hip_ops/runtime.py b/neurips21-self-supervised-bug-detection-and-repair_amd/buglab/models/hip_ops/runtime.py
--- a/neurips21-self-supervised-bug-detection-and-repair_amd/buglab/models/hip_ops/runtime.py
+++ b/neurips21-self-supervised-bug-detection-and-repair_amd/buglab/models/hip_ops/runtime.py
@@ -6,7 +6,8 @@
 from ._cabi import load_library
 
 __all__ = ["set_deterministic", "_MSG_GEMM_MODES", "set_msg_gemm_mode", "msg_gemm_mode", "set_seq_gemm_mode", "seq_gemm_mode", "set_wgrad_tile",
-           "set_wgrad_kchunk_cap", "set_fused_node_bwd", "set_run_rows", "set_live_backward", "live_backward", "deterministic"]
+           "set_wgrad_kchunk_cap", "set_fused_node_bwd", "set_run_rows", "set_live_backward", "live_backward", "set_live_forward", "live_forward",
+           "deterministic"]
 
 
 def set_deterministic(on: bool = True) -> None:
@@ -63,5 +64,13 @@
     return bool(load_library().bl_get_live_backward())
 
 
+def set_live_forward(on: bool) -> bool:
+    return bool(load_library().bl_set_live_forward(1 if on else 0))
+
+
+def live_forward() -> bool:
+    return bool(load_library().bl_get_live_forward())
+
+
 def deterministic() -> bool:
     return bool(load_library().bl_get_deterministic())
diff --git a/neurips21-self-supervised-bug-detection-and-repair_amd/buglab/models/layers/messagepassing.py b/neurips21-self-supervised-bug-detection-and-repair_amd/buglab/models/layers/messagepassing.py
--- a/neurips21-self-supervised-bug-detection-and-repair_amd/buglab/models/layers/messagepassing.py
+++ b/neurips21-self-supervised-bug-detection-and-repair_amd/buglab/models/layers/messagepassing.py
@@ -162,6 +162,31 @@
         self.mp = nn.ModuleList(mp)
         self.input_node_state_dim = node_embedder.embedding_size
         self.output_node_state_dim = [l for l in layer_recipe if isinstance(l, nn.Module)][-1].output_state_dimension
+
+    def _live_forward_plan(self, graph: GraphIndex, live, mk) -> Dict[int, int]:
+        if not isinstance(self._recipe[-1], nn.Module):
+            return {}
+        seq, width, stash = [], self.input_node_state_dim, {}
+        for layer in self._recipe:
+            if isinstance(layer, _PassThrough):
+                stash[id(layer.owner)] = width
+            elif isinstance(layer, ConcatResidualLayer):
+                width = (stash.pop(id(layer)), width)
+            else:
+                seq.append((layer, width[0] if isinstance(width, tuple) else None, sum(width) if isinstance(width, tuple) else width))
+                width = layer.output_state_dimension
+        plan: Dict[int, int] = {}
+        for depth in range(min(len(live), len(seq))):
+            li = len(seq) - 1 - depth
+            layer, lo_width, din = seq[li]
+            if not (isinstance(layer, MlpMessagePassingLayer) and layer.features_dimension == 0):
+                break
+            if not hip_ops.live_forward_ok(din, lo_width, layer.W, layer.ln_g, layer.ln_b, layer.Wd, layer.bd, graph._replace(live=live[depth]),
+                                           layer._msg_act(), mk(layer.dropout_rate, 1 + li),
+                                           getattr(layer, "message_aggregation_function", "max")):
+                break
+            plan[li] = hip_ops.LIVE_FWD_LAST if depth == 0 else hip_ops.LIVE_FWD_INNER
+        return plan
 
     @property
     def message_passing_layers(self):
@@ -192,6 +217,7 @@
         if live_backward and live_arrays is not None and live_layout is not None and not return_all_states and input_transform is None:
             live = live_rows_of(live_arrays, live_layout, graph.num_types)
         num_mp = sum(1 for l in self._recipe if isinstance(l, nn.Module))
+        live_fwd = self._live_forward_plan(graph, live, mk) if live else {}
         h = h0
         all_states = [h0]
         stash: Dict[int, torch.Tensor] = {}
@@ -205,7 +231,7 @@
                 if isinstance(h, tuple) and not isinstance(layer, MlpMessagePassingLayer):
                     h = torch.cat(h, dim=-1)
                 depth = num_mp - 1 - li
-                layer_graph = graph._replace(live=live[depth]) if depth < len(live) else graph
+                layer_graph = graph._replace(live=live[depth], live_fwd=live_fwd.get(li, 0)) if depth < len(live) else graph
                 if isinstance(layer, MlpMessagePassingLayer) and layer.features_dimension > 0:
                     h = layer(h, graph, mk(layer.dropout_rate, 1 + li), edge_features)
                 else:
diff --git a/neurips21-self-supervised-bug-detection-and-repair_amd/csrc/bl_common.h b/neurips21-self-supervised-bug-detection-and-repair_amd/csrc/bl_common.h
--- a/neurips21-self-supervised-bug-detection-and-repair_amd/csrc/bl_common.h
+++ b/neurips21-self-supervised-bug-detection-and-repair_amd/csrc/bl_common.h
@@ -17,7 +17,8 @@
 int bl_segment_max_fwd_impl(const float* x, int32_t ldx, const int32_t* seg_ptr, const int32_t* seg_items, int32_t nseg, int32_t D,
                             int32_t act, float* out, int32_t* arg, const float* ln_g, const float* ln_b, float eps, float* ln_out,
                             float* mean, float* rstd, float* dact, uint32_t* winbits, const int32_t* seg_order,
-                            uint16_t* ln_out_packed, int32_t num_hub_slots, void* stream);
+                            uint16_t* ln_out_packed, int32_t num_hub_slots, void* stream,
+                            const int32_t* item_row = nullptr, int32_t x_rows = 0);
 int bl_segment_sum_fwd_impl(const float* x, int32_t ldx, const int32_t* seg_ptr, const int32_t* seg_items, int32_t nseg, int32_t D,
                             int32_t act, int32_t mean_agg, float* out, const float* ln_g, const float* ln_b, float eps, float* ln_out,
                             float* mean, float* rstd, float* dact, const int32_t* seg_order, uint16_t* ln_out_packed, void* stream);
diff --git a/neurips21-self-supervised-bug-detection-and-repair_amd/csrc/bl_gemm_h3.hip b/neurips21-self-supervised-bug-detection-and-repair_amd/csrc/bl_gemm_h3.hip
--- a/neurips21-self-supervised-bug-detection-and-repair_amd/csrc/bl_gemm_h3.hip
+++ b/neurips21-self-supervised-bug-detection-and-repair_amd/csrc/bl_gemm_h3.hip
@@ -7,14 +7,15 @@
 #include "bl_x6_locate.h"
 #include "bl_h3_image.h"
 
+template <bool LIST>
 __global__ __launch_bounds__(256) void pack_rows_h_kernel(const float* __restrict__ x, int ld, long long R, int D, uint4* __restrict__ out,
                                                           int kg_total, int kg_off, float scale, const float* __restrict__ amax_dev,
-                                                          unsigned* __restrict__ sat_counter) {
+                                                          unsigned* __restrict__ sat_counter, const int* __restrict__ rows) {
   const int kgs = D >> 3;
   const long long t = (long long)blockIdx.x * blockDim.x + threadIdx.x;
   if (t >= R * kgs) return;
   if (amax_dev) scale *= h3_scale_from_amax(*amax_dev);
-  const long long r = t / kgs;
+  const long long r = LIST ? (long long)rows[t / kgs] : t / kgs;
   const int kgn = kg_total;
   const int kg = (int)(t % kgs) + kg_off;
   x -= 8 * kg_off;
@@ -104,9 +105,23 @@
                "bl_pack_f16x2: widths / offset must be multiples of 8 with col_off + D <= D_total");
   BL_CHECK_ARG(scale > 0.f, "bl_pack_f16x2: scale must be positive (a power of two)");
   const long long total = (long long)R * (D / 8);
-  hipLaunchKernelGGL(pack_rows_h_kernel, dim3((unsigned)((total + 255) / 256)), dim3(256), 0, (hipStream_t)stream, x, ld, (long long)R, D,
-                     reinterpret_cast<uint4*>(out), D_total / 8, col_off / 8, scale, amax_dev, bl_h3_sat_counter());
+  hipLaunchKernelGGL(pack_rows_h_kernel<false>, dim3((unsigned)((total + 255) / 256)), dim3(256), 0, (hipStream_t)stream, x, ld, (long long)R, D,
+                     reinterpret_cast<uint4*>(out), D_total / 8, col_off / 8, scale, amax_dev, bl_h3_sat_counter(), nullptr);
   BL_LAUNCH_CHECK("bl_pack_f16x2");
+  return BL_OK;
+}
+
+extern "C" int bl_pack_f16x2_rows(const float* x, int32_t ld, const int32_t* rows, int32_t R, int32_t D, int32_t D_total, int32_t col_off,
+                                  float scale, uint16_t* out, void* stream) {
+  if (R == 0) return BL_OK;
+  BL_CHECK_ARG(x && out && rows && R > 0 && bl_aligned16(x) && bl_aligned16(out), "bl_pack_f16x2_rows: null or misaligned pointer");
+  BL_CHECK_ARG(D > 0 && D % 8 == 0 && ld % 4 == 0 && D_total % 8 == 0 && col_off % 8 == 0 && col_off >= 0 && col_off + D <= D_total,
+               "bl_pack_f16x2_rows: widths / offset must be multiples of 8 with col_off + D <= D_total");
+  BL_CHECK_ARG(scale > 0.f, "bl_pack_f16x2_rows: scale must be positive (a power of two)");
+  const long long total = (long long)R * (D / 8);
+  hipLaunchKernelGGL(pack_rows_h_kernel<true>, dim3((unsigned)((total + 255) / 256)), dim3(256), 0, (hipStream_t)stream, x, ld, (long long)R, D,
+                     reinterpret_cast<uint4*>(out), D_total / 8, col_off / 8, scale, nullptr, bl_h3_sat_counter(), rows);
+  BL_LAUNCH_CHECK("bl_pack_f16x2_rows");
   return BL_OK;
 }
 
diff --git a/neurips21-self-supervised-bug-detection-and-repair_amd/csrc/bl_gemm_split.h b/neurips21-self-supervised-bug-detection-and-repair_amd/csrc/bl_gemm_split.h
--- a/neurips21-self-supervised-bug-detection-and-repair_amd/csrc/bl_gemm_split.h
+++ b/neurips21-self-supervised-bug-detection-and-repair_amd/csrc/bl_gemm_split.h
@@ -62,6 +62,7 @@
   float mask_scale;
   float* colsum;
   uint2* c_packed;
+  const int* out_rows;
 };
 
 template <class S, bool MASKED, int EPI, bool ONE>
@@ -72,7 +73,8 @@
     long long strideB, const int* __restrict__ group_ptr, const int* __restrict__ group_w, int G, int M, int N, int K,
     float* __restrict__ c, int ldc, int xcd_remap, X6Epi epi, float out_scale, const float* __restrict__ a_amax_dev) {
   static_assert(EPI == -1 || !S::SCALED, "the epilogues are built for the unscaled split only");
-  constexpr bool E_ACT = EPI >= 0 && EPI < 32, E_PACK = EPI >= 16 && (EPI < 32 || EPI == 64), E_RES = EPI == 32, E_MASK = EPI == 64;
+  constexpr bool E_ROWS = EPI >= 128 && EPI < 144;
+  constexpr bool E_ACT = (EPI >= 0 && EPI < 32) || E_ROWS, E_PACK = EPI >= 16 && (EPI < 32 || EPI == 64), E_RES = EPI == 32, E_MASK = EPI == 64;
   constexpr int ACT = EPI >= 0 ? (EPI & 15) : 0;
   constexpr bool SWZ = S::swizzled(MASKED);
   constexpr int NP = ONE ? 1 : S::NP;
@@ -203,6 +205,7 @@
 #pragma unroll
   for (int ti = 0; ti < 2; ++ti) {
     const int m = wm * 64 + ti * 32 + li;
+    const uint32_t drow = E_ROWS ? (uint32_t)epi.out_rows[row0 + min(m, nrows - 1)] : (uint32_t)(row0 + m);
 #pragma unroll
     for (int tj = 0; tj < 2; ++tj)
 #pragma unroll
@@ -221,7 +224,7 @@
           for (int u = 0; u < 4; ++u) {
             v[u] = bl_act(ACT, v[u]);
             if (epi.drop_thresh) {
-              const uint32_t idx = (uint32_t)(row0 + m) * (uint32_t)N + (uint32_t)(n + u);
+              const uint32_t idx = drow * (uint32_t)N + (uint32_t)(n + u);
               v[u] = ((bl_lowbias32(idx + epi.drop_key) >> 8) >= epi.drop_thresh) ? v[u] * epi.drop_scale : 0.f;
             }
           }
@@ -235,7 +238,7 @@
       const int mm = wm * 64 + ti * 32 + r;
       float4 v = *reinterpret_cast<const float4*>(stage + r * 68 + 4 * c4);
       if (mm < nrows && n < N) {
-        const size_t grow = (size_t)(row0 + mm);
+        const size_t grow = E_ROWS ? (size_t)epi.out_rows[row0 + mm] : (size_t)(row0 + mm);
         if (E_RES) {
           const float4 rv = *reinterpret_cast<const float4*>(epi.res + grow * epi.ld_res + n);
           v.x += rv.x; v.y += rv.y; v.z += rv.z; v.w += rv.w;
diff --git a/neurips21-self-supervised-bug-detection-and-repair_amd/csrc/bl_gemm_x6.hip b/neurips21-self-supervised-bug-detection-and-repair_amd/csrc/bl_gemm_x6.hip
--- a/neurips21-self-supervised-bug-detection-and-repair_amd/csrc/bl_gemm_x6.hip
+++ b/neurips21-self-supervised-bug-detection-and-repair_amd/csrc/bl_gemm_x6.hip
@@ -425,7 +425,13 @@
     X6_LAUNCH(false, 32)
   else if (epi && e.form == BL_X6_EPI_MASK_PACK)
     X6_LAUNCH(false, 64)
-  else if (epi && e.form != BL_X6_EPI_ACT) {
+  else if (epi && e.out_rows) {
+    if (e.form != BL_X6_EPI_ACT || e.act != BL_ACT_TANH) {
+      bl_set_error("%s: the row-list epilogue is built for bias / tanh / dropout only (got form %d, activation %d)", who, e.form, e.act);
+      return BL_EINVAL;
+    }
+    X6_LAUNCH(false, 128 + BL_ACT_TANH)
+  } else if (epi && e.form != BL_X6_EPI_ACT) {
     bl_set_error("%s: epilogue form %d with activation %d is not built (packed result: relu only)", who, e.form, e.act);
     return BL_EINVAL;
   } else if (epi == nullptr)
@@ -528,6 +534,17 @@
   return gemm_rows_x6_impl("bl_gemm_rows_x6_epi", a, nullptr, 0, bp, b_group_stride, group_ptr, group_w, G, M, N, K, &e, c, ldc, stream);
 }
 
+extern "C" int bl_gemm_rows_x6_epi_rows(const bl_rows_packed_t* a, const uint16_t* bp, int32_t M, int32_t N, int32_t K, const float* bias,
+                                        int32_t act, bl_dropout_t drop, const int32_t* out_rows, int32_t nrows_out, float* c, int32_t ldc,
+                                        void* stream) {
+  BL_CHECK_ARG(out_rows && nrows_out >= M, "bl_gemm_rows_x6_epi_rows: out_rows missing or fewer output rows than result rows");
+  BL_CHECK_ARG((uint64_t)nrows_out * (uint64_t)N < (1ull << 32) || drop.p <= 0.f, "bl_gemm_rows_x6_epi_rows: dropout index space is 32 bit");
+  BL_CHECK_ARG(bias == nullptr || bl_aligned16(bias), "bl_gemm_rows_x6_epi_rows: misaligned bias");
+  const bl_drop_dev d = bl_make_drop(drop);
+  X6Epi e = {bias, act, d.key, d.thresh, d.scale, 0, nullptr, 0, nullptr, 1.f, nullptr, nullptr, out_rows};
+  return gemm_rows_x6_impl("bl_gemm_rows_x6_epi_rows", a, nullptr, 0, bp, 0, nullptr, nullptr, 1, M, N, K, &e, c, ldc, stream);
+}
+
 extern "C" int bl_gemm_rows_x6_epi2(const bl_rows_packed_t* a, const uint16_t* bp, int32_t M, int32_t N, int32_t K, const bl_x6_epi_t* epi,
                                     float* c, int32_t ldc, void* stream) {
   BL_CHECK_ARG(epi, "bl_gemm_rows_x6_epi2: null epilogue");
diff --git a/neurips21-self-supervised-bug-detection-and-repair_amd/csrc/bl_graph_ops.hip b/neurips21-self-supervised-bug-detection-and-repair_amd/csrc/bl_graph_ops.hip
--- a/neurips21-self-supervised-bug-detection-and-repair_amd/csrc/bl_graph_ops.hip
+++ b/neurips21-self-supervised-bug-detection-and-repair_amd/csrc/bl_graph_ops.hip
@@ -173,21 +173,23 @@
 #define SEGMAX_HUB 40
 #define SEGMAX_HUB_SLOTS 4096
 
-template <int NV, bool GELU2>
+template <int NV, bool GELU2, bool MAP = false>
 __device__ __forceinline__ void segmax_scan(const float* __restrict__ x, int ldx, const int* __restrict__ seg_items, int beg, int end, int D,
-                                            int act, float (&best)[NV], int (&barg)[NV], float (&low)[NV], int (&larg)[NV]) {
+                                            int act, float (&best)[NV], int (&barg)[NV], float (&low)[NV], int (&larg)[NV],
+                                            const int* __restrict__ item_row = nullptr, int x_rows = 0) {
   constexpr int U = NV <= 4 ? 8 : 4;
   const int lane = threadIdx.x & 63;
   for (int base = beg; base < end; base += 64) {
     const int cnt = min(64, end - base);
     const int mine = lane < cnt ? (seg_items ? seg_items[base + lane] : base + lane) : 0;
+    const int mine_row = (MAP && lane < cnt) ? min(max(item_row[mine], 0), max(x_rows - 1, 0)) : 0;
     for (int i = 0; i < cnt; i += U) {
       int e[U];
       float v[U][NV];
 #pragma unroll
       for (int u = 0; u < U; ++u) {
         e[u] = __shfl(mine, min(i + u, cnt - 1), 64);
-        const float* __restrict__ row = x + (size_t)e[u] * ldx;
+        const float* __restrict__ row = x + (size_t)(MAP ? __shfl(mine_row, min(i + u, cnt - 1), 64) : e[u]) * ldx;
 #pragma unroll
         for (int j = 0; j < NV; ++j) {
           const int d = lane + 64 * j;
@@ -406,6 +408,23 @@
   }
   segmax_finish<NV, HAS_LN, GELU2>(x, ldx, seg, D, act, best, barg, raw, werf, out, arg, ln_g, ln_b, eps, ln_out, mean_out, rstd_out, dact,
                                    ln_out_packed);
+}
+
+template <int NV, bool GELU2>
+__global__ __launch_bounds__(256) void segment_max_rows_kernel(SEGMAX_PARAMS, const int* __restrict__ item_row, int x_rows) {
+  const int slot = (int)blockIdx.x * 4 + (threadIdx.x >> 6);
+  if (slot >= nseg) return;
+  const int seg = seg_order[slot];
+  const int beg = seg_ptr[seg], end = seg_ptr[seg + 1];
+  float best[NV], low[NV], raw[NV], werf[NV];
+  int barg[NV], larg[NV];
+#pragma unroll
+  for (int j = 0; j < NV; ++j) { best[j] = NEG_INF; barg[j] = -1; low[j] = -NEG_INF; larg[j] = -1; raw[j] = 0.f; werf[j] = 0.f; }
+  segmax_scan<NV, GELU2, true>(x, ldx, seg_items, beg, end, D, act, best, barg, low, larg, item_row, x_rows);
+  segmax_pick<NV, GELU2>(best, barg, low, larg, raw, werf);
+  if (winbits) segmax_winbits<NV>(seg_items, beg, end, D, barg, winbits);
+  segmax_finish<NV, true, GELU2>(x, ldx, seg, D, act, best, barg, raw, werf, out, arg, ln_g, ln_b, eps, ln_out, mean_out, rstd_out, dact,
+                                 ln_out_packed);
 }
 
 template <int NV, bool HAS_LN>
@@ -893,7 +912,7 @@
 int bl_segment_max_fwd_impl(const float* x, int32_t ldx, const int32_t* seg_ptr, const int32_t* seg_items, int32_t nseg, int32_t D,
                             int32_t act, float* out, int32_t* arg, const float* ln_g, const float* ln_b, float eps, float* ln_out,
                             float* mean, float* rstd, float* dact, uint32_t* winbits, const int32_t* seg_order,
-                            uint16_t* ln_out_packed, int32_t num_hub_slots, void* stream) {
+                            uint16_t* ln_out_packed, int32_t num_hub_slots, void* stream, const int32_t* item_row, int32_t x_rows) {
   if (nseg == 0) return BL_OK;
   BL_CHECK_ARG(seg_ptr && (out || ln_g), "bl_segment_max_fwd: null pointer");
   BL_CHECK_ARG(D > 0 && D <= 512, "bl_segment_max_fwd: D must be in 1..512 (got %d)", D);
@@ -904,6 +923,20 @@
   BL_CHECK_ARG(ln_out_packed == nullptr || (has_ln && D % 8 == 0), "bl_segment_max_fwd: the packed LayerNorm output needs D %% 8 == 0");
   hipStream_t st = (hipStream_t)stream;
   uint32_t* lnp = reinterpret_cast<uint32_t*>(ln_out_packed);
+  if (item_row) {
+    BL_CHECK_ARG(has_ln && seg_order && seg_items && arg == nullptr && x_rows >= 0, "bl_segment_max_fwd: the row-mapped form needs LayerNorm, seg_order and seg_items, and writes no winner table");
+    dim3 grid((nseg + 3) / 4), block(256);
+    DISPATCH_NV(D, {
+      if (act == BL_ACT_GELU)
+        hipLaunchKernelGGL((segment_max_rows_kernel<NV, true>), grid, block, 0, st, x, ldx, seg_ptr, seg_items, nseg, D, act, out, arg, ln_g,
+                           ln_b, eps, ln_out, mean, rstd, dact, winbits, seg_order, lnp, 0, item_row, x_rows);
+      else
+        hipLaunchKernelGGL((segment_max_rows_kernel<NV, false>), grid, block, 0, st, x, ldx, seg_ptr, seg_items, nseg, D, act, out, arg, ln_g,
+                           ln_b, eps, ln_out, mean, rstd, dact, winbits, seg_order, lnp, 0, item_row, x_rows);
+    })
+    BL_LAUNCH_CHECK("bl_segment_max_fwd");
+    return BL_OK;
+  }
   const int hub_slots = seg_order ? (num_hub_slots < 0 ? min(nseg, SEGMAX_HUB_SLOTS) : min(nseg, num_hub_slots)) : 0;
   dim3 grid(hub_slots + (nseg - hub_slots + 3) / 4), block(256);
 #define SEGMAX_GO(LN_, G2_)                                                                                                          \
diff --git a/neurips21-self-supervised-bug-detection-and-repair_amd/csrc/bl_mp_layer.hip b/neurips21-self-supervised-bug-detection-and-repair_amd/csrc/bl_mp_layer.hip
--- a/neurips21-self-supervised-bug-detection-and-repair_amd/csrc/bl_mp_layer.hip
+++ b/neurips21-self-supervised-bug-detection-and-repair_amd/csrc/bl_mp_layer.hip
@@ -21,11 +21,14 @@
                             "linear_x6_epi", "linear_dgrad_x6", "gemm_wgrad_x6", "attn_probs_fwd", "attn_probs_bwd", "attn_rows_times",
                             "attn_transposed_times", "add_layernorm", "layernorm_bwd_branch",
                             "winbits_or_runs",
-                            "winbits_gather_live"};
+                            "winbits_gather_live",
+                            "live_index_fwd"};
 constexpr int kProfWinbitsOrRuns = 26;
 constexpr int kProfWinbitsGatherLive = 27;
+constexpr int kProfLiveIndexFwd = 28;
 constexpr int kProfKinds = sizeof(kProfNames) / sizeof(kProfNames[0]);
-static_assert(kProfWinbitsGatherLive == kProfKinds - 1 && kProfWinbitsOrRuns == kProfKinds - 2, "the kProf constants must index their names");
+static_assert(kProfLiveIndexFwd == kProfKinds - 1 && kProfWinbitsGatherLive == kProfKinds - 2 && kProfWinbitsOrRuns == kProfKinds - 3,
+              "the kProf constants must index their names");
 
 hipEvent_t prof_event() {
   if (!g_prof_pool.empty()) {
@@ -216,6 +219,70 @@
           L->tgt_run_rows) ? L->num_runs : 0;
 }
 
+int g_live_fwd = -1;
+bool live_fwd_on() {
+  if (g_live_fwd < 0) {
+    const char* e = getenv("BL_LIVE_FWD");
+    g_live_fwd = (e && e[0] == '0') ? 0 : 1;
+  }
+  return g_live_fwd != 0;
+}
+
+struct WsLiveFwd {
+  float* pre;
+  int32_t* msg_pos;
+  int32_t* tgt_id;
+  size_t bytes;
+};
+WsLiveFwd carve_live_fwd(void* base, int E, int Ex, int Dm) {
+  WsLiveFwd w;
+  char* p = (char*)base;
+  size_t o = 0;
+  auto take = [&](size_t b) { char* q = p ? p + o : nullptr; o += al(b); return q; };
+  w.pre = (float*)take((size_t)Ex * Dm * 4);
+  w.msg_pos = (int32_t*)take((size_t)E * 4);
+  w.tgt_id = (int32_t*)take((size_t)Ex * 4);
+  w.bytes = o;
+  return w;
+}
+
+bool live_ok(const bl_mp_layer_t* L, bool have_w_bwd, bool forward, bool want_winners, const char** why) {
+  const char* dummy;
+  if (!why) why = &dummy;
+  const int N = L->N, E = L->E, Din = L->Din, Dm = L->Dm, Dout = L->Dout;
+#define LIVE_NEEDS(cond_, text_) \
+  if (!(cond_)) { *why = text_; return false; }
+  LIVE_NEEDS(live_bwd_on(), "the live backward is switched off (bl_set_live_backward / BL_LIVE_BWD)");
+  LIVE_NEEDS(layer_has_live(L), "the descriptor carries no (complete) live arrays");
+  LIVE_NEEDS(layer_runs(L) > 0 && E > 0 && run_rows_on(), "the run rows are off or the minibatch carries no run arrays");
+  LIVE_NEEDS(msg_h3() && g_msg_h3 == 1, "the message GEMMs are not in the f16x3 three-term mode");
+  LIVE_NEEDS(L->aggregation == BL_AGG_MAX, "the aggregation is not max");
+  LIVE_NEEDS(have_w_bwd && !(L->Wt != nullptr && bl_routed_dgrad_vec_ok(Dm, 2 * Din)), "the input gradient takes the vector-unit (Wt) path");
+  LIVE_NEEDS(Din % 128 == 0, "Din is not a multiple of 128");
+  LIVE_NEEDS(L->Wd_packed != nullptr && Dm % 32 == 0 && Dout % 32 == 0, "the dense node update is not on the bf16x6 path");
+  LIVE_NEEDS(g_fused_node_bwd && bl_node_update_bwd_ok(Dm, Dout), "the one-kernel node update backward does not apply (shape, switch or deterministic mode)");
+  LIVE_NEEDS((uint64_t)N * (uint64_t)Dout < (1ull << 32) || L->drop.p <= 0.f, "the dropout counter of a node's own row leaves 32 bits");
+  const size_t Ex = (size_t)L->live_num_msgs, Rx = (size_t)L->live_num_runs;
+  LIVE_NEEDS(al((Ex + Rx) * Din * 4) + (Ex + Rx) * (Dm / 32) * 4 <= (size_t)E * 2 * Din * 4, "the compact gradient and masks do not fit the backward workspace");
+  if (forward) {
+    LIVE_NEEDS(live_fwd_on(), "the live forward is switched off (bl_set_live_forward / BL_LIVE_FWD)");
+    LIVE_NEEDS(!want_winners, "a winner table is wanted");
+    LIVE_NEEDS(carve_live_fwd(nullptr, E, (int)Ex, Dm).bytes <= al((size_t)E * Dm * 4), "the compact pre-activations and index arrays do not fit the forward workspace");
+  }
+#undef LIVE_NEEDS
+  return true;
+}
+
+__global__ __launch_bounds__(256) void live_index_kernel(const int* __restrict__ live_msgs, const int* __restrict__ msg_tgt, int Ex, int E,
+                                                         int* __restrict__ msg_pos, int* __restrict__ tgt_id) {
+  const int i = (int)(blockIdx.x * blockDim.x + threadIdx.x);
+  if (i >= Ex) return;
+  const int e = live_msgs[i];
+  if ((unsigned)e >= (unsigned)E) return;
+  msg_pos[e] = i;
+  tgt_id[i] = msg_tgt[e];
+}
+
 constexpr int kMaxDevices = 16;
 struct SideEvents { hipEvent_t fork1 = nullptr, fork2 = nullptr, join = nullptr; };
 SideEvents g_side_events[kMaxDevices];
@@ -271,6 +338,22 @@
 }
 
 extern "C" int32_t bl_get_live_backward(void) { return live_bwd_on() ? 1 : 0; }
+
+extern "C" int32_t bl_set_live_forward(int32_t on) {
+  const int32_t prev = live_fwd_on() ? 1 : 0;
+  g_live_fwd = on != 0 ? 1 : 0;
+  return prev;
+}
+
+extern "C" int32_t bl_get_live_forward(void) { return live_fwd_on() ? 1 : 0; }
+
+extern "C" int32_t bl_mp_layer_live_ok(const bl_mp_layer_t* L, int32_t have_w_packed_bwd, int32_t forward, int32_t want_winners) {
+  if (L == nullptr || check_layer(L, "bl_mp_layer_live_ok") != BL_OK) return 0;
+  const char* why = nullptr;
+  const bool ok = live_ok(L, have_w_packed_bwd != 0, forward != 0, want_winners != 0, &why);
+  if (!ok) bl_set_error("bl_mp_layer_live_ok: %s", why);
+  return ok ? 1 : 0;
+}
 
 extern "C" int64_t bl_mp_layer_saved_bytes(int32_t N, int32_t E, int32_t Din, int32_t Dm, int32_t msg_act) {
   return (int64_t)carve_saved(nullptr, N, E, Din, Dm, msg_act).bytes;
@@ -330,6 +413,53 @@
     S.dact = nullptr; S.bits = nullptr; S.agg = nullptr; S.mean = nullptr; S.rstd = nullptr;
   }
   const bool h3 = msg_h3();
+  if (L->live_fwd) {
+    const char* why = nullptr;
+    if (infer || !live_ok(L, true, true, winner_out != nullptr, &why)) {
+      bl_set_error("bl_mp_layer_fwd: live_fwd is set but the layer cannot run over its live rows: %s", infer ? "forward-only call (saved == NULL)" : why);
+      return BL_EINVAL;
+    }
+    const int Nx = L->live_num_nodes, Nr = L->live_num_recv, Ex = L->live_num_msgs;
+    const WsLiveFwd V = carve_live_fwd(ws, E, Ex, Dm);
+    if (L->live_fwd == BL_LIVE_FWD_LAST &&
+        hipMemsetAsync(h_out, 0, (size_t)N * Dout * 4, st) != hipSuccess) {
+      bl_set_error("bl_mp_layer_fwd: memset failed");
+      return BL_EINVAL;
+    }
+    if (Ex > 0) {
+      ProfScope ps(kProfLiveIndexFwd, 0.0, st, false);
+      hipLaunchKernelGGL(live_index_kernel, dim3((unsigned)((Ex + 255) / 256)), dim3(256), 0, st, L->live_msgs, L->msg_tgt, Ex, E, V.msg_pos, V.tgt_id);
+      BL_LAUNCH_CHECK("bl_mp_layer_fwd (live index)");
+    }
+    {
+      ProfScope ps(0, 0.0, st, false);
+      BL_TRY(bl_pack_f16x2_rows(h_lo, ld_lo, L->live_recv, Nr, h_hi ? width_lo : Din, Din, 0, BL_H3_ROW_SCALE, S.hp, st));
+      if (h_hi) BL_TRY(bl_pack_f16x2_rows(h_hi, ld_hi, L->live_recv, Nr, Din - width_lo, Din, width_lo, BL_H3_ROW_SCALE, S.hp, st));
+    }
+    if (Ex > 0) {
+      bl_rows_packed_t a;
+      a.xp[0] = S.hp; a.xp[1] = S.hp; a.xp[2] = nullptr;
+      a.idx[0] = L->live_rows_src; a.idx[1] = V.tgt_id; a.idx[2] = nullptr;
+      a.width[0] = Din; a.width[1] = Din; a.width[2] = 0;
+      a.nsrc = 2;
+      ProfScope ps(13, 2.0 * Ex * (2.0 * Din) * Dm, st, false);
+      BL_TRY(bl_gemm_rows_h3(&a, nullptr, 0, w_packed, bl_packed_weight_elems_h3(1, 2 * Din, Dm), L->live_group_ptr, nullptr, T, Ex, Dm, 2 * Din,
+                             1.0f / (BL_H3_ROW_SCALE * BL_H3_W_SCALE), nullptr, V.pre, Dm, st));
+    }
+    {
+      ProfScope ps(2, 0.0, st, false);
+      BL_TRY(bl_segment_max_fwd_impl(V.pre, Dm, L->tgt_ptr, L->tgt_msgs, Nx, Dm, L->msg_act, S.agg, nullptr, L->ln_g, L->ln_b, L->ln_eps, nullptr,
+                                     S.mean, S.rstd, S.dact, S.bits, L->live_nodes, (uint16_t*)S.ln_out, 0, st, V.msg_pos, Ex));
+    }
+    {
+      ProfScope ps(3, 2.0 * Nx * (double)Dm * Dout, st, false);
+      bl_rows_packed_t d;
+      d.xp[0] = (const uint16_t*)S.ln_out; d.xp[1] = d.xp[2] = nullptr; d.idx[0] = L->live_nodes; d.idx[1] = d.idx[2] = nullptr;
+      d.width[0] = Dm; d.width[1] = d.width[2] = 0; d.nsrc = 1;
+      BL_TRY(bl_gemm_rows_x6_epi_rows(&d, L->Wd_packed, Nx, Dout, Dm, L->bd, BL_ACT_TANH, L->drop, L->live_nodes, N, h_out, Dout, st));
+    }
+    return BL_OK;
+  }
   if (h3) {
     ProfScope ps(0, 0.0, st, false);
     BL_TRY(bl_pack_f16x2(h_lo, ld_lo, N, h_hi ? width_lo : Din, Din, 0, BL_H3_ROW_SCALE, nullptr, S.hp, st));
@@ -420,9 +550,13 @@
   const bool fused_node = dense_x6 && g_fused_node_bwd && bl_node_update_bwd_ok(Dm, Dout);
   const int Ex = L->live_num_msgs, Rx = L->live_num_runs;
   const size_t live_ga_bytes = al(((size_t)Ex + Rx) * Din * 4);
-  const bool live = run_rows && fused_node && live_bwd_on() && layer_has_live(L) &&
-                    ((uint64_t)N * (uint64_t)Dout < (1ull << 32) || L->drop.p <= 0.f) &&
-                    live_ga_bytes + ((size_t)Ex + Rx) * (Dm / 32) * 4 <= (size_t)E * 2 * Din * 4;
+  const char* why_not = "the run-row path or the one-kernel node update does not apply";
+  const bool live = run_rows && fused_node && live_ok(L, w_packed_bwd != nullptr, false, false, &why_not);
+  if (L->live_fwd && !live) {
+    bl_set_error("bl_mp_layer_bwd: this layer's forward ran over its live rows, but backward cannot take the live path: %s (a switch "
+                 "was changed between forward and backward?)", why_not);
+    return BL_EINVAL;
+  }
   const int Nn = live ? L->live_num_nodes : N;
   uint32_t* live_bits = live ? (uint32_t*)((char*)B.g_a + live_ga_bytes) : nullptr;
   const bool h3 = msg_h3();
```

New measurement: 6869 graphs/s (median of 6 runs). 14.1% higher.
